# lms-07/LGTEUN

Hardware: AMD Instinct MI355X
Metric: train image-pairs/sec, GF-2 4-band 128x128, K=4, bs=32/GPU (higher is better)
Workload: dtype f32 (GEMMs and the local mixer: split 16-bit MFMA -- f16 pairs in the forward FFN, the W2 products of its backward and P V, bf16 triples elsewhere -- fp32 accumulate; fp32-equivalent); 1 GPU; BASELINE configs[1]: C=4, MS 32x32, PAN 128x128, K=4, 32 pairs/GPU, train step = fwd + L1 + bwd + Adam + StepLR tick; mode=faithful, global_batch=32, parallelism=dp1, dropout=True

## Files before the change

include/lgteun_hip.h:

```cpp
#ifndef LGTEUN_HIP_H
#define LGTEUN_HIP_H

#include <stddef.h>
#include <stdint.h>

#ifdef __cplusplus
extern "C" {
#endif

#define LG_TENSORS_SHARED 12
#define LG_TENSORS_PER_STAGE 119

#define LG_FLAG_FAITHFUL 1
#define LG_FLAG_SAVE 2
#define LG_FLAG_DROPOUT 4

#define LG_FLAG_BWD_LGT 8
#define LG_FLAG_BWD_DATA 16

#define LG_FLAG_CHAINED 32

#define LG_FLAG_DEFER_DEAD 64

enum lg_kernel_id {
    LG_K_NONE = 0, LG_K_FFN1, LG_K_FFN2, LG_K_FFT, LG_K_ATTN, LG_K_UPFUSE, LG_K_DOWN, LG_K_EMBED, LG_K_TAIL, LG_K_DATASTEP,
    LG_K_FFN1_BWD, LG_K_FFN2_BWD, LG_K_FFT_BWD, LG_K_ATTN_BWD, LG_K_WGRAD, LG_K_COUNT
};

typedef struct lg_config {
    int32_t C;
    int32_t K;
    int32_t H, W;
    int32_t precision;
    uint32_t variant;
} lg_config;

#define LG_VAR_FFN_IMPL_MASK 3u
#define LG_VAR_FFN_STRIP 1u
#define LG_VAR_FFN_TILE 2u
#define LG_VAR_FFN_XP 3u
#define LG_VAR_FFN_SAVE_MASK (3u << 2)
#define LG_VAR_FFN_SAVE3 (1u << 2)
#define LG_VAR_FFN_SAVE5 (2u << 2)
#define LG_VAR_FFN_BWD32_PAIR (1u << 4)
#define LG_VAR_FFN_DWBWD_TILE (1u << 5)
#define LG_VAR_ATTN_BWD_R3 (1u << 6)
#define LG_VAR_DSTEP_TILES (1u << 7)
#define LG_VAR_ATTN_FWD_VALU (1u << 8)
#define LG_VAR_FFN_BF16X3 (1u << 9)
#define LG_VAR_FFT_FULL (1u << 10)
#define LG_VAR_FFN_BWD_BF16X3 (1u << 11)
#define LG_VAR_ATTN_BWD_CORE_M (1u << 12)
#define LG_VAR_FFN_XS (1u << 13)
#define LG_VAR_ATTN_BF16X3 (1u << 14)
#define LG_VAR_FFN_H3_RECOMPUTE (1u << 15)
#define LG_VAR_ATTN_BWD_RESTATS (1u << 16)
#define LG_VAR_ALL 0x1ffffu

typedef struct lg_plan lg_plan;

const char* lg_version(void);
#define LG_ABI_VERSION 2
int32_t lg_abi_version(void);
const char* lg_last_error(void);

int lg_plan_create(const lg_config* cfg, const int64_t* offsets, int32_t n_offsets, lg_plan** out);
void lg_plan_destroy(lg_plan* plan);
size_t lg_workspace_bytes(const lg_plan* plan, int32_t B, int32_t train);

int lgteun_forward(const lg_plan* plan, const float* params, const float* ms, const float* pan, float* out,
                   void* workspace, size_t workspace_bytes, int32_t B, int32_t flags, uint64_t seed, void* stream);

int lgteun_dead_forward(const lg_plan* plan, const float* params, void* workspace, size_t workspace_bytes, int32_t B, int32_t flags,
                        uint64_t seed, void* stream);

int lgteun_backward(const lg_plan* plan, const float* params, float* grads, const float* ms, const float* pan,
                    const float* dout, void* workspace, size_t workspace_bytes, int32_t B, int32_t flags,
                    uint64_t seed, void* stream);

int lg_l1_loss(const float* out, const float* gt, float* dout, float* loss_accum, int64_t n_local, int64_t n_global,
               float scale, void* stream);

int lg_adam_step(float* params, const float* grads, float* exp_avg, float* exp_avg_sq, const int64_t* ranges,
                 int32_t n_ranges, int64_t max_range, int32_t step, float lr, float beta1, float beta2, float eps,
                 float grad_scale, void* stream);

int lg_l2_loss(const float* out, const float* gt, float* dout, float* loss_accum, int64_t n_local, int64_t n_global,
               float scale, void* stream);

#define LG_OPT_ADAM 0
#define LG_OPT_ADAMW 1
#define LG_OPT_SGD 2
#define LG_OPT_RMSPROP 3
#define LG_OPT_AMSGRAD 1
#define LG_OPT_NESTEROV 2
#define LG_OPT_CENTERED 4
int lg_optim_step(float* params, const float* grads, float* state0, float* state1, float* state2, const int64_t* ranges,
                  int32_t n_ranges, int64_t max_range, int32_t step, int32_t algo, int32_t flags, double lr, double h0, double h1,
                  double eps, double weight_decay, double grad_scale, void* stream);

int lg_prof_enable(int32_t kernel_id, int32_t max_launches);
int lg_prof_reset(void);
void lg_prof_pause(int32_t paused);
int lg_prof_read(double* total_ms, int64_t* launches);
void lg_prof_disable(void);
const char* lg_kernel_name(int32_t kernel_id);

int lg_dropout_mask(uint64_t seed, int32_t stage, int32_t blk, int64_t first, int64_t n, float* out, void* stream);

int lg_op_resample(const float* x, float* y, int32_t planes, int32_t hi, int32_t wi, int32_t mode, void* stream);
int lg_op_data_step(const lg_plan* plan, const float* params, int32_t stage, const float* z_in, const float* ms,
                    const float* pan, float* z_out, float* tmp, int32_t B, void* stream);
int lg_op_lgt(const lg_plan* plan, const float* params, int32_t stage, const float* z, float* out, void* workspace,
              size_t workspace_bytes, int32_t B, int32_t flags, uint64_t seed, void* stream);
int lg_op_block(const lg_plan* plan, const float* params, int32_t stage, int32_t blk, int32_t which, const float* x,
                float* y, void* workspace, size_t workspace_bytes, int32_t B, void* stream);

int lg_op_block_bwd(const lg_plan* plan, const float* params, float* grads, int32_t stage, int32_t blk, int32_t which,
                    const float* x, const float* dy, float* dx, void* workspace, size_t workspace_bytes, int32_t B,
                    void* stream);

int lg_op_data_step_bwd(const lg_plan* plan, const float* params, float* grads, int32_t stage, const float* z_in, const float* ms,
                        const float* pan, const float* dz_out, float* dz_in, void* workspace, size_t workspace_bytes, int32_t B,
                        void* stream);
int lg_op_lgt_bwd(const lg_plan* plan, const float* params, float* grads, int32_t stage, const float* z, const float* dout, float* dz,
                  void* workspace, size_t workspace_bytes, int32_t B, int32_t flags, uint64_t seed, void* stream);

#define LG_IQA_PEAK 2047.5
#define LG_IQA_SSIM_TAPS 11
#define LG_IQA_SSIM_SIGMA 1.5
#define LG_IQA_Q_BLOCK 8
#define LG_IQA_RATIO 4
#define LG_IQA_QNR_BLOCK 32
#define LG_IQA_MTF_TAPS 41
#define LG_IQA_MTF_GAIN 0.15
#define LG_IQA_MAX_BANDS 16
size_t lg_iqa_workspace_bytes(int32_t B, int32_t C, int32_t H, int32_t W, int32_t no_ref);
int lg_iqa_ref(const float* pred, const float* gt, double* out, int32_t B, int32_t C, int32_t H, int32_t W, float scale,
               void* workspace, size_t workspace_bytes, void* stream);
int lg_iqa_no_ref(const float* pred, const float* pan, const float* ms, double* out, int32_t B, int32_t C, int32_t H, int32_t W,
                  float scale, void* workspace, size_t workspace_bytes, void* stream);

#ifdef __cplusplus
}
#endif
#endif
```

lgteun_amd/_lib.py:

```python
import ctypes
import os
from ctypes import POINTER, c_char_p, c_double, c_float, c_int32, c_int64, c_size_t, c_uint64, c_void_p

_HERE = os.path.dirname(os.path.abspath(__file__))
LIB_PATH = os.environ.get('LGTEUN_HIP_LIB') or os.path.join(_HERE, '_lgteun_hip.so')

LG_FLAG_FAITHFUL = 1
LG_FLAG_SAVE = 2
LG_FLAG_DROPOUT = 4
LG_FLAG_BWD_LGT = 8
LG_FLAG_BWD_DATA = 16
LG_FLAG_CHAINED = 32
LG_FLAG_DEFER_DEAD = 64
KERNEL_IDS = {n: i for i, n in enumerate(['none', 'ffn1', 'ffn', 'fft', 'attn', 'upfuse', 'down', 'embed', 'tail', 'datastep', 'ffn1_bwd',
                                           'ffn2_bwd', 'fft_bwd', 'attn_bwd', 'wgrad'])}


class LgConfig(ctypes.Structure):
    _fields_ = [('C', c_int32), ('K', c_int32), ('H', c_int32), ('W', c_int32), ('precision', c_int32), ('variant', ctypes.c_uint32)]


LG_VAR_FFN_STRIP, LG_VAR_FFN_TILE, LG_VAR_FFN_XP = 1, 2, 3
LG_VAR_FFN_SAVE3, LG_VAR_FFN_SAVE5 = 1 << 2, 2 << 2
LG_VAR_FFN_BWD32_PAIR, LG_VAR_FFN_DWBWD_TILE, LG_VAR_ATTN_BWD_R3 = 1 << 4, 1 << 5, 1 << 6
LG_VAR_DSTEP_TILES = 1 << 7
LG_VAR_ATTN_FWD_VALU = 1 << 8
LG_VAR_FFN_BF16X3 = 1 << 9
LG_VAR_FFT_FULL = 1 << 10
LG_VAR_FFN_BWD_BF16X3 = 1 << 11
LG_VAR_ATTN_BWD_CORE_M = 1 << 12
LG_VAR_FFN_XS = 1 << 13
LG_VAR_ATTN_BF16X3 = 1 << 14
LG_VAR_FFN_H3_RECOMPUTE = 1 << 15
LG_VAR_ATTN_BWD_RESTATS = 1 << 16
LG_OPT_ADAM, LG_OPT_ADAMW, LG_OPT_SGD, LG_OPT_RMSPROP = 0, 1, 2, 3
LG_OPT_AMSGRAD, LG_OPT_NESTEROV, LG_OPT_CENTERED = 1, 2, 4
LG_ABI_VERSION = 2


def variant_from_env(env=None):
    env = os.environ if env is None else env
    v = {'strip': LG_VAR_FFN_STRIP, 'tile': LG_VAR_FFN_TILE, 'xp': LG_VAR_FFN_XP}.get(env.get('LG_FFN_IMPL', ''), 0)
    v |= {'3': LG_VAR_FFN_SAVE3, '5': LG_VAR_FFN_SAVE5}.get(env.get('LG_FFN_SAVE', ''), 0)
    if env.get('LG_FFN_BWD32') == 'pair':
        v |= LG_VAR_FFN_BWD32_PAIR
    if env.get('LG_FFN_DWBWD') == 'tile':
        v |= LG_VAR_FFN_DWBWD_TILE
    if env.get('LG_ATTN_BWD') in ('old', 'r3'):
        v |= LG_VAR_ATTN_BWD_R3
    if env.get('LG_DSTEP') == 'tiles':
        v |= LG_VAR_DSTEP_TILES
    if env.get('LG_ATTN_FWD', '') == 'valu':
        v |= LG_VAR_ATTN_FWD_VALU
    if env.get('LG_FFN_SPLIT', '') == 'bf16x3':
        v |= LG_VAR_FFN_BF16X3
    if env.get('LG_FFT', '') == 'full':
        v |= LG_VAR_FFT_FULL
    if env.get('LG_FFN_BWD_SPLIT', '') == 'bf16x3':
        v |= LG_VAR_FFN_BWD_BF16X3
    if env.get('LG_ATTN_BWD_CORE', '') == 'm':
        v |= LG_VAR_ATTN_BWD_CORE_M
    if env.get('LG_FFN_FWD', '') == 'xs':
        v |= LG_VAR_FFN_XS
    if env.get('LG_ATTN_SPLIT', '') == 'bf16x3':
        v |= LG_VAR_ATTN_BF16X3
    if env.get('LG_FFN_H3', '') == 'recompute':
        v |= LG_VAR_FFN_H3_RECOMPUTE
    if env.get('LG_ATTN_BWD_STATS', '') == 'recompute':
        v |= LG_VAR_ATTN_BWD_RESTATS
    return v


class LgteunHipError(RuntimeError):
    pass


_lib = None

SIGNATURES = {
    'lg_version': (c_char_p, []),
    'lg_abi_version': (c_int32, []),
    'lg_last_error': (c_char_p, []),
    'lg_plan_create': (c_int32, [POINTER(LgConfig), POINTER(c_int64), c_int32, POINTER(c_void_p)]),
    'lg_plan_destroy': (None, [c_void_p]),
    'lg_workspace_bytes': (c_size_t, [c_void_p, c_int32, c_int32]),
    'lgteun_forward': (c_int32, [c_void_p, c_void_p, c_void_p, c_void_p, c_void_p, c_void_p, c_size_t, c_int32, c_int32,
                                 c_uint64, c_void_p]),
    'lgteun_backward': (c_int32, [c_void_p, c_void_p, c_void_p, c_void_p, c_void_p, c_void_p, c_void_p, c_size_t, c_int32,
                                  c_int32, c_uint64, c_void_p]),
    'lgteun_dead_forward': (c_int32, [c_void_p, c_void_p, c_void_p, c_size_t, c_int32, c_int32, c_uint64, c_void_p]),
    'lg_l1_loss': (c_int32, [c_void_p, c_void_p, c_void_p, c_void_p, c_int64, c_int64, c_float, c_void_p]),
    'lg_adam_step': (c_int32, [c_void_p, c_void_p, c_void_p, c_void_p, c_void_p, c_int32, c_int64, c_int32, c_float, c_float,
                               c_float, c_float, c_float, c_void_p]),
    'lg_l2_loss': (c_int32, [c_void_p, c_void_p, c_void_p, c_void_p, c_int64, c_int64, c_float, c_void_p]),
    'lg_optim_step': (c_int32, [c_void_p, c_void_p, c_void_p, c_void_p, c_void_p, c_void_p, c_int32, c_int64, c_int32, c_int32, c_int32,
                                c_double, c_double, c_double, c_double, c_double, c_double, c_void_p]),
    'lg_op_resample': (c_int32, [c_void_p, c_void_p, c_int32, c_int32, c_int32, c_int32, c_void_p]),
    'lg_op_data_step': (c_int32, [c_void_p, c_void_p, c_int32, c_void_p, c_void_p, c_void_p, c_void_p, c_void_p, c_int32,
                                  c_void_p]),
    'lg_op_lgt': (c_int32, [c_void_p, c_void_p, c_int32, c_void_p, c_void_p, c_void_p, c_size_t, c_int32, c_int32, c_uint64,
                            c_void_p]),
    'lg_op_block': (c_int32, [c_void_p, c_void_p, c_int32, c_int32, c_int32, c_void_p, c_void_p, c_void_p, c_size_t, c_int32,
                              c_void_p]),
    'lg_dropout_mask': (c_int32, [c_uint64, c_int32, c_int32, c_int64, c_int64, c_void_p, c_void_p]),
    'lg_prof_enable': (c_int32, [c_int32, c_int32]),
    'lg_prof_reset': (c_int32, []),
    'lg_prof_pause': (None, [c_int32]),
    'lg_prof_read': (c_int32, [POINTER(ctypes.c_double), POINTER(c_int64)]),
    'lg_prof_disable': (None, []),
    'lg_kernel_name': (c_char_p, [c_int32]),
    'lg_op_data_step_bwd': (c_int32, [c_void_p, c_void_p, c_void_p, c_int32, c_void_p, c_void_p, c_void_p, c_void_p, c_void_p, c_void_p,
                                      c_size_t, c_int32, c_void_p]),
    'lg_op_lgt_bwd': (c_int32, [c_void_p, c_void_p, c_void_p, c_int32, c_void_p, c_void_p, c_void_p, c_void_p, c_size_t, c_int32, c_int32,
                                c_uint64, c_void_p]),
    'lg_op_block_bwd': (c_int32, [c_void_p, c_void_p, c_void_p, c_int32, c_int32, c_int32, c_void_p, c_void_p, c_void_p, c_void_p,
                                  c_size_t, c_int32, c_void_p]),
    'lg_iqa_workspace_bytes': (c_size_t, [c_int32, c_int32, c_int32, c_int32, c_int32]),
    'lg_iqa_ref': (c_int32, [c_void_p, c_void_p, c_void_p, c_int32, c_int32, c_int32, c_int32, c_float, c_void_p, c_size_t, c_void_p]),
    'lg_iqa_no_ref': (c_int32, [c_void_p, c_void_p, c_void_p, c_void_p, c_int32, c_int32, c_int32, c_int32, c_float, c_void_p, c_size_t,
                                c_void_p]),
}


def lib():
    global _lib
    if _lib is None:
        if not os.path.exists(LIB_PATH):
            raise LgteunHipError(
                f'HIP extension not built: {LIB_PATH} is missing. Run `make` (or __graft_entry__.build()). '
                'lgteun_amd has no CPU/PyTorch fallback.')
        L = ctypes.CDLL(LIB_PATH)
        for name, (res, args) in SIGNATURES.items():
            fn = getattr(L, name)
            fn.restype = res
            fn.argtypes = args
        got = int(L.lg_abi_version())
        if got != LG_ABI_VERSION:
            raise LgteunHipError(f'{LIB_PATH}: ABI version {got}, this binding was written for {LG_ABI_VERSION} (include/lgteun_hip.h): rebuild with `make`')
        _lib = L
    return _lib


def check(rc, what):
    if rc != 0:
        msg = lib().lg_last_error().decode(errors='replace')
        raise LgteunHipError(f'{what} failed (rc={rc}): {msg}')
```

lgteun_amd/csrc/api.hip:

```cpp
#include <stdarg.h>
#include <stdio.h>
#include <stdlib.h>
#include <string.h>
#include <math.h>
#include <atomic>
#include <mutex>

#pragma GCC visibility push(default)
#include "../../include/lgteun_hip.h"
#pragma GCC visibility pop

#include "kernels.h"
#include "workspace.h"
#include "backward.h"

static thread_local char g_err[512] = "";

void lg_set_error(const char* fmt, ...) {
    va_list ap;
    va_start(ap, fmt);
    vsnprintf(g_err, sizeof(g_err), fmt, ap);
    va_end(ap);
}

static struct {
    std::atomic<int> kid{0};
    std::atomic<int> paused{0};
    int cap = 0, n = 0;
    hipEvent_t* ev = nullptr;
    std::mutex mu;
} g_prof;

void lg_prof_begin(int kid, hipStream_t s) {
    if (kid != g_prof.kid.load(std::memory_order_relaxed) || g_prof.paused.load(std::memory_order_relaxed)) return;
    std::lock_guard<std::mutex> lk(g_prof.mu);
    if (kid != g_prof.kid.load(std::memory_order_relaxed) || g_prof.n >= g_prof.cap) return;
    hipEventRecord(g_prof.ev[2 * g_prof.n], s);
}
void lg_prof_end(int kid, hipStream_t s) {
    if (kid != g_prof.kid.load(std::memory_order_relaxed) || g_prof.paused.load(std::memory_order_relaxed)) return;
    std::lock_guard<std::mutex> lk(g_prof.mu);
    if (kid != g_prof.kid.load(std::memory_order_relaxed) || g_prof.n >= g_prof.cap) return;
    hipEventRecord(g_prof.ev[2 * g_prof.n + 1], s);
    g_prof.n++;
}
static void prof_disable_locked() {
    for (int i = 0; i < 2 * g_prof.cap; ++i) hipEventDestroy(g_prof.ev[i]);
    free(g_prof.ev);
    g_prof.ev = nullptr;
    g_prof.cap = g_prof.n = 0;
    g_prof.kid.store(0);
    g_prof.paused.store(0);
}
extern "C" void lg_prof_disable(void) {
    std::lock_guard<std::mutex> lk(g_prof.mu);
    prof_disable_locked();
}
extern "C" int lg_prof_enable(int32_t kernel_id, int32_t max_launches) {
    if (kernel_id <= 0 || kernel_id >= LG_K_COUNT || max_launches <= 0) { lg_set_error("prof_enable: invalid argument"); return -1; }
    std::lock_guard<std::mutex> lk(g_prof.mu);
    prof_disable_locked();
    g_prof.ev = (hipEvent_t*)malloc(sizeof(hipEvent_t) * 2 * max_launches);
    for (int i = 0; i < 2 * max_launches; ++i) {
        hipError_t e = hipEventCreate(&g_prof.ev[i]);
        if (e != hipSuccess) { lg_set_error("prof_enable: hipEventCreate: %s", hipGetErrorString(e)); return (int)e; }
    }
    g_prof.cap = max_launches;
    g_prof.kid.store(kernel_id);
    return 0;
}
extern "C" void lg_prof_pause(int32_t paused) { g_prof.paused.store(paused ? 1 : 0); }
extern "C" int lg_prof_reset(void) {
    std::lock_guard<std::mutex> lk(g_prof.mu);
    g_prof.n = 0;
    return 0;
}
extern "C" int lg_prof_read(double* total_ms, int64_t* launches) {
    if (!total_ms || !launches) { lg_set_error("prof_read: null argument"); return -1; }
    std::lock_guard<std::mutex> lk(g_prof.mu);
    double tot = 0.0;
    for (int i = 0; i < g_prof.n; ++i) {
        hipError_t e = hipEventSynchronize(g_prof.ev[2 * i + 1]);
        if (e != hipSuccess) { lg_set_error("prof_read: %s", hipGetErrorString(e)); return (int)e; }
        float ms = 0.f;
        hipEventElapsedTime(&ms, g_prof.ev[2 * i], g_prof.ev[2 * i + 1]);
        tot += ms;
    }
    *total_ms = tot;
    *launches = g_prof.n;
    return 0;
}
extern "C" const char* lg_kernel_name(int32_t k) {
    static const char* names[LG_K_COUNT] = {"none", "k_ffn1", "fused FFN forward (k_ffn_xr e=16 / k_ffn_x32 e=32 / k_ffn1_x64+k_ffn2_x64 e=64)", "k_fftmix", "k_attn", "k_upfuse", "k_down", "k_embed", "k_tail",
                                            "k_resample_dw", "k_ffn1_bwd", "k_ffn2_bwd", "k_fftmix_bwd", "k_attn_bwd", "k_wgrad"};
    return (k >= 0 && k < LG_K_COUNT) ? names[k] : "?";
}

extern "C" const char* lg_version(void) { return "lgteun_hip 0.2 (gfx950)"; }
extern "C" int32_t lg_abi_version(void) { return LG_ABI_VERSION; }
extern "C" const char* lg_last_error(void) { return g_err; }

extern "C" int lg_plan_create(const lg_config* cfg, const int64_t* offsets, int32_t n_offsets, lg_plan** out) {
    if (!cfg || !offsets || !out) { lg_set_error("plan_create: null argument"); return -1; }
    if (cfg->C != 4 && cfg->C != 8) { lg_set_error("plan_create: C must be 4 or 8 (got %d)", cfg->C); return -2; }
    if (cfg->precision != 0 && cfg->precision != 1) { lg_set_error("plan_create: precision must be 0 (fp32) or 1 (bf16 hidden storage)"); return -2; }
    if (cfg->K < 1 || cfg->K > LG_MAX_K) { lg_set_error("plan_create: K out of range (%d)", cfg->K); return -2; }
    if (cfg->H % 16 || cfg->W % 16 || cfg->H <= 0 || cfg->W <= 0) { lg_set_error("plan_create: H,W must be positive multiples of 16"); return -2; }
    if (cfg->H > 1024 || cfg->W > 1024) {
        lg_set_error("plan_create: PAN sizes up to 1024x1024 are supported (got %dx%d)", cfg->H, cfg->W);
        return -2;
    }
    const int expect = S_NSHARED + cfg->K + L_NSLOT * cfg->K;
    if (n_offsets != expect) { lg_set_error("plan_create: expected %d offsets, got %d", expect, n_offsets); return -2; }
    for (int i = 0; i < n_offsets; ++i)
        if (offsets[i] < 0 || (offsets[i] & 3)) { lg_set_error("plan_create: offset %d (=%lld) must be a non-negative multiple of 4 floats", i, (long long)offsets[i]); return -2; }
    if (cfg->variant & ~LG_VAR_ALL) { lg_set_error("plan_create: unknown variant bits 0x%x", cfg->variant & ~LG_VAR_ALL); return -2; }
    if ((cfg->variant & LG_VAR_FFN_SAVE_MASK) == LG_VAR_FFN_SAVE_MASK) { lg_set_error("plan_create: invalid FFN save variant"); return -2; }
#ifndef LG_BUILD_AB
    if ((cfg->variant & LG_VAR_FFN_IMPL_MASK) >= LG_VAR_FFN_TILE) { lg_set_error("plan_create: FFN variants 2 / 3 exist in `make AB=1` builds only"); return -2; }
    if (cfg->precision == 1 && (cfg->variant & LG_VAR_FFN_IMPL_MASK)) { lg_set_error("plan_create: precision = 1 with an FFN variant exists in `make AB=1` builds only"); return -2; }
#endif
    lg_plan* p = new lg_plan;
    p->cfg = *cfg;
    p->n_offsets = n_offsets;
    {
        const uint32_t v = cfg->variant;
        p->ffn_tile = (int)(v & LG_VAR_FFN_IMPL_MASK);
        const uint32_t sv = v & LG_VAR_FFN_SAVE_MASK;
        p->save_mode = sv == LG_VAR_FFN_SAVE5 ? 5 : (sv == LG_VAR_FFN_SAVE3 ? 3 : 2);
        p->bwd32_old = (v & LG_VAR_FFN_BWD32_PAIR) ? 1 : 0;
        p->dwbwd_tile = (v & LG_VAR_FFN_DWBWD_TILE) ? 1 : 0;
        p->attn_bwd_old = (v & LG_VAR_ATTN_BWD_R3) ? 1 : 0;
        p->dstep_tiles = (v & LG_VAR_DSTEP_TILES) ? 1 : 0;
        p->attn_fwd_valu = (v & LG_VAR_ATTN_FWD_VALU) ? 1 : 0;
        p->ffn_bf16x3 = (v & LG_VAR_FFN_BF16X3) ? 1 : 0;
        p->fft_full = (v & LG_VAR_FFT_FULL) ? 1 : 0;
        p->attn_bwd_core_m = (v & LG_VAR_ATTN_BWD_CORE_M) ? 1 : 0;
        p->ffn_bwd_bf16x3 = (v & LG_VAR_FFN_BWD_BF16X3) ? 1 : 0;
        p->ffn_xs = (v & LG_VAR_FFN_XS) ? 1 : 0;
        p->attn_bf16x3 = (v & LG_VAR_ATTN_BF16X3) ? 1 : 0;
        p->ffn_h3_re = (v & LG_VAR_FFN_H3_RECOMPUTE) ? 1 : 0;
        p->attn_restats = (v & LG_VAR_ATTN_BWD_RESTATS) ? 1 : 0;
    }
    p->off = (int64_t*)malloc(sizeof(int64_t) * n_offsets);
    memcpy(p->off, offsets, sizeof(int64_t) * n_offsets);
    *out = p;
    return 0;
}

extern "C" void lg_plan_destroy(lg_plan* plan) {
    if (!plan) return;
    free(plan->off);
    delete plan;
}

extern "C" size_t lg_workspace_bytes(const lg_plan* plan, int32_t B, int32_t train) {
    if (!plan || B <= 0 || train < 0 || train > 2) return 0;
    NetBufs nb;
    carve(plan, B, train, nullptr, nb);
    size_t fwd = nb.bytes;
    if (train) fwd += bwd_workspace_bytes(plan, B);
    return fwd;
}

static int data_step_fwd(const lg_plan* pl, const float* P, int stage, const float* z_in, const float* ms, const float* pan,
                         float* z_out, float* t1, float* r, float* s1, float* pr, int B, hipStream_t s) {
    const lg_config& c = pl->cfg;
    const int planes = B * c.C, H = c.H, W = c.W;
    if (pl->dstep_fused(H, W)) {
        DstepFwdArgs f;
        f.z = z_in; f.ms = ms; f.pan = pan; f.zout = z_out; f.t1 = t1; f.r = r; f.s1 = s1; f.pr = pr;
        f.d1w = P + pl->shared(S_D1W); f.d1b = P + pl->shared(S_D1B); f.d3w = P + pl->shared(S_D3W); f.d3b = P + pl->shared(S_D3B);
        f.dt1w = P + pl->shared(S_DT1W); f.dt1b = P + pl->shared(S_DT1B); f.dt3w = P + pl->shared(S_DT3W); f.dt3b = P + pl->shared(S_DT3B);
        f.rw = P + pl->shared(S_RW); f.rb = P + pl->shared(S_RB); f.rtw = P + pl->shared(S_RTW); f.rtb = P + pl->shared(S_RTB);
        f.eta = P + pl->eta(stage);
        f.B = B; f.C = c.C; f.N = H;
        return launch_dstep_fwd(f, s);
    }
    DwArgs a;
    memset(&a, 0, sizeof(a));
    a.C = c.C; a.planes = planes;
    int rc;
    a.in = z_in; a.out = t1; a.w9 = P + pl->shared(S_D1W); a.bias = P + pl->shared(S_D1B);
    a.hi = H; a.wi = W; a.ho = H / 2; a.wo = W / 2;
    if ((rc = launch_resample_dw(0, 0, a, s))) return rc;
    a.in = t1; a.out = r; a.w9 = P + pl->shared(S_D3W); a.bias = P + pl->shared(S_D3B); a.sub = ms;
    a.hi = H / 2; a.wi = W / 2; a.ho = H / 4; a.wo = W / 4;
    if ((rc = launch_resample_dw(0, 1, a, s))) return rc;
    a.in = r; a.out = s1; a.w9 = P + pl->shared(S_DT1W); a.bias = P + pl->shared(S_DT1B); a.sub = nullptr;
    a.hi = H / 4; a.wi = W / 4; a.ho = H / 2; a.wo = W / 2;
    if ((rc = launch_resample_dw(1, 0, a, s))) return rc;
    a.in = s1; a.out = z_out; a.w9 = P + pl->shared(S_DT3W); a.bias = P + pl->shared(S_DT3B);
    a.z = z_in; a.pan = pan; a.rw = P + pl->shared(S_RW); a.rb = P + pl->shared(S_RB);
    a.rtw = P + pl->shared(S_RTW); a.rtb = P + pl->shared(S_RTB); a.eta = P + pl->eta(stage);
    a.hi = H / 2; a.wi = W / 2; a.ho = H; a.wo = W;
    return launch_resample_dw(1, 2, a, s);
}

static int block_mixer_fwd(const lg_plan* pl, const float* P, int stage, int j, const BlockBufs& bb, const float* posT, int B,
                           int flags, uint64_t seed, hipStream_t s, float* fft_scratch = nullptr, const float* attn_scales = nullptr) {
    int rc;
    FftArgs f;
    f.g = bb.g; f.o = bb.o2;
    f.amp = (flags & LG_FLAG_SAVE) ? bb.amp : nullptr;
    f.pha = (flags & LG_FLAG_SAVE) ? bb.pha : nullptr;
    f.sgn = (flags & LG_FLAG_SAVE) ? bb.sgn : nullptr;
    f.scratch = fft_scratch;
    f.ampw = P + pl->blk(stage, j, B_AMPW); f.ampb = P + pl->blk(stage, j, B_AMPB);
    f.phaw = P + pl->blk(stage, j, B_PHAW); f.phab = P + pl->blk(stage, j, B_PHAB);
    f.ch = bb.e / 2; f.planes = B * f.ch; f.n = bb.h; f.h = bb.h; f.w = bb.w; f.full = pl->fft_full;
    if ((rc = launch_fftmix(f, s))) return rc;
    AttnArgs t;
    t.x = bb.xin; t.o2 = bb.o2; t.y = bb.xmid; t.posT = posT; t.pos = P + pl->blk(stage, j, B_POS);
    t.bf16 = pl->cfg.precision == 1 ? 1 : 0;
    t.ln1g = P + pl->blk(stage, j, B_LN1G); t.ln1b = P + pl->blk(stage, j, B_LN1B);
    t.qkvw = P + pl->blk(stage, j, B_QKVW); t.qkvb = P + pl->blk(stage, j, B_QKVB);
    t.projw = P + pl->blk(stage, j, B_PROJW); t.projb = P + pl->blk(stage, j, B_PROJB);
    t.B = B; t.h = bb.h; t.w = bb.w;
    t.dropout = (flags & LG_FLAG_DROPOUT) ? 1 : 0;
    t.seed = mix_seed(seed, stage, j);
    t.scales = (attn_scales && pl->attn_f16x2()) ? attn_scales + ((size_t)stage * 5 + j) * 4 : nullptr;
    if ((flags & LG_FLAG_SAVE) && pl->attn_saves_stats(bb.e)) { t.save_o = bb.att_o; t.save_l = bb.att_l; }
    return pl->attn_fwd_valu ? launch_attn(bb.e, t, s) : launch_attn_m(bb.e, t, s);
}

static int block_ffn_fwd(const lg_plan* pl, const float* P, int stage, int j, const BlockBufs& bb, float* g_next, int next_blk,
                         int B, int flags, hipStream_t s, float* wsplit, const float* ffn_scales) {
    int rc;
    Ffn1Args a1;
    const bool pre = pl->ffn_saves_preact(bb.e);
    const bool noh1 = pl->ffn_bwd_x(bb.e) || pl->ffn1_bwd_x32(bb.e);
    a1.x = bb.xmid; a1.a1s = ((flags & LG_FLAG_SAVE) && !noh1) ? bb.a1 : nullptr; a1.g1s = ((flags & LG_FLAG_SAVE) && !pre && !noh1) ? bb.g1 : nullptr; a1.h2 = bb.h2;
    a1.ln2g = P + pl->blk(stage, j, B_LN2G); a1.ln2b = P + pl->blk(stage, j, B_LN2B);
    a1.w1 = P + pl->blk(stage, j, B_W1); a1.b1 = P + pl->blk(stage, j, B_B1);
    a1.w2 = P + pl->blk(stage, j, B_W2); a1.b2 = P + pl->blk(stage, j, B_B2);
    a1.P = (long)B * bb.h * bb.w;
    a1.hbf = pl->hidden_bf16(bb.e) ? 1 : 0;
    a1.tile16 = pl->ffn_tile ? pl->ffn_tile : ((pl->ffn_xs && bb.e == 16) ? 4 : 0);
    a1.wsplit = wsplit ? wsplit + ((size_t)stage * 5 + j) * (ffn_wsplit_bytes(8 * pl->cfg.C) / sizeof(float)) : nullptr;
    a1.wsplit_ready = (wsplit && bb.e >= 32) ? 1 : 0;
    a1.scales = pl->ffn_f16x2(bb.e) ? ffn_scales + ((size_t)stage * 5 + j) * 8 : nullptr;
    Ffn2Args a2;
    a2.h2 = bb.h2; a2.x = bb.xmid; a2.a3s = ((flags & LG_FLAG_SAVE) && !pl->ffn_h3_recompute(bb.e)) ? bb.a3 : nullptr; a2.g3s = ((flags & LG_FLAG_SAVE) && !pre && !pl->ffn_dw_x32(bb.e, bb.h, bb.w)) ? bb.g3 : nullptr; a2.y = bb.xout;
    a2.g = g_next;
    a2.dww = P + pl->blk(stage, j, B_DWW); a2.dwb = P + pl->blk(stage, j, B_DWB);
    a2.w3 = P + pl->blk(stage, j, B_W3); a2.b3 = P + pl->blk(stage, j, B_B3);
    a2.n1g = g_next ? P + pl->blk(stage, next_blk, B_LN1G) : nullptr;
    a2.n1b = g_next ? P + pl->blk(stage, next_blk, B_LN1B) : nullptr;
    a2.B = B; a2.h = bb.h; a2.w = bb.w; a2.hbf = a1.hbf;
    a1.h2 = ((flags & LG_FLAG_SAVE) || bb.e == 64) ? bb.h2 : nullptr;
    rc = launch_ffn_fused(bb.e, a1, a2, s);
    if (rc != LG_FFN_NOT_FUSED) return rc;
    a1.h2 = bb.h2;
    if ((rc = launch_ffn1(bb.e, a1, s))) return rc;
    return launch_ffn2(bb.e, a2, s);
}

static int pos_transpose_stages(const lg_plan* pl, const float* P, int st0, int st1, float* posT_all, hipStream_t s) {
    if (st1 <= st0) return 0;
    const float* src[5 * LG_MAX_K];
    float* dst[5 * LG_MAX_K];
    int n = 0;
    for (int st = st0; st < st1; ++st)
        for (int j = 0; j < 5; ++j, ++n) { src[n] = P + pl->blk(st, j, B_POS); dst[n] = posT_all + ((size_t)st * 5 + j) * 2 * 64 * 64; }
    return launch_pos_transpose_n(n, src, dst, s);
}
static int prep_stages(const lg_plan* pl, const float* P, int st0, int st1, NetBufs& nb, hipStream_t s) {
    int rc = pl->attn_fwd_valu ? pos_transpose_stages(pl, P, st0, st1, nb.posT, s) : 0;
    if (rc || st1 <= st0) return rc;
    const int E = 4 * pl->cfg.C;
    if (pl->ffn_f16x2(E) || pl->ffn_f16x2(2 * E)) {
        FfnPrepJob jobs[5 * LG_MAX_K];
        int n = 0;
        for (int st = st0; st < st1; ++st)
            for (int j = 0; j < 5; ++j, ++n) {
                FfnPrepJob& q = jobs[n];
                q.ln2g = P + pl->blk(st, j, B_LN2G); q.ln2b = P + pl->blk(st, j, B_LN2B);
                q.w1 = P + pl->blk(st, j, B_W1); q.b1 = P + pl->blk(st, j, B_B1); q.w2 = P + pl->blk(st, j, B_W2); q.b2 = P + pl->blk(st, j, B_B2);
                q.dww = P + pl->blk(st, j, B_DWW); q.dwb = P + pl->blk(st, j, B_DWB); q.w3 = P + pl->blk(st, j, B_W3);
                q.e = j == 2 ? 2 * E : E;
                q.ln1g = P + pl->blk(st, j, B_LN1G); q.ln1b = P + pl->blk(st, j, B_LN1B); q.qkvw = P + pl->blk(st, j, B_QKVW); q.qkvb = P + pl->blk(st, j, B_QKVB);
            }
        if ((rc = launch_ffn_scales(n, jobs, nb.ffn_scales + (size_t)st0 * 5 * 8, s, pl->attn_f16x2() ? nb.attn_scales + (size_t)st0 * 5 * 4 : nullptr))) return rc;
    }
    SplitWJob sj[5 * LG_MAX_K];
    int ns = 0;
    const size_t slot = ffn_wsplit_bytes(2 * E) / sizeof(float);
    for (int st = st0; st < st1; ++st)
        for (int j = 0; j < 5; ++j) {
            const int e = j == 2 ? 2 * E : E;
            if (e < 32 || e % 32) continue;
            SplitWJob& q = sj[ns++];
            q.w1 = P + pl->blk(st, j, B_W1); q.w2 = P + pl->blk(st, j, B_W2); q.w3 = P + pl->blk(st, j, B_W3);
            q.e = e; q.np = pl->hidden_bf16(e) ? 1 : (pl->ffn_f16x2(e) ? 2 : 3);
            q.scales = q.np == 2 ? nb.ffn_scales + ((size_t)st * 5 + j) * 8 : nullptr;
            q.out = nb.wsplit + ((size_t)st * 5 + j) * slot;
        }
    return ns ? launch_split_w_jobs(ns, sj, s) : 0;
}

static int lgt_fwd(const lg_plan* pl, const float* P, int stage, const float* z, float* out, NetBufs& nb, int B, int flags,
                   uint64_t seed, hipStream_t s, bool pos_ready = false) {
    const lg_config& c = pl->cfg;
    const int E = 4 * c.C;
    int rc;
    float* posT = nb.posT + (size_t)stage * 5 * 2 * 64 * 64;
    if (!pos_ready && (rc = prep_stages(pl, P, stage, stage + 1, nb, s))) return rc;
    EmbedArgs ea;
    ea.z = z; ea.x = nb.x0; ea.g = nb.blk[0].g;
    ea.dww = P + pl->lgt(stage, L_PE_DWW); ea.dwb = P + pl->lgt(stage, L_PE_DWB);
    ea.w = P + pl->lgt(stage, L_PE_W); ea.b = P + pl->lgt(stage, L_PE_B);
    ea.lng = P + pl->lgt(stage, L_PE_LNG); ea.lnb = P + pl->lgt(stage, L_PE_LNB);
    ea.n1g = P + pl->blk(stage, 0, B_LN1G); ea.n1b = P + pl->blk(stage, 0, B_LN1B);
    ea.HW = c.H * c.W; ea.total = (long)B * c.H * c.W;
    if ((rc = launch_embed(c.C, ea, s))) return rc;
    if ((rc = block_mixer_fwd(pl, P, stage, 0, nb.blk[0], posT + 0 * 8192, B, flags, seed, s, nb.fft_scratch, nb.attn_scales))) return rc;
    if ((rc = block_ffn_fwd(pl, P, stage, 0, nb.blk[0], nb.blk[1].g, 1, B, flags, s, nb.wsplit, nb.ffn_scales))) return rc;
    if ((rc = block_mixer_fwd(pl, P, stage, 1, nb.blk[1], posT + 1 * 8192, B, flags, seed, s, nb.fft_scratch, nb.attn_scales))) return rc;
    if ((rc = block_ffn_fwd(pl, P, stage, 1, nb.blk[1], nullptr, 0, B, flags, s, nb.wsplit, nb.ffn_scales))) return rc;
    DownArgs da;
    da.x = nb.blk[1].xout; da.y = nb.blk[2].xin; da.g = nb.blk[2].g;
    da.u_save = (flags & LG_FLAG_SAVE) ? nb.u_down : nullptr;
    da.w = P + pl->lgt(stage, L_DOWNW); da.b = P + pl->lgt(stage, L_DOWNB);
    da.n1g = P + pl->blk(stage, 2, B_LN1G); da.n1b = P + pl->blk(stage, 2, B_LN1B);
    da.B = B; da.H = c.H; da.W = c.W;
    if ((rc = launch_down(E, da, s))) return rc;
    if ((rc = block_mixer_fwd(pl, P, stage, 2, nb.blk[2], posT + 2 * 8192, B, flags, seed, s, nb.fft_scratch, nb.attn_scales))) return rc;
    if ((rc = block_ffn_fwd(pl, P, stage, 2, nb.blk[2], nullptr, 0, B, flags, s, nb.wsplit, nb.ffn_scales))) return rc;
    UpFuseArgs ua;
    ua.xb = nb.blk[2].xout; ua.skip = nb.blk[1].xout; ua.y = nb.blk[3].xin; ua.g = nb.blk[3].g;
    ua.t_save = (flags & LG_FLAG_SAVE) ? nb.t_up : nullptr;
    ua.upw = P + pl->lgt(stage, L_UPW); ua.upb = P + pl->lgt(stage, L_UPB);
    ua.fw = P + pl->lgt(stage, L_FUSEW); ua.fb = P + pl->lgt(stage, L_FUSEB);
    ua.n1g = P + pl->blk(stage, 3, B_LN1G); ua.n1b = P + pl->blk(stage, 3, B_LN1B);
    ua.B = B; ua.H = c.H; ua.W = c.W;
    if ((rc = launch_upfuse(E, ua, s))) return rc;
    if ((rc = block_mixer_fwd(pl, P, stage, 3, nb.blk[3], posT + 3 * 8192, B, flags, seed, s, nb.fft_scratch, nb.attn_scales))) return rc;
    if ((rc = block_ffn_fwd(pl, P, stage, 3, nb.blk[3], nb.blk[4].g, 4, B, flags, s, nb.wsplit, nb.ffn_scales))) return rc;
    if ((rc = block_mixer_fwd(pl, P, stage, 4, nb.blk[4], posT + 4 * 8192, B, flags, seed, s, nb.fft_scratch, nb.attn_scales))) return rc;
    if ((rc = block_ffn_fwd(pl, P, stage, 4, nb.blk[4], nullptr, 0, B, flags, s, nb.wsplit, nb.ffn_scales))) return rc;
    TailArgs ta;
    ta.x = nb.blk[4].xout; ta.z = z; ta.out = out;
    ta.w = P + pl->lgt(stage, L_TAILW); ta.b = P + pl->lgt(stage, L_TAILB);
    ta.HW = c.H * c.W; ta.total = (long)B * c.H * c.W;
    return launch_tail(c.C, ta, s);
}

extern "C" int lgteun_forward(const lg_plan* plan, const float* params, const float* ms, const float* pan, float* out,
                              void* workspace, size_t workspace_bytes, int32_t B, int32_t flags, uint64_t seed, void* stream) {
    if (!plan || !params || !ms || !pan || !out || !workspace || B <= 0) { lg_set_error("forward: null/invalid argument"); return -1; }
    const bool chained = (flags & LG_FLAG_CHAINED) != 0;
    const int train = (flags & LG_FLAG_SAVE) ? (chained ? 2 : 1) : 0;
    if (workspace_bytes < lg_workspace_bytes(plan, B, train)) {
        lg_set_error("forward: workspace too small (%zu < %zu)", workspace_bytes, lg_workspace_bytes(plan, B, train));
        return -3;
    }
    hipStream_t s = (hipStream_t)stream;
    const lg_config& c = plan->cfg;
    NetBufs nb;
    carve(plan, B, train, workspace, nb);
    int rc;
    const bool all_stages = chained || ((flags & LG_FLAG_FAITHFUL) && !(flags & LG_FLAG_DEFER_DEAD));
    if ((rc = prep_stages(plan, params, all_stages ? 0 : c.K - 1, c.K, nb, s))) return rc;
    if ((rc = launch_resample(2, ms, nb.Z[0], B * c.C, c.H / 4, c.W / 4, s))) return rc;
    if (chained) {
        for (int i = 0; i < c.K; ++i) {
            if ((rc = data_step_fwd(plan, params, i, nb.X[i], ms, pan, nb.Z[i + 1], nb.t1[i], nb.r[i], nb.s1[i], nb.pr, B, s))) return rc;
            NetBufs sv = (train == 2) ? stage_view(nb, i) : nb;
            if ((rc = lgt_fwd(plan, params, i, nb.Z[i + 1], i == c.K - 1 ? out : nb.X[i + 1], sv, B, flags, seed, s, true))) return rc;
        }
        return 0;
    }
    for (int i = 0; i < c.K; ++i) {
        if ((rc = data_step_fwd(plan, params, i, nb.Z[i], ms, pan, nb.Z[i + 1], nb.t1[i], nb.r[i], nb.s1[i], nb.pr, B, s))) return rc;
        const bool last = (i == c.K - 1);
        if (last) {
            if ((rc = lgt_fwd(plan, params, i, nb.Z[i + 1], out, nb, B, flags, seed, s, true))) return rc;
        } else if ((flags & LG_FLAG_FAITHFUL) && !(flags & LG_FLAG_DEFER_DEAD)) {
            if ((rc = lgt_fwd(plan, params, i, nb.Z[i + 1], nb.deadout, nb, B, flags & ~LG_FLAG_SAVE, seed, s, true))) return rc;
        }
    }
    return 0;
}

extern "C" int lgteun_dead_forward(const lg_plan* plan, const float* params, void* workspace, size_t workspace_bytes, int32_t B,
                                   int32_t flags, uint64_t seed, void* stream) {
    if (!plan || !params || !workspace || B <= 0) { lg_set_error("dead_forward: null/invalid argument"); return -1; }
    if ((flags & LG_FLAG_CHAINED) || !(flags & LG_FLAG_FAITHFUL)) { lg_set_error("dead_forward: only the faithful unfolding has dead stages"); return -2; }
    const int train = (flags & LG_FLAG_SAVE) ? 1 : 0;
    if (workspace_bytes < lg_workspace_bytes(plan, B, train)) { lg_set_error("dead_forward: workspace too small"); return -3; }
    NetBufs nb;
    carve(plan, B, train, workspace, nb);
    {
        const int rc = prep_stages(plan, params, 0, plan->cfg.K - 1, nb, (hipStream_t)stream);
        if (rc) return rc;
    }
    for (int i = 0; i + 1 < plan->cfg.K; ++i) {
        const int rc = lgt_fwd(plan, params, i, nb.Z[i + 1], nb.deadout, nb, B, flags & ~LG_FLAG_SAVE, seed, (hipStream_t)stream, true);
        if (rc) return rc;
    }
    return 0;
}

extern "C" int lgteun_backward(const lg_plan* plan, const float* params, float* grads, const float* ms, const float* pan,
                               const float* dout, void* workspace, size_t workspace_bytes, int32_t B, int32_t flags, uint64_t seed,
                               void* stream) {
    if (!plan || !params || !grads || !ms || !pan || !dout || !workspace || B <= 0) { lg_set_error("backward: null/invalid argument"); return -1; }
    const int train = (flags & LG_FLAG_CHAINED) ? 2 : 1;
    if ((flags & LG_FLAG_CHAINED) && (flags & (LG_FLAG_BWD_LGT | LG_FLAG_BWD_DATA))) {
        lg_set_error("backward: LG_FLAG_BWD_LGT / LG_FLAG_BWD_DATA do not apply to LG_FLAG_CHAINED");
        return -2;
    }
    if (workspace_bytes < lg_workspace_bytes(plan, B, train)) { lg_set_error("backward: workspace too small"); return -3; }
    NetBufs nb;
    carve(plan, B, train, workspace, nb);
    return net_backward(plan, params, grads, ms, pan, dout, nb, (char*)workspace + nb.bytes, B, flags, seed, (hipStream_t)stream);
}

extern "C" int lg_op_resample(const float* x, float* y, int32_t planes, int32_t hi, int32_t wi, int32_t mode, void* stream) {
    if (!x || !y || planes <= 0 || hi <= 0 || wi <= 0 || mode < 0 || mode > 2) { lg_set_error("op_resample: invalid argument"); return -1; }
    if (mode == 0 && ((hi & 1) || (wi & 1))) { lg_set_error("op_resample: x0.5 needs even sizes"); return -2; }
    return launch_resample(mode, x, y, planes, hi, wi, (hipStream_t)stream);
}

extern "C" int lg_op_data_step(const lg_plan* plan, const float* params, int32_t stage, const float* z_in, const float* ms,
                               const float* pan, float* z_out, float* tmp, int32_t B, void* stream) {
    if (!plan || !params || !z_in || !ms || !pan || !z_out || !tmp || stage < 0 || stage >= plan->cfg.K) { lg_set_error("op_data_step: invalid argument"); return -1; }
    const lg_config& c = plan->cfg;
    size_t q = (size_t)B * c.C * c.H * c.W / 4;
    return data_step_fwd(plan, params, stage, z_in, ms, pan, z_out, tmp, tmp + q, tmp + 2 * q, tmp + 3 * q, B, (hipStream_t)stream);
}

extern "C" int lg_op_lgt(const lg_plan* plan, const float* params, int32_t stage, const float* z, float* out, void* workspace,
                         size_t workspace_bytes, int32_t B, int32_t flags, uint64_t seed, void* stream) {
    if (!plan || !params || !z || !out || !workspace || stage < 0 || stage >= plan->cfg.K) { lg_set_error("op_lgt: invalid argument"); return -1; }
    const int train = (flags & LG_FLAG_SAVE) ? 1 : 0;
    if (workspace_bytes < lg_workspace_bytes(plan, B, train)) { lg_set_error("op_lgt: workspace too small"); return -3; }
    NetBufs nb;
    carve(plan, B, train, workspace, nb);
    return lgt_fwd(plan, params, stage, z, out, nb, B, flags, seed, (hipStream_t)stream);
}

extern "C" int lg_op_block(const lg_plan* plan, const float* params, int32_t stage, int32_t blk, int32_t which, const float* x,
                           float* y, void* workspace, size_t workspace_bytes, int32_t B, void* stream) {
    if (!plan || !params || !x || !y || !workspace || stage < 0 || stage >= plan->cfg.K || blk < 0 || blk > 4 || which < 0 || which > 2) {
        lg_set_error("op_block: invalid argument");
        return -1;
    }
    if (workspace_bytes < lg_workspace_bytes(plan, B, 0)) { lg_set_error("op_block: workspace too small"); return -3; }
    hipStream_t s = (hipStream_t)stream;
    NetBufs nb;
    carve(plan, B, 0, workspace, nb);
    BlockBufs bb = nb.blk[blk];
    int rc;
    const size_t npix = (size_t)B * bb.h * bb.w;
    if (which == 0 || which == 1) {
        if ((rc = launch_ln_split(bb.e, x, params + plan->blk(stage, blk, B_LN1G), params + plan->blk(stage, blk, B_LN1B), bb.g, B,
                                  bb.h * bb.w, s)))
            return rc;
    }
    if (which == 0) {
        FftArgs f;
        f.g = bb.g; f.o = y; f.amp = nullptr; f.pha = nullptr; f.sgn = nullptr; f.scratch = nb.fft_scratch;
        f.ampw = params + plan->blk(stage, blk, B_AMPW); f.ampb = params + plan->blk(stage, blk, B_AMPB);
        f.phaw = params + plan->blk(stage, blk, B_PHAW); f.phab = params + plan->blk(stage, blk, B_PHAB);
        f.ch = bb.e / 2; f.planes = B * f.ch; f.n = bb.h; f.h = bb.h; f.w = bb.w; f.full = plan->fft_full;
        return launch_fftmix(f, s);
    }
    if (which == 1) {
        float* posT = nb.posT;
        if ((rc = prep_stages(plan, params, stage, stage + 1, nb, s))) return rc;
        if ((rc = launch_pos_transpose(params + plan->blk(stage, blk, B_POS), posT, s))) return rc;
        bb.xin = const_cast<float*>(x);
        bb.xmid = y;
        return block_mixer_fwd(plan, params, stage, blk, bb, posT, B, 0, 0, s, nb.fft_scratch, nb.attn_scales);
    }
    bb.xmid = const_cast<float*>(x);
    bb.xout = y;
    (void)npix;
    if ((rc = prep_stages(plan, params, stage, stage + 1, nb, s))) return rc;
    return block_ffn_fwd(plan, params, stage, blk, bb, nullptr, 0, B, 0, s, nb.wsplit, nb.ffn_scales);
}

extern "C" int lg_op_block_bwd(const lg_plan* plan, const float* params, float* grads, int32_t stage, int32_t blk, int32_t which,
                               const float* x, const float* dy, float* dx, void* workspace, size_t workspace_bytes, int32_t B,
                               void* stream) {
    if (!plan || !params || !grads || !x || !dy || !dx || !workspace || stage < 0 || stage >= plan->cfg.K || blk < 0 || blk > 4 ||
        which < 0 || which > 2) {
        lg_set_error("op_block_bwd: invalid argument");
        return -1;
    }
    if (workspace_bytes < lg_workspace_bytes(plan, B, 1)) { lg_set_error("op_block_bwd: workspace too small"); return -3; }
    hipStream_t s = (hipStream_t)stream;
    NetBufs nb;
    carve(plan, B, 1, workspace, nb);
    BlockBufs& bb = nb.blk[blk];
    int rc;
    if (which == 0 || which == 1) {
        if ((rc = launch_ln_split(bb.e, x, params + plan->blk(stage, blk, B_LN1G), params + plan->blk(stage, blk, B_LN1B), bb.g, B,
                                  bb.h * bb.w, s)))
            return rc;
        if ((rc = prep_stages(plan, params, stage, stage + 1, nb, s))) return rc;
        if ((rc = launch_pos_transpose(params + plan->blk(stage, blk, B_POS), nb.posT, s))) return rc;
        bb.xin = const_cast<float*>(x);
        if ((rc = block_mixer_fwd(plan, params, stage, blk, bb, nb.posT, B, LG_FLAG_SAVE, 0, s, nb.fft_scratch, nb.attn_scales))) return rc;
    } else {
        bb.xmid = const_cast<float*>(x);
        if ((rc = prep_stages(plan, params, stage, stage + 1, nb, s))) return rc;
        if ((rc = block_ffn_fwd(plan, params, stage, blk, bb, nullptr, 0, B, LG_FLAG_SAVE, s, nb.wsplit, nb.ffn_scales))) return rc;
    }
    return op_block_bwd(plan, params, grads, stage, blk, which, dy, dx, nb, (char*)workspace + nb.bytes, B, s);
}

extern "C" int lg_op_data_step_bwd(const lg_plan* plan, const float* params, float* grads, int32_t stage, const float* z_in,
                                   const float* ms, const float* pan, const float* dz_out, float* dz_in, void* workspace,
                                   size_t workspace_bytes, int32_t B, void* stream) {
    if (!plan || !params || !grads || !z_in || !ms || !pan || !dz_out || !dz_in || !workspace || B <= 0 || stage < 0 || stage >= plan->cfg.K) {
        lg_set_error("op_data_step_bwd: invalid argument");
        return -1;
    }
    if (workspace_bytes < lg_workspace_bytes(plan, B, 1)) { lg_set_error("op_data_step_bwd: workspace too small"); return -3; }
    hipStream_t s = (hipStream_t)stream;
    NetBufs nb;
    carve(plan, B, 1, workspace, nb);
    int rc;
    if ((rc = data_step_fwd(plan, params, stage, z_in, ms, pan, nb.Z[stage + 1], nb.t1[stage], nb.r[stage], nb.s1[stage], nb.pr, B, s))) return rc;
    return op_data_step_bwd(plan, params, grads, stage, nb, (char*)workspace + nb.bytes, z_in, pan, dz_out, dz_in, B, s);
}

extern "C" int lg_op_lgt_bwd(const lg_plan* plan, const float* params, float* grads, int32_t stage, const float* z, const float* dout,
                             float* dz, void* workspace, size_t workspace_bytes, int32_t B, int32_t flags, uint64_t seed, void* stream) {
    if (!plan || !params || !grads || !z || !dout || !dz || !workspace || B <= 0 || stage < 0 || stage >= plan->cfg.K) {
        lg_set_error("op_lgt_bwd: invalid argument");
        return -1;
    }
    if (flags & ~LG_FLAG_DROPOUT) { lg_set_error("op_lgt_bwd: only LG_FLAG_DROPOUT applies"); return -2; }
    if (workspace_bytes < lg_workspace_bytes(plan, B, 1)) { lg_set_error("op_lgt_bwd: workspace too small"); return -3; }
    hipStream_t s = (hipStream_t)stream;
    NetBufs nb;
    carve(plan, B, 1, workspace, nb);
    int rc;
    if ((rc = lgt_fwd(plan, params, stage, z, nb.deadout, nb, B, flags | LG_FLAG_SAVE, seed, s))) return rc;
    return op_lgt_bwd(plan, params, grads, stage, nb, (char*)workspace + nb.bytes, z, dout, dz, B, flags, seed, s);
}

__global__ __launch_bounds__(256) void k_dropout_mask(uint64_t seed, long first, long n, float* __restrict__ out) {
    for (long i = blockIdx.x * 256L + threadIdx.x; i < n; i += gridDim.x * 256L) out[i] = dropout_scale(seed, (uint64_t)(first + i));
}
extern "C" int lg_dropout_mask(uint64_t seed, int32_t stage, int32_t blk, int64_t first, int64_t n, float* out, void* stream) {
    if (!out || n < 0 || first < 0 || stage < 0 || stage >= LG_MAX_K || blk < 0 || blk > 4) { lg_set_error("dropout_mask: invalid argument"); return -1; }
    if (n == 0) return 0;
    const int grid = (int)((n + 255) / 256 < 1024 ? (n + 255) / 256 : 1024);
    k_dropout_mask<<<grid, 256, 0, (hipStream_t)stream>>>(mix_seed(seed, stage, blk), first, n, out);
    LG_CHECK_LAUNCH();
    return 0;
}

__global__ __launch_bounds__(256) void k_l1(const float* __restrict__ out, const float* __restrict__ gt, float* __restrict__ dout,
                                            float* loss_accum, long n, float inv_n, float gscale) {
    float part = 0.f;
    const long n4 = n >> 2, stride = (long)gridDim.x * 256L;
    const float4* __restrict__ o4 = reinterpret_cast<const float4*>(out);
    const float4* __restrict__ g4 = reinterpret_cast<const float4*>(gt);
    float4* __restrict__ d4 = reinterpret_cast<float4*>(dout);
    auto one = [&](float d) { part += fabsf(d); return d > 0.f ? gscale : (d < 0.f ? -gscale : 0.f); };
    long i = blockIdx.x * 256L + threadIdx.x;
    for (; i + 3 * stride < n4; i += 4 * stride) {
        float4 a[4], b[4];
#pragma unroll
        for (int u = 0; u < 4; ++u) { a[u] = o4[i + u * stride]; b[u] = g4[i + u * stride]; }
#pragma unroll
        for (int u = 0; u < 4; ++u)
            d4[i + u * stride] = make_float4(one(a[u].x - b[u].x), one(a[u].y - b[u].y), one(a[u].z - b[u].z), one(a[u].w - b[u].w));
    }
    for (; i < n4; i += stride) {
        const float4 a = o4[i], b = g4[i];
        d4[i] = make_float4(one(a.x - b.x), one(a.y - b.y), one(a.z - b.z), one(a.w - b.w));
    }
    for (long j = 4 * n4 + blockIdx.x * 256L + threadIdx.x; j < n; j += stride) dout[j] = one(out[j] - gt[j]);
#pragma unroll
    for (int off = 32; off > 0; off >>= 1) part += __shfl_xor(part, off);
    __shared__ float sm[4];
    if ((threadIdx.x & 63) == 0) sm[threadIdx.x >> 6] = part;
    __syncthreads();
    if (threadIdx.x == 0) atomicAdd(loss_accum, (sm[0] + sm[1] + sm[2] + sm[3]) * inv_n);
}

extern "C" int lg_l1_loss(const float* out, const float* gt, float* dout, float* loss_accum, int64_t n_local, int64_t n_global,
                          float scale, void* stream) {
    if (!out || !gt || !dout || !loss_accum || n_local <= 0 || n_global <= 0) { lg_set_error("l1_loss: invalid argument"); return -1; }
    if (((uintptr_t)out | (uintptr_t)gt | (uintptr_t)dout) & 15) { lg_set_error("l1_loss: tensors must be 16-byte aligned"); return -1; }
    int grid = (int)((n_local / 4 + 255) / 256);
    if (grid > 256) grid = 256;
    if (grid < 1) grid = 1;
    k_l1<<<grid, 256, 0, (hipStream_t)stream>>>(out, gt, dout, loss_accum, n_local, 1.0f / (float)n_global, scale / (float)n_global);
    LG_CHECK_LAUNCH();
    return 0;
}

#define LG_L2_SLOTS 64
struct l2_slot { double acc; unsigned int arrived; unsigned int pad; };
__device__ l2_slot g_l2_slots[LG_L2_SLOTS];

__global__ __launch_bounds__(256) void k_l2(const float* __restrict__ out, const float* __restrict__ gt, float* __restrict__ dout,
                                            float* loss_accum, long n, double inv_n, float norm, float scale, int slot_id) {
    l2_slot* slot = &g_l2_slots[slot_id];
    double part = 0.0;
    const long n4 = n >> 2, stride = (long)gridDim.x * 256L;
    const float4* __restrict__ o4 = reinterpret_cast<const float4*>(out);
    const float4* __restrict__ g4 = reinterpret_cast<const float4*>(gt);
    float4* __restrict__ d4 = reinterpret_cast<float4*>(dout);
    auto one = [&](float d) { part += (double)d * (double)d; return (norm * d) * scale; };
    long i = blockIdx.x * 256L + threadIdx.x;
    for (; i + 3 * stride < n4; i += 4 * stride) {
        float4 a[4], b[4];
#pragma unroll
        for (int u = 0; u < 4; ++u) { a[u] = o4[i + u * stride]; b[u] = g4[i + u * stride]; }
#pragma unroll
        for (int u = 0; u < 4; ++u)
            d4[i + u * stride] = make_float4(one(a[u].x - b[u].x), one(a[u].y - b[u].y), one(a[u].z - b[u].z), one(a[u].w - b[u].w));
    }
    for (; i < n4; i += stride) {
        const float4 a = o4[i], b = g4[i];
        d4[i] = make_float4(one(a.x - b.x), one(a.y - b.y), one(a.z - b.z), one(a.w - b.w));
    }
    for (long j = 4 * n4 + blockIdx.x * 256L + threadIdx.x; j < n; j += stride) dout[j] = one(out[j] - gt[j]);
#pragma unroll
    for (int off = 32; off > 0; off >>= 1) part += __shfl_xor(part, off);
    __shared__ double sm[4];
    if ((threadIdx.x & 63) == 0) sm[threadIdx.x >> 6] = part;
    __syncthreads();
    if (threadIdx.x == 0) {
        atomicAdd(&slot->acc, sm[0] + sm[1] + sm[2] + sm[3]);
        __threadfence();
        if (atomicAdd(&slot->arrived, 1u) == gridDim.x - 1) {
            __threadfence();
            const double total = __longlong_as_double((long long)atomicExch((unsigned long long*)&slot->acc, 0ull));
            atomicExch(&slot->arrived, 0u);
            atomicAdd(loss_accum, (float)(total * inv_n));
        }
    }
}

extern "C" int lg_l2_loss(const float* out, const float* gt, float* dout, float* loss_accum, int64_t n_local, int64_t n_global,
                          float scale, void* stream) {
    if (!out || !gt || !dout || !loss_accum || n_local <= 0 || n_global <= 0) { lg_set_error("l2_loss: invalid argument"); return -1; }
    if (((uintptr_t)out | (uintptr_t)gt | (uintptr_t)dout) & 15) { lg_set_error("l2_loss: tensors must be 16-byte aligned"); return -1; }
    int grid = (int)((n_local / 4 + 255) / 256);
    if (grid > 256) grid = 256;
    if (grid < 1) grid = 1;
    static std::atomic<unsigned> next_slot{0};
    k_l2<<<grid, 256, 0, (hipStream_t)stream>>>(out, gt, dout, loss_accum, n_local, 1.0 / (double)n_global, (float)(2.0 / (double)n_global), scale,
                                                (int)(next_slot.fetch_add(1) % LG_L2_SLOTS));
    LG_CHECK_LAUNCH();
    return 0;
}

extern "C" size_t lg_iqa_workspace_bytes(int32_t B, int32_t C, int32_t H, int32_t W, int32_t no_ref) {
    return iqa_workspace_bytes(B, C, H, W, no_ref);
}
extern "C" int lg_iqa_ref(const float* pred, const float* gt, double* out, int32_t B, int32_t C, int32_t H, int32_t W, float scale,
                          void* workspace, size_t workspace_bytes, void* stream) {
    return launch_iqa_ref(pred, gt, out, B, C, H, W, scale, workspace, workspace_bytes, (hipStream_t)stream);
}
extern "C" int lg_iqa_no_ref(const float* pred, const float* pan, const float* ms, double* out, int32_t B, int32_t C, int32_t H, int32_t W,
                             float scale, void* workspace, size_t workspace_bytes, void* stream) {
    return launch_iqa_no_ref(pred, pan, ms, out, B, C, H, W, scale, workspace, workspace_bytes, (hipStream_t)stream);
}

__global__ __launch_bounds__(256) void k_adam(float* __restrict__ p, const float* __restrict__ g, float* __restrict__ m,
                                              float* __restrict__ v, const int64_t* __restrict__ ranges, float step_size, float b1,
                                              float b2, float inv_bc2_sqrt, float eps, float gscale) {
    const int64_t lo = ranges[2 * blockIdx.y], hi = ranges[2 * blockIdx.y + 1];
    for (int64_t i = lo + blockIdx.x * 256L + threadIdx.x; i < hi; i += (int64_t)gridDim.x * 256L) {
        float gi = g[i] * gscale;
        float mi = b1 * m[i] + (1.0f - b1) * gi;
        float vi = b2 * v[i] + (1.0f - b2) * gi * gi;
        m[i] = mi;
        v[i] = vi;
        float denom = sqrtf(vi) * inv_bc2_sqrt + eps;
        p[i] = p[i] - step_size * (mi / denom);
    }
}

extern "C" int lg_adam_step(float* params, const float* grads, float* exp_avg, float* exp_avg_sq, const int64_t* ranges,
                            int32_t n_ranges, int64_t max_range, int32_t step, float lr, float beta1, float beta2, float eps,
                            float grad_scale, void* stream) {
    if (!params || !grads || !exp_avg || !exp_avg_sq || !ranges || n_ranges <= 0 || step < 1) { lg_set_error("adam_step: invalid argument"); return -1; }
    double bc1 = 1.0 - pow((double)beta1, (double)step);
    double bc2 = 1.0 - pow((double)beta2, (double)step);
    int gx = (int)((max_range + 255) / 256);
    if (gx < 1) gx = 1;
    if (gx > 512) gx = 512;
    dim3 grid(gx, n_ranges);
    k_adam<<<grid, 256, 0, (hipStream_t)stream>>>(params, grads, exp_avg, exp_avg_sq, ranges, (float)(lr / bc1), beta1, beta2,
                                                   (float)(1.0 / sqrt(bc2)), eps, grad_scale);
    LG_CHECK_LAUNCH();
    return 0;
}

enum { OPT_WD = 1, OPT_ALT = 2, OPT_MOM = 4, OPT_FIRST = 8 };
struct optim_args {
    float lr;
    float h0, h1;
    float c0, c1;
    float eps, wd, gscale;
    float bc2_sqrt;
    float decay;
};

#ifndef LG_OPT_FMA
#define LG_OPT_FMA(a, b, c) __builtin_fmaf(a, b, c)
#endif
template <int ALGO, int OPT>
__global__ __launch_bounds__(256) void k_optim(float* __restrict__ p, const float* __restrict__ g, float* __restrict__ s0,
                                               float* __restrict__ s1, float* __restrict__ s2, const int64_t* __restrict__ ranges,
                                               optim_args a) {
#pragma clang fp contract(off)
    const int64_t lo = ranges[2 * blockIdx.y], hi = ranges[2 * blockIdx.y + 1];
    for (int64_t i = lo + blockIdx.x * 256L + threadIdx.x; i < hi; i += (int64_t)gridDim.x * 256L) {
        float pi = p[i];
        float gi = g[i] * a.gscale;
        if constexpr (ALGO == LG_OPT_ADAMW) pi = pi * a.decay;
        else if constexpr ((OPT & OPT_WD) != 0) gi = LG_OPT_FMA(a.wd, pi, gi);
        if constexpr (ALGO == LG_OPT_ADAM || ALGO == LG_OPT_ADAMW) {
            float mi = s0[i];
            mi = LG_OPT_FMA(a.c0, gi - mi, mi);
            const float vb = s1[i] * a.h1;
            float vi = LG_OPT_FMA(a.c1, gi * gi, vb);
            s0[i] = mi;
            s1[i] = vi;
            if constexpr ((OPT & OPT_ALT) != 0) { vi = fmaxf(s2[i], vi); s2[i] = vi; }
            float denom = sqrtf(vi) / a.bc2_sqrt;
            denom = denom + a.eps;
            pi = LG_OPT_FMA(-a.lr, mi / denom, pi);
        } else if constexpr (ALGO == LG_OPT_SGD) {
            if constexpr ((OPT & OPT_MOM) != 0) {
                float bi;
                if constexpr ((OPT & OPT_FIRST) != 0) bi = gi;
                else bi = LG_OPT_FMA(a.c1, gi, s0[i] * a.h0);
                s0[i] = bi;
                if constexpr ((OPT & OPT_ALT) != 0) gi = LG_OPT_FMA(a.h0, bi, gi);
                else gi = bi;
            }
            pi = LG_OPT_FMA(-a.lr, gi, pi);
        } else {
            const float vb = s0[i] * a.h0;
            const float vi = LG_OPT_FMA(a.c0, gi * gi, vb);
            s0[i] = vi;
            float avg;
            if constexpr ((OPT & OPT_ALT) != 0) {
                float ci = s2[i];
                ci = LG_OPT_FMA(a.c0, gi - ci, ci);
                s2[i] = ci;
                avg = sqrtf(LG_OPT_FMA(-1.0f, ci * ci, vi));
            } else {
                avg = sqrtf(vi);
            }
            avg = avg + a.eps;
            if constexpr ((OPT & OPT_MOM) != 0) {
                const float bi = LG_OPT_FMA(1.0f, gi / avg, s1[i] * a.h1);
                s1[i] = bi;
                pi = LG_OPT_FMA(-a.lr, bi, pi);
            } else {
                pi = LG_OPT_FMA(-a.lr, gi / avg, pi);
            }
        }
        p[i] = pi;
    }
}

template <int ALGO, int OPT>
static void launch_optim(dim3 grid, hipStream_t st, float* p, const float* g, float* s0, float* s1, float* s2, const int64_t* ranges,
                         const optim_args& a) {
    k_optim<ALGO, OPT><<<grid, 256, 0, st>>>(p, g, s0, s1, s2, ranges, a);
}

extern "C" int lg_optim_step(float* params, const float* grads, float* state0, float* state1, float* state2, const int64_t* ranges,
                             int32_t n_ranges, int64_t max_range, int32_t step, int32_t algo, int32_t flags, double lr, double h0, double h1,
                             double eps, double weight_decay, double grad_scale, void* stream) {
    if (!params || !grads || !ranges || n_ranges <= 0 || step < 1 || algo < LG_OPT_ADAM || algo > LG_OPT_RMSPROP ||
        (flags & ~(LG_OPT_AMSGRAD | LG_OPT_NESTEROV | LG_OPT_CENTERED))) { lg_set_error("optim_step: invalid argument"); return -1; }
    const bool adam = algo == LG_OPT_ADAM || algo == LG_OPT_ADAMW;
    const int own = adam ? LG_OPT_AMSGRAD : (algo == LG_OPT_SGD ? LG_OPT_NESTEROV : LG_OPT_CENTERED);
    if (flags & ~own) { lg_set_error("optim_step: the flag belongs to another algorithm"); return -1; }
    int opt = (weight_decay != 0.0 && algo != LG_OPT_ADAMW ? OPT_WD : 0) | (flags ? OPT_ALT : 0);
    if (algo == LG_OPT_SGD && h0 != 0.0) opt |= OPT_MOM | (step == 1 ? OPT_FIRST : 0);
    if (algo == LG_OPT_RMSPROP && h1 > 0.0) opt |= OPT_MOM;
    if (algo == LG_OPT_SGD && (opt & OPT_ALT) && !(opt & OPT_MOM)) { lg_set_error("optim_step: nesterov needs a momentum"); return -1; }
    const bool need0 = algo != LG_OPT_SGD || (opt & OPT_MOM), need1 = adam || (algo == LG_OPT_RMSPROP && (opt & OPT_MOM));
    const bool need2 = algo != LG_OPT_SGD && (opt & OPT_ALT);
    if ((need0 && !state0) || (need1 && !state1) || (need2 && !state2)) { lg_set_error("optim_step: a state buffer of this option set is missing"); return -1; }
    optim_args a = {(float)lr, (float)h0, (float)h1, (float)(1.0 - h0), (float)(1.0 - h1), (float)eps, (float)weight_decay, (float)grad_scale,
                    1.f, 1.f};
    if (adam) {
        a.lr = (float)(lr / (1.0 - pow(h0, (double)step)));
        a.bc2_sqrt = (float)sqrt(1.0 - pow(h1, (double)step));
        a.decay = (float)(1.0 - lr * weight_decay);
    }
    int gx = (int)((max_range + 255) / 256);
    if (gx < 1) gx = 1;
    if (gx > 512) gx = 512;
    const dim3 grid(gx, n_ranges);
    const hipStream_t st = (hipStream_t)stream;
#define LG_OPT_CASE(A, O) case (A) * 16 + (O): launch_optim<A, O>(grid, st, params, grads, state0, state1, state2, ranges, a); break;
    switch (algo * 16 + opt) {
        LG_OPT_CASE(LG_OPT_ADAM, 0) LG_OPT_CASE(LG_OPT_ADAM, OPT_WD) LG_OPT_CASE(LG_OPT_ADAM, OPT_ALT) LG_OPT_CASE(LG_OPT_ADAM, OPT_WD | OPT_ALT)
        LG_OPT_CASE(LG_OPT_ADAMW, 0) LG_OPT_CASE(LG_OPT_ADAMW, OPT_ALT)
        LG_OPT_CASE(LG_OPT_SGD, 0) LG_OPT_CASE(LG_OPT_SGD, OPT_WD)
        LG_OPT_CASE(LG_OPT_SGD, OPT_MOM) LG_OPT_CASE(LG_OPT_SGD, OPT_MOM | OPT_WD)
        LG_OPT_CASE(LG_OPT_SGD, OPT_MOM | OPT_FIRST) LG_OPT_CASE(LG_OPT_SGD, OPT_MOM | OPT_FIRST | OPT_WD)
        LG_OPT_CASE(LG_OPT_SGD, OPT_MOM | OPT_ALT) LG_OPT_CASE(LG_OPT_SGD, OPT_MOM | OPT_ALT | OPT_WD)
        LG_OPT_CASE(LG_OPT_SGD, OPT_MOM | OPT_ALT | OPT_FIRST) LG_OPT_CASE(LG_OPT_SGD, OPT_MOM | OPT_ALT | OPT_FIRST | OPT_WD)
        LG_OPT_CASE(LG_OPT_RMSPROP, 0) LG_OPT_CASE(LG_OPT_RMSPROP, OPT_WD) LG_OPT_CASE(LG_OPT_RMSPROP, OPT_ALT) LG_OPT_CASE(LG_OPT_RMSPROP, OPT_ALT | OPT_WD)
        LG_OPT_CASE(LG_OPT_RMSPROP, OPT_MOM) LG_OPT_CASE(LG_OPT_RMSPROP, OPT_MOM | OPT_WD)
        LG_OPT_CASE(LG_OPT_RMSPROP, OPT_MOM | OPT_ALT) LG_OPT_CASE(LG_OPT_RMSPROP, OPT_MOM | OPT_ALT | OPT_WD)
        default: lg_set_error("optim_step: no kernel for this option set"); return -1;
    }
#undef LG_OPT_CASE
    LG_CHECK_LAUNCH();
    return 0;
}
```

lgteun_amd/csrc/bwd_kernels.h:

```cpp
#pragma once
#include "common.h"

struct WgradArgs {
    const void* Y;
    const void* X;
    float* dW;
    float* db;
    long P;
    int ldy, ldx, ldw;
    int N, K;
    int n_valid, k_valid;
    int ybf, xbf;
    int xgelu;
};
size_t wgrad_slab_floats(int N, int K, long P);
#define PIXEL_PART_WGS 2048
size_t chan_partial_floats(int C, int B, int H, int W);
struct ChanReduce {
    float* dst[14];
    float* dst2[14];
    int stride[14];
    int NK, C, nslices;
    unsigned allc_mask;
};
int launch_reduce_chan(const float* part, const ChanReduce& m, hipStream_t s);
int launch_reduce_slab_pair(const float* slab_a, const float* slab_b, long nslices, int n, float* dst_a, float* dst_b, hipStream_t s);

struct ReduceJob {
    const float* slab;
    float* dst;
    float* dst2;
    long nslices, slice_stride;
    int rows, cols, row_stride, ld, rows_valid, cols_valid;
};
#define LG_MAX_REDUCE_JOBS 56
struct ReduceJobTable {
    ReduceJob j[LG_MAX_REDUCE_JOBS];
    int n;
};
struct ReduceQueue {
    float* arena;
    size_t cap, off;
    hipStream_t stream;
    ReduceJobTable tab;
    void init(float* base, size_t cap_floats, hipStream_t s) { arena = base; cap = cap_floats; off = 0; stream = s; tab.n = 0; }
    float* take(size_t nfloats);
    int push(const ReduceJob& j);
    int flush();
};
int launch_reduce_slab_wb(const float* wslab, const float* bslab, long nslices, int rows, int cols, float* dW, int ld, float* db, hipStream_t s);
int launch_reduce_job(const ReduceJob& j, hipStream_t s);
bool reduce_chan_enqueue(const float* part, const ChanReduce& m, int* rc);
void reduce_queue_begin(ReduceQueue* q);
int reduce_queue_end();
int launch_wgrad(const WgradArgs& a, float* slab, hipStream_t s);
int launch_reduce_slab(const float* slab, long nslices, int rows, int cols, float* dst, int ld, int rows_valid, int cols_valid,
                       hipStream_t s);

struct DwBwdArgs {
    const float* gout;
    const float* in;
    float* gin;
    const float* w9;
    float* dw9;
    float* dbias;
    float* part;
    int C, planes, hi, wi, n_h, n_w;
};
int launch_dw_bwd(int mode, const DwBwdArgs& a, hipStream_t s);
struct DstepTopArgs {
    const float* g;
    const float* s1;
    const float* z;
    const float* pan;
    float* gu;
    float* dz;
    const float *w9, *b9, *rw, *rb, *rtw, *rtb, *eta;
    float *dw9, *dbias, *drw, *drb, *drtw, *drtb, *deta;
    float* part;
    int C, B, H, W;
};
int launch_dstep_top_bwd(const DstepTopArgs& a, hipStream_t s);
struct DstepPreBwdArgs {
    const float *z, *g, *pan;
    float* dz;
    const float *rw, *rb, *rtw, *rtb, *eta;
    float* part;
    int hw4;
};
struct DstepBwdArgs {
    const float* g;
    const float* z;
    const float* pan;
    const float *t1, *r, *s1;
    float* dz;
    const float *d1w, *d3w, *dt1w, *dt3w, *dt3b, *rw, *rb, *rtw, *rtb, *eta;
    float *part_top, *part_dt1, *part_d3, *part_d1, *part_pre;
    int B, C, N;
};
struct DstepBwdGrads { float *d1w, *d1b, *d3w, *d3b, *dt1w, *dt1b, *dt3w, *dt3b, *rw, *rb, *rtw, *rtb, *eta; };
size_t dstep_bwd_part_floats(int C, int B, int N);
int launch_dstep_bwd(const DstepBwdArgs& a, const DstepBwdGrads& g, hipStream_t s);
int launch_resample_adj(int mode, const float* gout, float* gin, int planes, int hi, int wi, int accumulate, hipStream_t s);

struct TailBwdArgs {
    const float* dout;
    const float* x;
    float* dx;
    float* dz;
    const float* w;
    float *d_w, *d_b;
    float* part;
    int HW;
    long total;
};
size_t tail_bwd_part_floats(int C);
int launch_tail_bwd(int C, const TailBwdArgs& a, hipStream_t s);

struct EmbedBwdArgs {
    const float* dx;
    const float* z;
    float* dz;
    const float *dww, *dwb, *w, *b, *lng;
    float *d_dww, *d_dwb, *d_lng, *d_lnb;
    float *d_w, *d_b;
    float* part;
    int HW;
    long total;
};
size_t embed_bwd_part_floats(int C);
int launch_embed_bwd(int C, const EmbedBwdArgs& a, hipStream_t s);

struct DownBwdArgs {
    const float* dy;
    float* du;
    const float* dskip;
    float* dx;
    const float* w;
    int B, H, W;
};
int launch_down_bwd_a(int E, const DownBwdArgs& a, hipStream_t s);
int launch_down_bwd_b(int E, const DownBwdArgs& a, hipStream_t s);

struct UpFuseBwdArgs {
    const float* dy;
    float* dt;
    float* dskip;
    float* v;
    float* dxb;
    float* tmp;
    const float *fw, *upw;
    int B, H, W;
};
int launch_upfuse_bwd_a(int E, const UpFuseBwdArgs& a, hipStream_t s);
int launch_upfuse_bwd_b(int E, const UpFuseBwdArgs& a, hipStream_t s);

struct FfnDwBwdArgs {
    const float* dy;
    const void* g3;
    const void* h2;
    void* dh2;
    int hbf;
    int pre;
    const float *w3t;
    const float* dww;
    float *slab_w, *slab_b;
    float *d_dww, *d_dwb;
    int B, h, w;
};
size_t ffn_dw_bwd_slab_floats(int e, int B, int h, int w);
int launch_ffn_dw_bwd(int e, const FfnDwBwdArgs& a, hipStream_t s);
struct Ffn1BwdArgs {
    const void* dh2;
    const void* g1;
    const float* x;
    const float* dy;
    void* dh1;
    float* y2;
    float* dx;
    const float *w2t, *w1t, *ln2g, *ln2b;
    float *d_ln2g, *d_ln2b;
    float* part;
    float *w1slab, *d_w1, *d_b1;
    float *w2slab, *d_w2, *d_b2;
    long P;
    int hbf;
    int pre;
    const float* w1;
    void* wsplit;
};
#define FFN1_BWD_WGS 512
inline bool ffn1_bwd_fuses_w1(int e) { return e <= 32; }
#ifndef LG_FW2
#define LG_FW2 0
#endif
inline bool ffn1_bwd_fuses_w2(int e, int pre) { return LG_FW2 && pre && e == 16; }
int launch_ffn1_bwd(int e, const Ffn1BwdArgs& a, hipStream_t s);
int launch_ffn1_bwd_x32(const Ffn1BwdArgs& a, const float* w1, void* wsplit, hipStream_t s);
struct Ffn1BwdXArgs {
    const void* dh2;
    int hbf;
    const float* x;
    const float* dy;
    float* dx;
    const float *w1, *b1;
    const float *w2t, *w1t;
    const float *ln2g, *ln2b;
    float* slab;
    float *d_w1, *d_b1, *d_w2, *d_b2, *d_ln2g, *d_ln2b;
    long P;
    const float* scales = nullptr;
};
inline int ffn1_bwd_x_wgs(int e) { return e == 16 ? 512 : 256; }
size_t ffn1_bwd_x_slab_floats(int e);
bool ffn1_bwd_x32_built();
int launch_ffn1_bwd_xs(int e, const Ffn1BwdXArgs& a, hipStream_t s);
struct FfnDwBwdXArgs {
    const float* dy;
    const void* h3;
    const void* h2;
    void* dh2;
    int hbf;
    const float* w3t;
    const float* dww;
    const float* dwb = nullptr;
    float* slab;
    float *d_dww, *d_dwb, *d_w3, *d_b3;
    int B, h, w;
    float* dh2_max = nullptr;
};
#define FFN_DW_BWD_X_WGS 512
#define FFN_DW_BWD_X_DB 576
#define FFN_DW_BWD_X_W3 640
#define FFN_DW_BWD_X_B3 1664
#define FFN_DW_BWD_X_ROW 1680
#define FFN_DW_BWD_X32_ROW 2720
inline size_t ffn_dw_bwd_x_slab_floats(int e) { return (size_t)FFN_DW_BWD_X_WGS * (e == 16 ? FFN_DW_BWD_X_ROW : FFN_DW_BWD_X32_ROW); }
int launch_ffn_dw_bwd_xs(int e, const FfnDwBwdXArgs& a, hipStream_t s);
#define FFN_DW_BWD_H_WGS 512
#define FFN_DW_BWD_H_ROW 848
inline size_t ffn_dw_bwd_h_slab_floats() { return (size_t)2 * FFN_DW_BWD_H_WGS * FFN_DW_BWD_H_ROW; }
int launch_ffn_dw_bwd_h(const FfnDwBwdXArgs& a, hipStream_t s);
int launch_transpose(const float* src, float* dst, int rows, int cols, hipStream_t s);
int launch_transpose3(const float* const* src, float* const* dst, const int* rows, const int* cols, int njobs, hipStream_t s);

struct ProjO2BwdArgs {
    const float* dy;
    float* do2;
    float* dym;
    const float* projw;
    int HW;
    long total;
    int dropout;
    uint64_t seed;
};
int launch_proj_o2_bwd(int e, const ProjO2BwdArgs& a, hipStream_t s);

struct FftBwdArgs {
    const float* do2;
    const float* sgn;
    const float* amp;
    const float* pha;
    float* dg;
    float* scratch;
    const float *ampw, *ampb, *phaw, *phab;
    float *d_ampw, *d_ampb, *d_phaw, *d_phab;
    float* part;
    int planes, ch, n;
    int h, w;
    int full = 0;
};
size_t fft_bwd_part_floats(int planes, int h, int w);
int launch_fftmix_bwd(const FftBwdArgs& a, hipStream_t s);

struct AttnBwdArgs {
    const float* x;
    const float* dy;
    const float* dym;
    const float* o2;
    const float* dg;
    float* dx;
    float* cat;
    float* y1;
    float* dqkv;
    const float* pos;
    const float* posT;
    float* dpos_slab;
    const float *ln1g, *ln1b, *qkvw, *qkvb, *projw;
    float *d_ln1g, *d_ln1b;
    float *d_qkvw, *d_qkvb;
    float* part;
    int B, h, w;
    const float* so = nullptr;
    const float* sl = nullptr;
    float* stats = nullptr;
    int core_m = 0;
};
int launch_attn_bwd_core_m(int e, const AttnBwdArgs& a, int grid, int nwin, int ngroups, hipStream_t s);
#ifndef LG_ATTN_FUSE_QKV
#define LG_ATTN_FUSE_QKV 1
#endif
constexpr bool attn_bwd_fuses_qkv(int e) { return LG_ATTN_FUSE_QKV && e == 16; }
inline size_t attn_bwd_part_floats(int e) { return (size_t)PIXEL_PART_WGS * 2 * e + (attn_bwd_fuses_qkv(e) ? (size_t)1024 * ((3 * e / 2) * (e / 2) + 3 * e / 2) : 0); }
int attn_bwd_grid(int e, int B, int h, int w);
int launch_attn_bwd(int e, const AttnBwdArgs& a, hipStream_t s);

struct ProjO2BwdKArgs {
    const float* dy;
    float* do2;
    uint32_t* keep;
    const float* projw;
    float* slab;
    float* d_projb;
    int HW;
    long total;
    uint64_t seed;
};
#ifndef PROJ_O2_K_WGS
#define PROJ_O2_K_WGS 512
#endif
int launch_proj_o2_bwd_k(int e, const ProjO2BwdKArgs& a, hipStream_t s);
struct AttnBwdFArgs {
    const float* x;
    const float* dy;
    const uint32_t* keep;
    const float* o2;
    const float* dg;
    float* dx;
    const float* pos;
    const float *ln1g, *ln1b, *qkvw, *qkvb, *projw;
    const float* so = nullptr;
    const float* sl = nullptr;
    float* slab;
    float *d_pos, *d_qkvw, *d_qkvb, *d_projw, *d_ln1g, *d_ln1b;
    int B, h, w;
    unsigned rcp_nwx, rcp_nwy;
};
#define ATTN_BWD_F_WGS 256
#define ATTN_BWD_F_WQ 8192
#define ATTN_BWD_F_ROW (8192 + 192 + 24 + 256 + 32)
inline bool attn_bwd_fused(int e) { return e == 16; }
int attn_bwd_f_grid(int B, int h, int w);
int launch_attn_bwd_f(int e, const AttnBwdFArgs& a, hipStream_t s);
```

lgteun_amd/csrc/common.h:

```cpp
#pragma once
#include <hip/hip_runtime.h>
#include <stdint.h>
#include <stddef.h>
#include <atomic>
#include "../../include/lgteun_hip.h"

enum SharedSlot { S_D1W, S_D1B, S_D3W, S_D3B, S_DT1W, S_DT1B, S_DT3W, S_DT3B, S_RW, S_RB, S_RTW, S_RTB, S_NSHARED };

enum BlockSlot {
    B_POS, B_QKVW, B_QKVB, B_AMPW, B_AMPB, B_PHAW, B_PHAB, B_PROJW, B_PROJB, B_LN1G, B_LN1B,
    B_W1, B_B1, B_W2, B_B2, B_DWW, B_DWB, B_W3, B_B3, B_LN2G, B_LN2B, B_NSLOT
};
enum LgtSlot {
    L_PE_DWW = 0, L_PE_DWB, L_PE_W, L_PE_B, L_PE_LNG, L_PE_LNB,
    L_ENC0 = 6, L_ENC1 = 27, L_DOWNW = 48, L_DOWNB, L_BOTT = 50, L_UPW = 71, L_UPB, L_FUSEW, L_FUSEB,
    L_DEC0 = 75, L_DEC1 = 96, L_TAILW = 117, L_TAILB, L_NSLOT = 119
};
static inline int block_base(int blk) {
    const int b[5] = {L_ENC0, L_ENC1, L_BOTT, L_DEC0, L_DEC1};
    return b[blk];
}

struct lg_plan {
    lg_config cfg;
    int n_offsets;
    int ffn_tile;
    int save_mode;
    int dwbwd_tile;
    bool hidden_bf16(int e) const { return cfg.precision == 1 && e != 64; }
    int attn_bwd_old;
    int ffn_bwd_bf16x3;
    int attn_bwd_core_m;
    int fft_full;
    int ffn_bf16x3;
    bool ffn_f16x2(int e) const { return cfg.precision == 0 && ffn_tile == 0 && !ffn_bf16x3 && (e == 16 || e == 32 || e == 64); }
    int attn_restats;
    int ffn_h3_re;
    bool ffn_h3_recompute(int e) const { return e == 16 && ffn_bwd_x(e) && cfg.precision == 0 && !dwbwd_tile && ffn_h3_re && !ffn_xs && ffn_f16x2(e); }
    int ffn_xs;
    int attn_bf16x3;
    bool attn_saves_stats(int e) const { return cfg.precision == 0 && !attn_fwd_valu && !attn_restats && !(e == 32 && attn_bwd_core_m); }
    bool attn_f16x2() const { return cfg.precision == 0 && !attn_bf16x3 && !attn_fwd_valu && ffn_tile == 0 && !ffn_bf16x3; }
    int attn_fwd_valu;
    int dstep_tiles;
    bool dstep_fused(int h, int w) const;
    int bwd32_old;
    bool ffn1_bwd_x32(int e) const { return e == 32 && ffn_tile == 0 && !bwd32_old; }
    bool ffn_dw_x32(int e, int h, int w) const { return e == 32 && ffn_tile == 0 && !dwbwd_tile && (h & 7) == 0 && (w & 15) == 0; }
    bool ffn_bwd_x(int e) const { return e == 16 && ffn_tile == 0 && save_mode == 2; }
    bool ffn_saves_preact(int e) const { return e == 16 && ffn_tile == 0 && (save_mode == 2 || (save_mode == 3 && cfg.precision == 0)); }
    int64_t* off;
    int64_t shared(int s) const { return off[s]; }
    int64_t eta(int i) const { return off[S_NSHARED + i]; }
    int64_t lgt(int stage, int slot) const { return off[S_NSHARED + cfg.K + stage * L_NSLOT + slot]; }
    int64_t blk(int stage, int b, int slot) const { return lgt(stage, block_base(b) + slot); }
};

void lg_set_error(const char* fmt, ...);

struct DeviceOnce {
    std::atomic<uint64_t> mask{0};
    static int dev() { int d = 0; (void)hipGetDevice(&d); return d & 63; }
    bool need() const { return !((mask.load(std::memory_order_acquire) >> dev()) & 1); }
    void done() { mask.fetch_or(1ull << dev(), std::memory_order_release); }
};

static inline uint64_t mix_seed(uint64_t seed, int stage, int blk) {
    uint64_t z = seed + 0x9E3779B97F4A7C15ull * (uint64_t)(stage * 8 + blk + 1);
    z = (z ^ (z >> 30)) * 0xBF58476D1CE4E5B9ull;
    z = (z ^ (z >> 27)) * 0x94D049BB133111EBull;
    return z ^ (z >> 31);
}


#define LG_CHECK_LAUNCH()                                                              \
    do {                                                                               \
        hipError_t e__ = hipGetLastError();                                            \
        if (e__ != hipSuccess) {                                                       \
            lg_set_error("%s:%d launch failed: %s", __FILE__, __LINE__, hipGetErrorString(e__)); \
            return (int)e__;                                                           \
        }                                                                              \
    } while (0)

#define LG_EPS 1e-5f

void lg_prof_begin(int kid, hipStream_t s);
void lg_prof_end(int kid, hipStream_t s);
struct ProfScope {
    int kid;
    hipStream_t s;
    ProfScope(int k, hipStream_t st) : kid(k), s(st) { lg_prof_begin(kid, s); }
    ~ProfScope() { lg_prof_end(kid, s); }
};

#ifdef __HIPCC__
__device__ __forceinline__ float erfc_abs_f(float az) {
    const float t = __builtin_amdgcn_rcpf(1.0f + 0.3275911f * az);
    const float poly = ((((1.061405429f * t - 1.453152027f) * t + 1.421413741f) * t - 0.284496736f) * t + 0.254829592f) * t;
    return poly * __expf(-az * az);
}
__device__ __forceinline__ float gelu_f(float x) {
    const float z = x * 0.70710678118654752440f;
    const float e = 0.5f * erfc_abs_f(fabsf(z));
    const float phi = z >= 0.f ? 1.0f - e : e;
    return x * phi;
}
__device__ __forceinline__ void gelu_both_f(float x, float& a, float& g) {
    const float az = fabsf(x) * 0.70710678118654752440f;
    const float t = __builtin_amdgcn_rcpf(1.0f + 0.3275911f * az);
    const float poly = ((((1.061405429f * t - 1.453152027f) * t + 1.421413741f) * t - 0.284496736f) * t + 0.254829592f) * t;
    const float ex = __expf(-az * az);
    const float e = 0.5f * poly * ex;
    const float cdf = x >= 0.f ? 1.0f - e : e;
    a = x * cdf;
    g = cdf + x * (0.39894228040143267794f * ex);
}
typedef float lg_v2f __attribute__((ext_vector_type(2)));
__device__ __forceinline__ lg_v2f gelu2_core(lg_v2f x, lg_v2f& absx, lg_v2f& ex) {
    absx = (lg_v2f){fabsf(x.x), fabsf(x.y)};
    const lg_v2f az = absx * 0.70710678118654752440f;
    const lg_v2f d = az * 0.3275911f + 1.0f;
    const lg_v2f t = (lg_v2f){__builtin_amdgcn_rcpf(d.x), __builtin_amdgcn_rcpf(d.y)};
    const lg_v2f poly = ((((1.061405429f * t - 1.453152027f) * t + 1.421413741f) * t - 0.284496736f) * t + 0.254829592f) * t;
    const lg_v2f m = az * az * -1.44269504088896340736f;
    ex = (lg_v2f){__builtin_amdgcn_exp2f(m.x), __builtin_amdgcn_exp2f(m.y)};
    return poly * ex * -0.5f + 0.5f;
}
__device__ __forceinline__ lg_v2f gelu2_f(lg_v2f x) {
    lg_v2f absx, ex;
    const lg_v2f sv = gelu2_core(x, absx, ex);
    return absx * sv + x * 0.5f;
}
__device__ __forceinline__ void gelu2_both_f(lg_v2f x, lg_v2f& a, lg_v2f& g) {
    lg_v2f absx, ex;
    const lg_v2f sv = gelu2_core(x, absx, ex);
    a = absx * sv + x * 0.5f;
    const lg_v2f cs = (lg_v2f){copysignf(sv.x, x.x), copysignf(sv.y, x.y)};
    g = x * (ex * 0.39894228040143267794f) + (cs + 0.5f);
}
__device__ __forceinline__ lg_v2f gelu2_scaled(lg_v2f x, float c1, float hr) {
    const lg_v2f absx = (lg_v2f){fabsf(x.x), fabsf(x.y)};
    const lg_v2f az = absx * c1;
    const lg_v2f d = az * 0.3275911f + 1.0f;
    const lg_v2f t = (lg_v2f){__builtin_amdgcn_rcpf(d.x), __builtin_amdgcn_rcpf(d.y)};
    const lg_v2f poly = ((((1.061405429f * t - 1.453152027f) * t + 1.421413741f) * t - 0.284496736f) * t + 0.254829592f) * t;
    const lg_v2f m = az * az * -1.44269504088896340736f;
    const lg_v2f ex = (lg_v2f){__builtin_amdgcn_exp2f(m.x), __builtin_amdgcn_exp2f(m.y)};
    const lg_v2f sv = poly * ex * (0.0f - hr) + hr;
    return absx * sv + x * hr;
}
struct GeluK { float k1, kd, hr, a1, a2, a3, a4, a5; };
__device__ __forceinline__ GeluK gelu_k(float c1, float hr) {
    GeluK k;
    k.k1 = c1 * 1.20112240878645f;
    k.kd = 0.3275911f / 1.20112240878645f;
    k.hr = hr;
    k.a1 = -hr * 0.254829592f; k.a2 = -hr * -0.284496736f; k.a3 = -hr * 1.421413741f; k.a4 = -hr * -1.453152027f; k.a5 = -hr * 1.061405429f;
    return k;
}
__device__ __forceinline__ lg_v2f gelu2_k(lg_v2f x, const GeluK& k) {
    const lg_v2f w = (lg_v2f){fabsf(x.x) * k.k1, fabsf(x.y) * k.k1};
    const lg_v2f d = w * k.kd + 1.0f;
    const lg_v2f t = (lg_v2f){__builtin_amdgcn_rcpf(d.x), __builtin_amdgcn_rcpf(d.y)};
    const lg_v2f ph = ((((k.a5 * t + k.a4) * t + k.a3) * t + k.a2) * t + k.a1) * t;
    const lg_v2f w2 = w * w;
    const lg_v2f ex = (lg_v2f){__builtin_amdgcn_exp2f(-w2.x), __builtin_amdgcn_exp2f(-w2.y)};
    const lg_v2f sv = ph * ex + k.hr;
    return (lg_v2f){__builtin_fmaf(fabsf(x.x), sv.x, x.x * k.hr), __builtin_fmaf(fabsf(x.y), sv.y, x.y * k.hr)};
}
__device__ __forceinline__ lg_v2f gelu2_fast_sig(lg_v2f x, lg_v2f& x2) {
    x2 = x * x;
    const lg_v2f v = x * (x2 * -0.1029432395800235f + -2.302208198144325f);
    const lg_v2f d = (lg_v2f){__builtin_amdgcn_exp2f(v.x), __builtin_amdgcn_exp2f(v.y)} + 1.0f;
    return (lg_v2f){__builtin_amdgcn_rcpf(d.x), __builtin_amdgcn_rcpf(d.y)};
}
template <bool FAST>
__device__ __forceinline__ lg_v2f gelu2_t(lg_v2f x) {
    if constexpr (FAST) {
        lg_v2f x2;
        return x * gelu2_fast_sig(x, x2);
    } else {
        return gelu2_f(x);
    }
}
template <bool FAST>
__device__ __forceinline__ void gelu2_both_t(lg_v2f x, lg_v2f& a, lg_v2f& g) {
    if constexpr (FAST) {
        lg_v2f x2;
        const lg_v2f sg = gelu2_fast_sig(x, x2);
        a = x * sg;
        g = a * (1.0f - sg) * (x2 * 0.21406444881780073f + 1.5957691216057308f) + sg;
    } else {
        gelu2_both_f(x, a, g);
    }
}
__device__ __forceinline__ float gelu_grad_f(float x) {
    const float z = x * 0.70710678118654752440f;
    const float e = 0.5f * erfc_abs_f(fabsf(z));
    const float cdf = z >= 0.f ? 1.0f - e : e;
    const float pdf = 0.39894228040143267794f * __expf(-0.5f * x * x);
    return cdf + x * pdf;
}
__device__ __forceinline__ int clampi(int v, int lo, int hi) { return v < lo ? lo : (v > hi ? hi : v); }

__device__ __forceinline__ void cubic_w(float t, float w[4]) {
    const float A = -0.75f;
    float x;
    x = t + 1.0f; w[0] = ((A * x - 5.0f * A) * x + 8.0f * A) * x - 4.0f * A;
    x = t;        w[1] = ((A + 2.0f) * x - (A + 3.0f)) * x * x + 1.0f;
    x = 1.0f - t; w[2] = ((A + 2.0f) * x - (A + 3.0f)) * x * x + 1.0f;
    x = 2.0f - t; w[3] = ((A * x - 5.0f * A) * x + 8.0f * A) * x - 4.0f * A;
}
template <int MODE>
__device__ __forceinline__ void resample_plan(int o, int& i0, float w[4]) {
    if (MODE == 0) { i0 = 2 * o; cubic_w(0.5f, w); }
    else if (MODE == 1) {
        int m = o >> 1;
        if (o & 1) { i0 = m; cubic_w(0.25f, w); } else { i0 = m - 1; cubic_w(0.75f, w); }
    } else {
        int m = o >> 2, r = o & 3;
        if (r == 0) { i0 = m - 1; cubic_w(0.625f, w); }
        else if (r == 1) { i0 = m - 1; cubic_w(0.875f, w); }
        else if (r == 2) { i0 = m; cubic_w(0.125f, w); }
        else { i0 = m; cubic_w(0.375f, w); }
    }
}
template <int MODE>
__device__ __forceinline__ float resample_at(const float* __restrict__ p, int hi, int wi, int oy, int ox) {
    int iy0, ix0;
    float wy[4], wx[4];
    resample_plan<MODE>(oy, iy0, wy);
    resample_plan<MODE>(ox, ix0, wx);
    float acc = 0.f;
#pragma unroll
    for (int a = 0; a < 4; ++a) {
        int yy = clampi(iy0 - 1 + a, 0, hi - 1);
        float r = 0.f;
#pragma unroll
        for (int b = 0; b < 4; ++b) r += wx[b] * p[yy * wi + clampi(ix0 - 1 + b, 0, wi - 1)];
        acc += wy[a] * r;
    }
    return acc;
}

template <int E>
__device__ __forceinline__ void ln_stats(const float (&x)[E], float& mu, float& rstd) {
    float s = 0.f;
#pragma unroll
    for (int i = 0; i < E; ++i) s += x[i];
    mu = s * (1.0f / E);
    float v = 0.f;
#pragma unroll
    for (int i = 0; i < E; ++i) { float d = x[i] - mu; v += d * d; }
    rstd = __builtin_amdgcn_rsqf(v * (1.0f / E) + LG_EPS);
}

template <int N>
__device__ __forceinline__ float lane_group_sum(float v) {
    static_assert(N == 4 || N == 8 || N == 16, "group of 4, 8 or 16 lanes");
    v += __builtin_bit_cast(float, __builtin_amdgcn_mov_dpp(__builtin_bit_cast(int, v), 0xB1, 0xF, 0xF, true));
    v += __builtin_bit_cast(float, __builtin_amdgcn_mov_dpp(__builtin_bit_cast(int, v), 0x4E, 0xF, 0xF, true));
    if (N >= 8) v += __shfl_xor(v, 4);
    if (N >= 16) v += __shfl_xor(v, 8);
    return v;
}
#define LG_DROP_T16 6554u
__device__ __forceinline__ uint32_t dropout_hash(uint64_t seed, uint64_t pair) {
    uint32_t x = (uint32_t)pair + (uint32_t)seed;
    x ^= x >> 16; x *= 0x7feb352du;
    x ^= (uint32_t)(seed >> 32) ^ (uint32_t)(pair >> 32);
    x ^= x >> 15; x *= 0x846ca68bu;
    x ^= x >> 16;
    return x;
}
__device__ __forceinline__ float dropout_scale(uint64_t seed, uint64_t idx) {
    const uint32_t x = dropout_hash(seed, idx >> 1);
    return ((idx & 1) ? (x >> 16) : (x & 0xffffu)) < LG_DROP_T16 ? 0.0f : (1.0f / 0.9f);
}
__device__ __forceinline__ void dropout_scale2(uint64_t seed, uint64_t idx_even, float& s0, float& s1) {
    const uint32_t x = dropout_hash(seed, idx_even >> 1);
    s0 = (x & 0xffffu) < LG_DROP_T16 ? 0.0f : (1.0f / 0.9f);
    s1 = (x >> 16) < LG_DROP_T16 ? 0.0f : (1.0f / 0.9f);
}
__device__ __forceinline__ void lds_stage(float* dst, const float* __restrict__ src, int n) {
    for (int i = threadIdx.x; i < n; i += blockDim.x) dst[i] = src[i];
}
template <int NT, int N>
__device__ __forceinline__ void lds_stage_ld(float (&v)[(N + NT - 1) / NT], const float* __restrict__ src) {
#pragma unroll
    for (int k = 0; k < (N + NT - 1) / NT; ++k) { const int i = k * NT + (int)threadIdx.x; v[k] = src[i < N ? i : N - 1]; }
}
template <int NT, int N>
__device__ __forceinline__ void lds_stage_st(float* dst, const float (&v)[(N + NT - 1) / NT]) {
#pragma unroll
    for (int k = 0; k < (N + NT - 1) / NT; ++k) { const int i = k * NT + (int)threadIdx.x; if (i < N) dst[i] = v[k]; }
}
#endif
```

lgteun_amd/csrc/k_bwd.hip:

```cpp
#include <string.h>

#include "kernels.h"
#include "bwd_kernels.h"
#include "backward.h"

struct BwdBufs {
    float *dzA, *dzB, *gu3, *gs1, *gu1, *gr, *gd3, *gt1, *gd1;
    float *dx[3];
    float *dh2, *dh1, *y2, *do2, *dg, *dym, *cat, *y1, *dqkv, *dpos_slab;
    float *w3t[5], *w2t[5], *w1t[5], *wsp, *dt, *dskip, *v, *du, *fft_scratch;
    float* slab_arena;
    float* attn_stats;
    float* ffn_scales;
    size_t slab_cap;
    ReduceQueue rq;
    size_t bytes;
};

static void carve_bwd(const lg_plan* plan, int B, void* base, BwdBufs& bb) {
    const lg_config& c = plan->cfg;
    Carver cv{reinterpret_cast<char*>(base), 0};
    const size_t P0 = (size_t)c.H * c.W * B, P1 = P0 / 4, E = 4 * (size_t)c.C, C = c.C;
    bb.dzA = cv.take(C * P0); bb.dzB = cv.take(C * P0); bb.gu3 = cv.take(C * P0);
    bb.gs1 = cv.take(C * P1); bb.gu1 = cv.take(C * P1); bb.gt1 = cv.take(C * P1); bb.gd1 = cv.take(C * P1);
    bb.gr = cv.take(C * P1 / 4); bb.gd3 = cv.take(C * P1 / 4);
    for (int i = 0; i < 3; ++i) bb.dx[i] = cv.take(P0 * E);
    bb.dh2 = cv.take(P0 * 4 * E); bb.dh1 = cv.take(P0 * 4 * E);
    bb.y2 = cv.take(P0 * E); bb.do2 = cv.take(P0 * E / 2); bb.dg = cv.take(P0 * E / 2);
    bb.dym = cv.take(P0 * E); bb.cat = cv.take(P0 * E); bb.y1 = cv.take(P0 * 16 > P0 * E / 2 ? P0 * 16 : P0 * E / 2);
    bb.dqkv = cv.take(P0 * 2 * E);
    bb.attn_stats = cv.take(P0 * 8);
    bb.dpos_slab = cv.take((size_t)ATTN_BWD_F_WGS * ATTN_BWD_F_ROW > (size_t)512 * 2 * 64 * 64 ? (size_t)ATTN_BWD_F_WGS * ATTN_BWD_F_ROW : (size_t)512 * 2 * 64 * 64);
    for (int j = 0; j < 5; ++j) { bb.w3t[j] = cv.take(8 * E * 2 * E); bb.w2t[j] = cv.take(8 * E * 8 * E); bb.w1t[j] = cv.take(8 * E * 2 * E); }
    bb.wsp = cv.take(ffn_wsplit_bytes(32) / sizeof(float));
    size_t sl = wgrad_slab_floats((int)(8 * E), (int)(8 * E), (long)P0);
    size_t sl2 = wgrad_slab_floats(64, 64, (long)P0);
    size_t sl3 = ffn_dw_bwd_slab_floats((int)E, B, c.H, c.W);
    if (sl2 > sl) sl = sl2;
    size_t sl4 = chan_partial_floats(c.C, B, c.H, c.W);
    const size_t sl5 = (size_t)PIXEL_PART_WGS * (2 * 8 * c.C + 2 * c.C);
    if (sl5 > sl4) sl4 = sl5;
    if (sl4 > sl) sl = sl4;
    if (sl3 > sl) sl = sl3;
    for (size_t e = E; e <= 2 * E; e *= 2)
        if ((e == 16 && plan->ffn_bwd_x(16)) || (e == 32 && plan->ffn1_bwd_x32(32))) {
            if (ffn1_bwd_x_slab_floats((int)e) > sl) sl = ffn1_bwd_x_slab_floats((int)e);
        }
    if (ffn_dw_bwd_x_slab_floats(16) > sl) sl = ffn_dw_bwd_x_slab_floats(16);
    if (ffn_dw_bwd_x_slab_floats(32) > sl) sl = ffn_dw_bwd_x_slab_floats(32);
    if (ffn_dw_bwd_h_slab_floats() > sl) sl = ffn_dw_bwd_h_slab_floats();
    bb.slab_cap = 4 * sl;
    bb.slab_arena = cv.take(bb.slab_cap);
    bb.ffn_scales = nullptr;
    bb.dt = cv.take(P0 * E); bb.dskip = cv.take(P0 * E); bb.v = cv.take(P1 * E); bb.du = cv.take(P1 * E);
    bb.bytes = cv.off;
}

size_t bwd_workspace_bytes(const lg_plan* plan, int B) {
    BwdBufs bb;
    carve_bwd(plan, B, nullptr, bb);
    return bb.bytes;
}

#define RC(x) do { int rc__ = (x); if (rc__) return rc__; } while (0)

struct ReduceQueueScope {
    explicit ReduceQueueScope(BwdBufs& bb, hipStream_t s) {
        bb.rq.init(bb.slab_arena, bb.slab_cap, s);
        reduce_queue_begin(&bb.rq);
    }
    ~ReduceQueueScope() { (void)reduce_queue_end(); }
};

static int wgrad(const void* Y, int ldy, const void* X, int ldx, float* dW, int ldw, float* db, long P, int N, int K, int nv, int kv,
                 int ybf, int xbf, BwdBufs& bb, hipStream_t s, int xgelu = 0) {
    float* slab = bb.rq.take(wgrad_slab_floats(N, K, P));
    if (!slab) return -3;
    WgradArgs a;
    a.Y = Y; a.X = X; a.dW = dW; a.db = db; a.P = P; a.ldy = ldy; a.ldx = ldx; a.ldw = ldw; a.N = N; a.K = K;
    a.n_valid = nv; a.k_valid = kv; a.ybf = ybf; a.xbf = xbf; a.xgelu = xgelu;
    return launch_wgrad(a, slab, s);
}

static int ffn_transposes(const lg_plan* pl, const float* P, int st, int j0, int j1, const NetBufs& nb, BwdBufs& bb, hipStream_t s) {
    const float* tsrc[15];
    float* tdst[15];
    int trows[15], tcols[15], n = 0;
    for (int j = j0; j < j1; ++j) {
        const int e = nb.blk[j].e, n1 = 4 * e;
        tsrc[n] = P + pl->blk(st, j, B_W3); tdst[n] = bb.w3t[j]; trows[n] = e; tcols[n] = n1; ++n;
        tsrc[n] = P + pl->blk(st, j, B_W2); tdst[n] = bb.w2t[j]; trows[n] = n1; tcols[n] = n1; ++n;
        tsrc[n] = P + pl->blk(st, j, B_W1); tdst[n] = bb.w1t[j]; trows[n] = n1; tcols[n] = e; ++n;
    }
    return launch_transpose3(tsrc, tdst, trows, tcols, n, s);
}

static int ffn_half_bwd(const lg_plan* pl, const float* P, float* G, int st, int j, const BlockBufs& fb, BwdBufs& bb, const float* dy,
                        float* tmp, int B, hipStream_t s) {
    const int e = fb.e, n1 = 4 * e;
    const int hbf = pl->hidden_bf16(e) ? 1 : 0;
    const int pre = pl->ffn_saves_preact(e) ? 1 : 0;
    const long Pn = (long)B * fb.h * fb.w;
    if (pl->ffn_bwd_x(e) && (!pl->dwbwd_tile || hbf)) {
        FfnDwBwdXArgs fk;
        const bool h3re = pl->ffn_h3_recompute(e) && (fb.h & 7) == 0 && (fb.w & 15) == 0;
        fk.dy = dy; fk.h3 = h3re ? nullptr : fb.a3; fk.h2 = fb.h2; fk.dh2 = bb.dh2; fk.w3t = bb.w3t[j]; fk.dww = P + pl->blk(st, j, B_DWW); fk.dwb = P + pl->blk(st, j, B_DWB);
        fk.slab = bb.rq.take(h3re ? ffn_dw_bwd_h_slab_floats() : ffn_dw_bwd_x_slab_floats(e));
        if (!fk.slab) return -3;
        fk.d_dww = G + pl->blk(st, j, B_DWW); fk.d_dwb = G + pl->blk(st, j, B_DWB); fk.d_w3 = G + pl->blk(st, j, B_W3); fk.d_b3 = G + pl->blk(st, j, B_B3);
        fk.B = B; fk.h = fb.h; fk.w = fb.w; fk.hbf = hbf;
        float* fsc = (bb.ffn_scales && pl->ffn_f16x2(e) && !pl->ffn_bwd_bf16x3 && !hbf) ? bb.ffn_scales + ((size_t)st * 5 + j) * 8 : nullptr;
        fk.dh2_max = fsc ? fsc + 6 : nullptr;
        RC(h3re ? launch_ffn_dw_bwd_h(fk, s) : launch_ffn_dw_bwd_xs(e, fk, s));
        Ffn1BwdXArgs fx;
        fx.scales = fsc;
        fx.dh2 = bb.dh2; fx.x = fb.xmid; fx.dy = dy; fx.dx = tmp;
        fx.w1 = P + pl->blk(st, j, B_W1); fx.b1 = P + pl->blk(st, j, B_B1); fx.w2t = bb.w2t[j]; fx.w1t = bb.w1t[j];
        fx.ln2g = P + pl->blk(st, j, B_LN2G); fx.ln2b = P + pl->blk(st, j, B_LN2B);
        fx.slab = bb.rq.take(ffn1_bwd_x_slab_floats(e));
        if (!fx.slab) return -3;
        fx.d_w1 = G + pl->blk(st, j, B_W1); fx.d_b1 = G + pl->blk(st, j, B_B1); fx.d_w2 = G + pl->blk(st, j, B_W2); fx.d_b2 = G + pl->blk(st, j, B_B2);
        fx.d_ln2g = G + pl->blk(st, j, B_LN2G); fx.d_ln2b = G + pl->blk(st, j, B_LN2B);
        fx.P = Pn; fx.hbf = hbf;
        return launch_ffn1_bwd_xs(e, fx, s);
    }
    const bool dwx32 = pl->ffn_dw_x32(e, fb.h, fb.w);
    float* fsc2 = nullptr;
    if (dwx32) {
        FfnDwBwdXArgs fk;
        fk.dy = dy; fk.h3 = fb.a3; fk.h2 = fb.h2; fk.dh2 = bb.dh2; fk.w3t = bb.w3t[j]; fk.dww = P + pl->blk(st, j, B_DWW);
        fk.slab = bb.rq.take(ffn_dw_bwd_x_slab_floats(e));
        if (!fk.slab) return -3;
        fk.d_dww = G + pl->blk(st, j, B_DWW); fk.d_dwb = G + pl->blk(st, j, B_DWB); fk.d_w3 = G + pl->blk(st, j, B_W3); fk.d_b3 = G + pl->blk(st, j, B_B3);
        fk.B = B; fk.h = fb.h; fk.w = fb.w; fk.hbf = hbf;
        fsc2 = (bb.ffn_scales && pl->ffn_f16x2(e) && !pl->ffn_bwd_bf16x3 && !hbf && pl->ffn1_bwd_x32(e)) ? bb.ffn_scales + ((size_t)st * 5 + j) * 8 : nullptr;
        fk.dh2_max = fsc2 ? fsc2 + 6 : nullptr;
        RC(launch_ffn_dw_bwd_xs(e, fk, s));
    }
    if (!dwx32) {
        FfnDwBwdArgs fd;
        fd.dy = dy; fd.g3 = pre ? fb.a3 : fb.g3; fd.h2 = fb.h2; fd.dh2 = bb.dh2; fd.w3t = bb.w3t[j]; fd.dww = P + pl->blk(st, j, B_DWW);
        fd.slab_w = bb.rq.take(ffn_dw_bwd_slab_floats(e, B, fb.h, fb.w));
        if (!fd.slab_w) return -3;
        fd.slab_b = fd.slab_w + ffn_dw_bwd_slab_floats(e, B, fb.h, fb.w) / 10 * 9;
        fd.d_dww = G + pl->blk(st, j, B_DWW); fd.d_dwb = G + pl->blk(st, j, B_DWB);
        fd.B = B; fd.h = fb.h; fd.w = fb.w; fd.hbf = hbf; fd.pre = pre;
        RC(launch_ffn_dw_bwd(e, fd, s));
    }
    if (pl->ffn_bwd_x(e) || pl->ffn1_bwd_x32(e)) {
        Ffn1BwdXArgs fx;
        fx.scales = fsc2;
        fx.dh2 = bb.dh2; fx.x = fb.xmid; fx.dy = dy; fx.dx = tmp;
        fx.w1 = P + pl->blk(st, j, B_W1); fx.b1 = P + pl->blk(st, j, B_B1); fx.w2t = bb.w2t[j]; fx.w1t = bb.w1t[j];
        fx.ln2g = P + pl->blk(st, j, B_LN2G); fx.ln2b = P + pl->blk(st, j, B_LN2B);
        fx.slab = bb.rq.take(ffn1_bwd_x_slab_floats(e));
        if (!fx.slab) return -3;
        fx.d_w1 = G + pl->blk(st, j, B_W1); fx.d_b1 = G + pl->blk(st, j, B_B1); fx.d_w2 = G + pl->blk(st, j, B_W2); fx.d_b2 = G + pl->blk(st, j, B_B2);
        fx.d_ln2g = G + pl->blk(st, j, B_LN2G); fx.d_ln2b = G + pl->blk(st, j, B_LN2B);
        fx.P = Pn; fx.hbf = hbf;
        RC(launch_ffn1_bwd_xs(e, fx, s));
        if (dwx32) return 0;
        return wgrad(dy, e, fb.a3, n1, G + pl->blk(st, j, B_W3), n1, G + pl->blk(st, j, B_B3), Pn, e, n1, e, n1, 0, hbf, bb, s, pre);
    }
    Ffn1BwdArgs f1;
    f1.dh2 = bb.dh2; f1.g1 = pre ? fb.a1 : fb.g1; f1.x = fb.xmid; f1.dy = dy; f1.dh1 = bb.dh1; f1.y2 = bb.y2; f1.dx = tmp;
    f1.w2t = bb.w2t[j]; f1.w1t = bb.w1t[j];
    f1.ln2g = P + pl->blk(st, j, B_LN2G); f1.ln2b = P + pl->blk(st, j, B_LN2B);
    f1.d_ln2g = G + pl->blk(st, j, B_LN2G); f1.d_ln2b = G + pl->blk(st, j, B_LN2B); f1.part = bb.rq.take((size_t)PIXEL_PART_WGS * 2 * e);
    if (!f1.part) return -3;
    f1.P = Pn; f1.hbf = hbf; f1.pre = pre;
    f1.w1 = nullptr; f1.wsplit = nullptr;
    if (e == 32 && pl->ffn_tile == 0) { f1.w1 = P + pl->blk(st, j, B_W1); f1.wsplit = bb.wsp; }
    f1.w1slab = nullptr; f1.d_w1 = nullptr; f1.d_b1 = nullptr;
    if (ffn1_bwd_fuses_w1(e)) {
        f1.w1slab = bb.rq.take((size_t)FFN1_BWD_WGS * ((size_t)n1 * e + n1));
        if (!f1.w1slab) return -3;
        f1.d_w1 = G + pl->blk(st, j, B_W1); f1.d_b1 = G + pl->blk(st, j, B_B1);
    }
    f1.w2slab = nullptr; f1.d_w2 = nullptr; f1.d_b2 = nullptr;
    if (ffn1_bwd_fuses_w2(e, pre)) {
        f1.w2slab = bb.rq.take((size_t)FFN1_BWD_WGS * ((size_t)n1 * n1 + n1));
        if (!f1.w2slab) return -3;
        f1.d_w2 = G + pl->blk(st, j, B_W2); f1.d_b2 = G + pl->blk(st, j, B_B2);
    }
    RC(launch_ffn1_bwd(e, f1, s));
    if (!ffn1_bwd_fuses_w2(e, pre))
        RC(wgrad(bb.dh2, n1, fb.a1, n1, G + pl->blk(st, j, B_W2), n1, G + pl->blk(st, j, B_B2), Pn, n1, n1, n1, n1, hbf, hbf, bb, s, pre));
    if (!ffn1_bwd_fuses_w1(e))
        RC(wgrad(bb.dh1, n1, bb.y2, e, G + pl->blk(st, j, B_W1), e, G + pl->blk(st, j, B_B1), Pn, n1, e, n1, e, hbf, 0, bb, s));
    if (!dwx32) RC(wgrad(dy, e, fb.a3, n1, G + pl->blk(st, j, B_W3), n1, G + pl->blk(st, j, B_B3), Pn, e, n1, e, n1, 0, hbf, bb, s, pre));
    return 0;
}

static int fft_bwd_call(const lg_plan* pl, const float* P, float* G, int st, int j, const BlockBufs& fb, const float* do2, float* dg,
                        int B, hipStream_t s, float* fft_scratch, float* part) {
    const int hc = fb.e / 2;
    FftBwdArgs fa;
    fa.do2 = do2; fa.sgn = fb.sgn; fa.amp = fb.amp; fa.pha = fb.pha; fa.dg = dg; fa.scratch = fft_scratch;
    fa.ampw = P + pl->blk(st, j, B_AMPW); fa.ampb = P + pl->blk(st, j, B_AMPB);
    fa.phaw = P + pl->blk(st, j, B_PHAW); fa.phab = P + pl->blk(st, j, B_PHAB);
    fa.d_ampw = G + pl->blk(st, j, B_AMPW); fa.d_ampb = G + pl->blk(st, j, B_AMPB);
    fa.d_phaw = G + pl->blk(st, j, B_PHAW); fa.d_phab = G + pl->blk(st, j, B_PHAB);
    fa.ch = hc; fa.planes = B * hc; fa.n = fb.h; fa.h = fb.h; fa.w = fb.w; fa.part = part; fa.full = pl->fft_full;
    return launch_fftmix_bwd(fa, s);
}

static int mixer_half_bwd(const lg_plan* pl, const float* P, float* G, int st, int j, const BlockBufs& fb, BwdBufs& bb, const float* posT,
                          const float* tmp, float* dx_out, int B, int flags, uint64_t seed, hipStream_t s) {
    const int e = fb.e, hc = e / 2;
    const long Pn = (long)B * fb.h * fb.w;
    const int drop = (flags & LG_FLAG_DROPOUT) ? 1 : 0;
    if (attn_bwd_fused(e) && !pl->attn_bwd_old) {
        uint32_t* keep = drop ? reinterpret_cast<uint32_t*>(bb.dym) : nullptr;
        ProjO2BwdKArgs pk;
        pk.dy = tmp; pk.do2 = bb.do2; pk.keep = keep; pk.projw = P + pl->blk(st, j, B_PROJW);
        pk.slab = bb.rq.take((size_t)PROJ_O2_K_WGS * e);
        if (!pk.slab) return -3;
        pk.d_projb = G + pl->blk(st, j, B_PROJB); pk.HW = fb.h * fb.w; pk.total = Pn; pk.seed = mix_seed(seed, st, j);
        RC(launch_proj_o2_bwd_k(e, pk, s));
        float* fpart = bb.rq.take(fft_bwd_part_floats(B * hc, fb.h, fb.w));
        if (!fpart) return -3;
        RC(fft_bwd_call(pl, P, G, st, j, fb, bb.do2, bb.dg, B, s, bb.fft_scratch, fpart));
        AttnBwdFArgs af;
        af.x = fb.xin; af.dy = tmp; af.keep = keep; af.o2 = fb.o2; af.dg = bb.dg; af.dx = dx_out;
        af.pos = P + pl->blk(st, j, B_POS);
        af.ln1g = P + pl->blk(st, j, B_LN1G); af.ln1b = P + pl->blk(st, j, B_LN1B);
        af.qkvw = P + pl->blk(st, j, B_QKVW); af.qkvb = P + pl->blk(st, j, B_QKVB); af.projw = P + pl->blk(st, j, B_PROJW);
        af.slab = bb.dpos_slab;
        af.d_pos = G + pl->blk(st, j, B_POS); af.d_qkvw = G + pl->blk(st, j, B_QKVW); af.d_qkvb = G + pl->blk(st, j, B_QKVB);
        af.d_projw = G + pl->blk(st, j, B_PROJW); af.d_ln1g = G + pl->blk(st, j, B_LN1G); af.d_ln1b = G + pl->blk(st, j, B_LN1B);
        af.B = B; af.h = fb.h; af.w = fb.w;
        if (pl->attn_saves_stats(e)) { af.so = fb.att_o; af.sl = fb.att_l; }
        return launch_attn_bwd_f(e, af, s);
    }
    ProjO2BwdArgs po;
    po.dy = tmp; po.do2 = bb.do2; po.dym = drop ? bb.dym : nullptr; po.projw = P + pl->blk(st, j, B_PROJW);
    po.HW = fb.h * fb.w; po.total = Pn; po.dropout = drop; po.seed = mix_seed(seed, st, j);
    RC(launch_proj_o2_bwd(e, po, s));
    const float* dym = drop ? bb.dym : tmp;
    float* fpart = bb.rq.take(fft_bwd_part_floats(B * hc, fb.h, fb.w));
    if (!fpart) return -3;
    RC(fft_bwd_call(pl, P, G, st, j, fb, bb.do2, bb.dg, B, s, bb.fft_scratch, fpart));
    AttnBwdArgs at;
    at.x = fb.xin; at.dy = tmp; at.dym = dym; at.o2 = fb.o2; at.dg = bb.dg; at.dx = dx_out;
    at.cat = bb.cat; at.y1 = bb.y1; at.dqkv = bb.dqkv;
    at.pos = P + pl->blk(st, j, B_POS); at.posT = posT; at.dpos_slab = bb.dpos_slab;
    at.ln1g = P + pl->blk(st, j, B_LN1G); at.ln1b = P + pl->blk(st, j, B_LN1B);
    at.qkvw = P + pl->blk(st, j, B_QKVW); at.qkvb = P + pl->blk(st, j, B_QKVB); at.projw = P + pl->blk(st, j, B_PROJW);
    at.d_ln1g = G + pl->blk(st, j, B_LN1G); at.d_ln1b = G + pl->blk(st, j, B_LN1B); at.part = bb.rq.take(attn_bwd_part_floats(e));
    at.d_qkvw = G + pl->blk(st, j, B_QKVW); at.d_qkvb = G + pl->blk(st, j, B_QKVB);
    if (attn_bwd_fuses_qkv(e)) at.y1 = nullptr;
    if (!at.part) return -3;
    at.B = B; at.h = fb.h; at.w = fb.w; at.core_m = pl->attn_bwd_core_m; at.stats = bb.attn_stats;
    if (pl->attn_saves_stats(e) && !(e == 32 && pl->attn_bwd_core_m)) { at.so = fb.att_o; at.sl = fb.att_l; }
    RC(launch_attn_bwd(e, at, s));
    const int grid = attn_bwd_grid(e, B, fb.h, fb.w);
    RC(launch_reduce_slab(bb.dpos_slab, grid, 1, 2 * 64 * 64, G + pl->blk(st, j, B_POS), 2 * 64 * 64, 1, 2 * 64 * 64, s));
    RC(wgrad(dym, e, bb.cat, e, G + pl->blk(st, j, B_PROJW), e, G + pl->blk(st, j, B_PROJB), Pn, e, e, e, e, 0, 0, bb, s));
    if (!attn_bwd_fuses_qkv(e)) {
        const int y1ld = (hc + 15) / 16 * 16, dqld = (3 * hc + 15) / 16 * 16;
        RC(wgrad(bb.dqkv, dqld, bb.y1, y1ld, G + pl->blk(st, j, B_QKVW), hc, G + pl->blk(st, j, B_QKVB), Pn, dqld, y1ld, 3 * hc, hc, 0, 0,
                 bb, s));
    }
    return 0;
}

static int block_bwd(const lg_plan* pl, const float* P, float* G, int st, int j, const BlockBufs& fb, BwdBufs& bb, const float* posT,
                     const float* dy, float* tmp, float* dx_out, int B, int flags, uint64_t seed, hipStream_t s) {
    RC(ffn_half_bwd(pl, P, G, st, j, fb, bb, dy, tmp, B, s));
    RC(mixer_half_bwd(pl, P, G, st, j, fb, bb, posT, tmp, dx_out, B, flags, seed, s));
    return bb.rq.flush();
}

int op_block_bwd(const lg_plan* pl, const float* P, float* G, int st, int j, int which, const float* dy, float* dx, NetBufs& nb,
                 void* bwd_ws, int B, hipStream_t s) {
    BwdBufs bb;
    carve_bwd(pl, B, bwd_ws, bb);
    bb.fft_scratch = nb.fft_scratch;
    bb.ffn_scales = nb.ffn_scales;
    const BlockBufs& fb = nb.blk[j];
    if (which == 0) return fft_bwd_call(pl, P, G, st, j, fb, dy, dx, B, s, nb.fft_scratch, bb.slab_arena);
    ReduceQueueScope rqs(bb, s);
    int rc = which == 1 ? 0 : ffn_transposes(pl, P, st, j, j + 1, nb, bb, s);
    if (!rc) rc = which == 1 ? mixer_half_bwd(pl, P, G, st, j, fb, bb, nb.posT, dy, dx, B, 0, 0, s)
                             : ffn_half_bwd(pl, P, G, st, j, fb, bb, dy, dx, B, s);
    const int rc2 = reduce_queue_end();
    return rc ? rc : rc2;
}

static int data_step_bwd(const lg_plan* pl, const float* P, float* G, int st, const NetBufs& nb, BwdBufs& bb, const float* zin,
                         const float* pan, const float* g, float* dz, int B, hipStream_t s) {
    const lg_config& c = pl->cfg;
    const int planes = B * c.C, H = c.H, W = c.W;
    if (pl->dstep_fused(H, W)) {
        DstepBwdArgs a;
        a.g = g; a.z = zin; a.pan = pan; a.t1 = nb.t1[st]; a.r = nb.r[st]; a.s1 = nb.s1[st]; a.dz = dz;
        a.d1w = P + pl->shared(S_D1W); a.d3w = P + pl->shared(S_D3W); a.dt1w = P + pl->shared(S_DT1W); a.dt3w = P + pl->shared(S_DT3W);
        a.dt3b = P + pl->shared(S_DT3B);
        a.rw = P + pl->shared(S_RW); a.rb = P + pl->shared(S_RB); a.rtw = P + pl->shared(S_RTW); a.rtb = P + pl->shared(S_RTB);
        a.eta = P + pl->eta(st);
        a.B = B; a.C = c.C; a.N = H;
        float* part = bb.rq.take(dstep_bwd_part_floats(c.C, B, H));
        if (!part) return -3;
        const size_t bc = (size_t)B * c.C;
        a.part_top = part; a.part_dt1 = part + 14 * bc; a.part_d3 = part + 24 * bc; a.part_d1 = part + 34 * bc; a.part_pre = part + 44 * bc;
        DstepBwdGrads gg;
        gg.d1w = G + pl->shared(S_D1W); gg.d1b = G + pl->shared(S_D1B); gg.d3w = G + pl->shared(S_D3W); gg.d3b = G + pl->shared(S_D3B);
        gg.dt1w = G + pl->shared(S_DT1W); gg.dt1b = G + pl->shared(S_DT1B); gg.dt3w = G + pl->shared(S_DT3W); gg.dt3b = G + pl->shared(S_DT3B);
        gg.rw = G + pl->shared(S_RW); gg.rb = G + pl->shared(S_RB); gg.rtw = G + pl->shared(S_RTW); gg.rtb = G + pl->shared(S_RTB);
        gg.eta = G + pl->eta(st);
        RC(launch_dstep_bwd(a, gg, s));
        return bb.rq.flush();
    }
    DstepTopArgs t;
    t.g = g; t.s1 = nb.s1[st]; t.z = zin; t.pan = pan; t.gu = bb.gu3; t.dz = dz;
    t.w9 = P + pl->shared(S_DT3W); t.b9 = P + pl->shared(S_DT3B);
    t.rw = P + pl->shared(S_RW); t.rb = P + pl->shared(S_RB); t.rtw = P + pl->shared(S_RTW); t.rtb = P + pl->shared(S_RTB);
    t.eta = P + pl->eta(st);
    t.dw9 = G + pl->shared(S_DT3W); t.dbias = G + pl->shared(S_DT3B);
    t.drw = G + pl->shared(S_RW); t.drb = G + pl->shared(S_RB); t.drtw = G + pl->shared(S_RTW); t.drtb = G + pl->shared(S_RTB);
    t.deta = G + pl->eta(st);
    t.C = c.C; t.B = B; t.H = H; t.W = W; t.part = bb.rq.take(chan_partial_floats(c.C, B, H, W));
    if (!t.part) return -3;
    RC(launch_dstep_top_bwd(t, s));
    RC(launch_resample_adj(1, bb.gu3, bb.gs1, planes, H / 2, W / 2, 0, s));
    DwBwdArgs d;
    d.C = c.C; d.planes = planes;
    d.gout = bb.gs1; d.in = nb.r[st]; d.gin = bb.gu1; d.w9 = P + pl->shared(S_DT1W);
    d.dw9 = G + pl->shared(S_DT1W); d.dbias = G + pl->shared(S_DT1B);
    d.hi = H / 4; d.wi = W / 4; d.n_h = H / 2; d.n_w = W / 2;
    d.part = bb.rq.take(chan_partial_floats(c.C, B, H, W));
    if (!d.part) return -3;
    RC(launch_dw_bwd(1, d, s));
    RC(launch_resample_adj(1, bb.gu1, bb.gr, planes, H / 4, W / 4, 0, s));
    d.gout = bb.gr; d.in = nb.t1[st]; d.gin = bb.gd3; d.w9 = P + pl->shared(S_D3W);
    d.dw9 = G + pl->shared(S_D3W); d.dbias = G + pl->shared(S_D3B);
    d.hi = H / 2; d.wi = W / 2; d.n_h = H / 4; d.n_w = W / 4;
    d.part = bb.rq.take(chan_partial_floats(c.C, B, H, W));
    if (!d.part) return -3;
    RC(launch_dw_bwd(0, d, s));
    RC(launch_resample_adj(0, bb.gd3, bb.gt1, planes, H / 2, W / 2, 0, s));
    d.gout = bb.gt1; d.in = zin; d.gin = bb.gd1; d.w9 = P + pl->shared(S_D1W);
    d.dw9 = G + pl->shared(S_D1W); d.dbias = G + pl->shared(S_D1B);
    d.hi = H; d.wi = W; d.n_h = H / 2; d.n_w = W / 2;
    d.part = bb.rq.take(chan_partial_floats(c.C, B, H, W));
    if (!d.part) return -3;
    RC(launch_dw_bwd(0, d, s));
    RC(launch_resample_adj(0, bb.gd1, dz, planes, H, W, 1, s));
    return bb.rq.flush();
}

static int lgt_bwd(const lg_plan* pl, const float* P, float* G, int st, const NetBufs& nb, BwdBufs& bb, const float* dout,
                   const float* zin, int B, int flags, uint64_t seed, hipStream_t s) {
    const lg_config& c = pl->cfg;
    const int E = 4 * c.C;
    const long P0 = (long)B * c.H * c.W, P1 = P0 / 4;
    const float* posT = nb.posT + (size_t)st * 5 * 2 * 64 * 64;
    float *A = bb.dx[0], *Bf = bb.dx[1], *Cf = bb.dx[2];
    RC(ffn_transposes(pl, P, st, 0, 5, nb, bb, s));
    TailBwdArgs tb;
    tb.dout = dout; tb.x = nb.blk[4].xout; tb.dx = A; tb.dz = bb.dzA; tb.w = P + pl->lgt(st, L_TAILW);
    tb.d_w = G + pl->lgt(st, L_TAILW); tb.d_b = G + pl->lgt(st, L_TAILB);
    tb.HW = c.H * c.W; tb.total = P0; tb.part = bb.rq.take(tail_bwd_part_floats(c.C));
    if (!tb.part) return -3;
    RC(launch_tail_bwd(c.C, tb, s));
    RC(block_bwd(pl, P, G, st, 4, nb.blk[4], bb, posT + 4 * 8192, A, Bf, Cf, B, flags, seed, s));
    RC(block_bwd(pl, P, G, st, 3, nb.blk[3], bb, posT + 3 * 8192, Cf, Bf, A, B, flags, seed, s));
    UpFuseBwdArgs ub;
    ub.dy = A; ub.dt = bb.dt; ub.dskip = bb.dskip; ub.v = bb.v; ub.dxb = Bf; ub.tmp = Cf;
    ub.fw = P + pl->lgt(st, L_FUSEW); ub.upw = P + pl->lgt(st, L_UPW);
    ub.B = B; ub.H = c.H; ub.W = c.W;
    RC(launch_upfuse_bwd_a(E, ub, s));
    RC(wgrad(A, E, nb.t_up, E, G + pl->lgt(st, L_FUSEW), 2 * E, G + pl->lgt(st, L_FUSEB), P0, E, E, E, E, 0, 0, bb, s));
    RC(wgrad(A, E, nb.blk[1].xout, E, G + pl->lgt(st, L_FUSEW) + E, 2 * E, nullptr, P0, E, E, E, E, 0, 0, bb, s));
    RC(launch_upfuse_bwd_b(E, ub, s));
    RC(wgrad(bb.v, E, nb.blk[2].xout, 2 * E, G + pl->lgt(st, L_UPW), 2 * E, G + pl->lgt(st, L_UPB), P1, E, 2 * E, E, 2 * E, 0, 0, bb, s));
    RC(block_bwd(pl, P, G, st, 2, nb.blk[2], bb, posT + 2 * 8192, Bf, Cf, A, B, flags, seed, s));
    DownBwdArgs db;
    db.dy = A; db.du = bb.du; db.dskip = bb.dskip; db.dx = Bf; db.w = P + pl->lgt(st, L_DOWNW);
    db.B = B; db.H = c.H; db.W = c.W;
    RC(launch_down_bwd_a(E, db, s));
    RC(wgrad(A, 2 * E, nb.u_down, E, G + pl->lgt(st, L_DOWNW), E, G + pl->lgt(st, L_DOWNB), P1, 2 * E, E, 2 * E, E, 0, 0, bb, s));
    RC(launch_down_bwd_b(E, db, s));
    RC(block_bwd(pl, P, G, st, 1, nb.blk[1], bb, posT + 1 * 8192, Bf, Cf, A, B, flags, seed, s));
    RC(block_bwd(pl, P, G, st, 0, nb.blk[0], bb, posT + 0 * 8192, A, Bf, Cf, B, flags, seed, s));
    EmbedBwdArgs eb;
    eb.dx = Cf; eb.z = zin; eb.dz = bb.dzA;
    eb.dww = P + pl->lgt(st, L_PE_DWW); eb.dwb = P + pl->lgt(st, L_PE_DWB); eb.w = P + pl->lgt(st, L_PE_W); eb.b = P + pl->lgt(st, L_PE_B);
    eb.lng = P + pl->lgt(st, L_PE_LNG);
    eb.d_dww = G + pl->lgt(st, L_PE_DWW); eb.d_dwb = G + pl->lgt(st, L_PE_DWB);
    eb.d_lng = G + pl->lgt(st, L_PE_LNG); eb.d_lnb = G + pl->lgt(st, L_PE_LNB);
    eb.d_w = G + pl->lgt(st, L_PE_W); eb.d_b = G + pl->lgt(st, L_PE_B);
    eb.HW = c.H * c.W; eb.total = P0; eb.part = bb.rq.take(embed_bwd_part_floats(c.C));
    if (!eb.part) return -3;
    RC(launch_embed_bwd(c.C, eb, s));
    return 0;
}

int op_data_step_bwd(const lg_plan* pl, const float* P, float* G, int st, NetBufs& nb, void* bwd_ws, const float* z_in, const float* pan,
                     const float* g, float* dz, int B, hipStream_t s) {
    BwdBufs bb;
    carve_bwd(pl, B, bwd_ws, bb);
    ReduceQueueScope rqs(bb, s);
    const int rc = data_step_bwd(pl, P, G, st, nb, bb, z_in, pan, g, dz, B, s);
    const int rc2 = reduce_queue_end();
    return rc ? rc : rc2;
}

int op_lgt_bwd(const lg_plan* pl, const float* P, float* G, int st, NetBufs& nb, void* bwd_ws, const float* z, const float* dout, float* dz,
               int B, int flags, uint64_t seed, hipStream_t s) {
    BwdBufs bb;
    carve_bwd(pl, B, bwd_ws, bb);
    bb.fft_scratch = nb.fft_scratch;
    bb.ffn_scales = nb.ffn_scales;
    bb.dzA = dz;
    ReduceQueueScope rqs(bb, s);
    const int rc = lgt_bwd(pl, P, G, st, nb, bb, dout, z, B, flags, seed, s);
    const int rc2 = reduce_queue_end();
    return rc ? rc : rc2;
}

int net_backward(const lg_plan* pl, const float* P, float* G, const float* ms, const float* pan, const float* dout, NetBufs& nb,
                 void* bwd_ws, int B, int flags, uint64_t seed, hipStream_t s) {
    (void)ms;
    const lg_config& c = pl->cfg;
    BwdBufs bb;
    carve_bwd(pl, B, bwd_ws, bb);
    bb.fft_scratch = nb.fft_scratch;
    bb.ffn_scales = nb.ffn_scales;
    ReduceQueueScope rqs(bb, s);
    if (flags & LG_FLAG_CHAINED) {
        const float* g = dout;
        for (int i = c.K - 1; i >= 0; --i) {
            const NetBufs sv = stage_view(nb, i);
            RC(lgt_bwd(pl, P, G, i, sv, bb, g, nb.Z[i + 1], B, flags, seed, s));
            RC(data_step_bwd(pl, P, G, i, nb, bb, nb.X[i], pan, bb.dzA, bb.dzB, B, s));
            g = bb.dzB;
        }
        return reduce_queue_end();
    }
    const bool do_lgt = !(flags & (LG_FLAG_BWD_LGT | LG_FLAG_BWD_DATA)) || (flags & LG_FLAG_BWD_LGT);
    const bool do_data = !(flags & (LG_FLAG_BWD_LGT | LG_FLAG_BWD_DATA)) || (flags & LG_FLAG_BWD_DATA);
    if (do_lgt) RC(lgt_bwd(pl, P, G, c.K - 1, nb, bb, dout, nb.Z[c.K], B, flags, seed, s));
    if (!do_data) return reduce_queue_end();
    float* g = bb.dzA;
    float* dz = bb.dzB;
    for (int i = c.K - 1; i >= 0; --i) {
        RC(data_step_bwd(pl, P, G, i, nb, bb, nb.Z[i], pan, g, dz, B, s));
        float* t = g; g = dz; dz = t;
    }
    return reduce_queue_end();
}
```

lgteun_amd/csrc/k_wgrad.hip:

```cpp
#include "kernels.h"
#include "bwd_kernels.h"
#include "hstore.h"

typedef float f32x4 __attribute__((ext_vector_type(4)));


#ifndef LG_WGRAD_VEC_U
#define LG_WGRAD_VEC_U 4
#endif
#ifndef LG_WGRAD_WGS
#define LG_WGRAD_WGS 512
#endif
#ifndef LG_WGRAD_INTERLEAVE
#define LG_WGRAD_INTERLEAVE 1
#endif
__host__ __device__ constexpr int wgrad_batch(int nt, int kt, bool vec) { return vec ? LG_WGRAD_VEC_U : (nt + kt <= 2 ? 16 : (nt + kt <= 4 ? 8 : 4)); }

template <int NT, int KT, bool VEC, bool YBF, bool XBF, bool XGELU = false>
__global__ __launch_bounds__(256) void k_wgrad_t(WgradArgs a, int k_blocks, long px_per_wave, float* slab, float* bslab) {
    constexpr int U = wgrad_batch(NT, KT, VEC);
    constexpr int NB = 16 * NT, KB = 16 * KT;
    const int wave = threadIdx.x >> 6, lane = threadIdx.x & 63, r = lane & 15, g = lane >> 4;
    const int nb = blockIdx.y / k_blocks, kb = blockIdx.y - nb * k_blocks;
    const int n0 = nb * NB, k0 = kb * KB;
    const long slice = (long)blockIdx.x * 4 + wave;
#if LG_WGRAD_INTERLEAVE
    const long p_stride = (long)gridDim.x * 4 * (4 * U);
    const long p_begin = slice * (4 * U);
    const long p_end = a.P;
#else
    const long p_stride = 4 * U;
    const long p_begin = slice * px_per_wave;
    long p_end = p_begin + px_per_wave;
    if (p_end > a.P) p_end = a.P;
#endif
    f32x4 acc[NT][KT];
    float bsum[NT];
#pragma unroll
    for (int i = 0; i < NT; ++i) {
        bsum[i] = 0.f;
#pragma unroll
        for (int j = 0; j < KT; ++j) acc[i][j] = (f32x4){0.f, 0.f, 0.f, 0.f};
    }
    int ycol[NT], xcol[KT];
    bool yok[NT], xok[KT];
#pragma unroll
    for (int t = 0; t < NT; ++t) { const int c = n0 + t * 16 + r; yok[t] = c < a.n_valid; ycol[t] = yok[t] ? c : 0; }
#pragma unroll
    for (int t = 0; t < KT; ++t) { const int c = k0 + t * 16 + r; xok[t] = c < a.k_valid; xcol[t] = xok[t] ? c : 0; }
    float ym[NT], xm[KT];
#pragma unroll
    for (int t = 0; t < NT; ++t) ym[t] = yok[t] ? 1.f : 0.f;
#pragma unroll
    for (int t = 0; t < KT; ++t) xm[t] = xok[t] ? 1.f : 0.f;
    auto fetch = [&](long p, float (&y)[U][NT], float (&x)[U][KT]) {
#pragma unroll
        for (int u = 0; u < U; ++u) {
            const long row = p + 4 * u + g;
            const long rc = row < p_end ? row : p_begin;
            if (VEC) {
                const float4 yv = HS<YBF>::ld4(a.Y, rc * a.ldy + n0 + 4 * r);
                const float4 xv = HS<XBF>::ld4(a.X, rc * a.ldx + k0 + 4 * r);
                const float yy[4] = {yv.x, yv.y, yv.z, yv.w}, xx[4] = {xv.x, xv.y, xv.z, xv.w};
#pragma unroll
                for (int t = 0; t < NT; ++t) y[u][t] = yy[t & 3];
#pragma unroll
                for (int t = 0; t < KT; ++t) x[u][t] = xx[t & 3];
            } else {
#pragma unroll
                for (int t = 0; t < NT; ++t) y[u][t] = HS<YBF>::ld1(a.Y, rc * a.ldy + ycol[t]);
#pragma unroll
                for (int t = 0; t < KT; ++t) x[u][t] = HS<XBF>::ld1(a.X, rc * a.ldx + xcol[t]);
            }
        }
    };
    if (p_begin < p_end) {
        float yc[U][NT], xc[U][KT];
        fetch(p_begin, yc, xc);
#pragma unroll 1
        for (long p = p_begin; p < p_end; p += p_stride) {
            float yn[U][NT], xn[U][KT];
            fetch(p + p_stride, yn, xn);
            __builtin_amdgcn_sched_barrier(0);
#pragma unroll
            for (int u = 0; u < U; ++u) {
                const float rm = (p + 4 * u + g) < p_end ? 1.f : 0.f;
                float yv[NT], xv[KT];
#pragma unroll
                for (int i = 0; i < NT; ++i) { yv[i] = yc[u][i] * (VEC ? rm : rm * ym[i]); bsum[i] += yv[i]; }
                if constexpr (XGELU && KT % 2 == 0) {
#pragma unroll
                    for (int j = 0; j < KT; j += 2) {
                        const lg_v2f gp = gelu2_f((lg_v2f){xc[u][j], xc[u][j + 1]});
                        xv[j] = VEC ? gp.x : gp.x * xm[j];
                        xv[j + 1] = VEC ? gp.y : gp.y * xm[j + 1];
                    }
                } else {
#pragma unroll
                    for (int j = 0; j < KT; ++j) {
                        const float xg = XGELU ? gelu_f(xc[u][j]) : xc[u][j];
                        xv[j] = VEC ? xg : xg * xm[j];
                    }
                }
#pragma unroll
                for (int i = 0; i < NT; ++i)
#pragma unroll
                    for (int j = 0; j < KT; ++j) acc[i][j] = __builtin_amdgcn_mfma_f32_16x16x4f32(yv[i], xv[j], acc[i][j], 0, 0, 0);
            }
            __builtin_amdgcn_sched_barrier(0);
#pragma unroll
            for (int u = 0; u < U; ++u) {
#pragma unroll
                for (int i = 0; i < NT; ++i) yc[u][i] = yn[u][i];
#pragma unroll
                for (int j = 0; j < KT; ++j) xc[u][j] = xn[u][j];
            }
        }
    }
    __shared__ float red[NB * KB + NB];
    for (int w = 0; w < 4; ++w) {
        if (wave == w) {
#pragma unroll
            for (int i = 0; i < NT; ++i)
#pragma unroll
                for (int j = 0; j < KT; ++j)
#pragma unroll
                    for (int v = 0; v < 4; ++v) {
                        const int idx = VEC ? (4 * (4 * g + v) + i) * KB + 4 * r + j : (i * 16 + 4 * g + v) * KB + j * 16 + r;
                        red[idx] = (w == 0 ? 0.f : red[idx]) + acc[i][j][v];
                    }
#pragma unroll
            for (int i = 0; i < NT; ++i) {
                float sv = bsum[i];
                sv += __shfl_xor(sv, 16);
                sv += __shfl_xor(sv, 32);
                const int idx = NB * KB + (VEC ? 4 * r + i : i * 16 + r);
                if (g == 0) red[idx] = (w == 0 ? 0.f : red[idx]) + sv;
            }
        }
        __syncthreads();
    }
    float* my = slab + (long)blockIdx.x * ((long)a.N * a.K);
    for (int i = threadIdx.x; i < NB * KB; i += 256) {
        const int rr = i / KB, cc = i - rr * KB;
        my[(long)(n0 + rr) * a.K + k0 + cc] = red[i];
    }
    if (a.db && kb == 0 && threadIdx.x < NB) bslab[(long)blockIdx.x * a.N + n0 + threadIdx.x] = red[NB * KB + threadIdx.x];
}

__global__ __launch_bounds__(256) void k_reduce_slab(const float* __restrict__ slab, long nslices, int rows, int cols, float* dst,
                                                     int ld, int rows_valid, int cols_valid, const float* __restrict__ slab2, int n2,
                                                     float* dst2, int n2_valid) {
    __shared__ float part[16][17];
    if (blockIdx.y == 1) { slab = slab2; rows = 1; cols = n2; dst = dst2; ld = n2; rows_valid = 1; cols_valid = n2_valid; }
    const long n = (long)rows * cols;
    const int o = threadIdx.x & 15, ph = threadIdx.x >> 4;
    const long i = blockIdx.x * 16L + o;
    float sv[8];
#pragma unroll
    for (int u = 0; u < 8; ++u) sv[u] = 0.f;
    if (i < n) {
        long k = ph;
        for (; k + 16 * 7 < nslices; k += 16 * 8) {
#pragma unroll
            for (int u = 0; u < 8; ++u) sv[u] += slab[(k + 16 * u) * n + i];
        }
        for (; k < nslices; k += 16) sv[0] += slab[k * n + i];
    }
    part[ph][o] = ((sv[0] + sv[1]) + (sv[2] + sv[3])) + ((sv[4] + sv[5]) + (sv[6] + sv[7]));
    __syncthreads();
    if (ph == 0 && i < n) {
        const int row = (int)(i / cols), col = (int)(i - (long)row * cols);
        if (row < rows_valid && col < cols_valid) {
            float t = 0.f;
#pragma unroll
            for (int q = 0; q < 16; ++q) t += part[q][o];
            dst[(long)row * ld + col] += t;
        }
    }
}

__global__ __launch_bounds__(256) void k_reduce_jobs(ReduceJobTable t) {
    __shared__ float4 part[16][17];
    const ReduceJob& jb = t.j[blockIdx.y];
    const long n = (long)jb.rows * jb.cols;
    const int o = threadIdx.x & 15, ph = threadIdx.x >> 4;
    const bool v4 = ((jb.cols | jb.row_stride | jb.ld) & 3) == 0 && (jb.slice_stride & 3) == 0 && jb.rows_valid == jb.rows && jb.cols_valid == jb.cols &&
                    ((reinterpret_cast<uintptr_t>(jb.slab) | reinterpret_cast<uintptr_t>(jb.dst) | reinterpret_cast<uintptr_t>(jb.dst2)) & 15) == 0;
    if (v4) {
        const long n4 = n >> 2;
        if (blockIdx.x * 16L >= n4) return;
        const long i4 = blockIdx.x * 16L + o;
        const long i = i4 << 2;
        const int row = (int)(i / jb.cols), col = (int)(i - (long)row * jb.cols);
        float4 sv[8];
#pragma unroll
        for (int u = 0; u < 8; ++u) sv[u] = make_float4(0.f, 0.f, 0.f, 0.f);
        if (i4 < n4) {
            const float* __restrict__ src = jb.slab + (long)row * jb.row_stride + col;
            const long ss = jb.slice_stride, ns = jb.nslices;
            long k = ph;
            for (; k + 16 * 7 < ns; k += 16 * 8) {
                float4 ld[8];
#pragma unroll
                for (int u = 0; u < 8; ++u) ld[u] = *reinterpret_cast<const float4*>(src + (k + 16 * u) * ss);
#pragma unroll
                for (int u = 0; u < 8; ++u) { sv[u].x += ld[u].x; sv[u].y += ld[u].y; sv[u].z += ld[u].z; sv[u].w += ld[u].w; }
            }
            for (; k < ns; k += 16) {
                const float4 l = *reinterpret_cast<const float4*>(src + k * ss);
                sv[0].x += l.x; sv[0].y += l.y; sv[0].z += l.z; sv[0].w += l.w;
            }
        }
        auto add4 = [](const float4& a, const float4& b) { return make_float4(a.x + b.x, a.y + b.y, a.z + b.z, a.w + b.w); };
        part[ph][o] = add4(add4(add4(sv[0], sv[1]), add4(sv[2], sv[3])), add4(add4(sv[4], sv[5]), add4(sv[6], sv[7])));
        __syncthreads();
        if (ph == 0 && i4 < n4) {
            float4 ts = make_float4(0.f, 0.f, 0.f, 0.f);
#pragma unroll
            for (int q = 0; q < 16; ++q) ts = add4(ts, part[q][o]);
            float4* d = reinterpret_cast<float4*>(jb.dst + (long)row * jb.ld + col);
            *d = add4(*d, ts);
            if (jb.dst2) {
                float4* d2 = reinterpret_cast<float4*>(jb.dst2 + (long)row * jb.ld + col);
                *d2 = add4(*d2, ts);
            }
        }
        return;
    }
    if (blockIdx.x * 16L >= n) return;
    const long i = blockIdx.x * 16L + o;
    const int row = (int)(i / jb.cols), col = (int)(i - (long)row * jb.cols);
    float sv[8];
#pragma unroll
    for (int u = 0; u < 8; ++u) sv[u] = 0.f;
    if (i < n) {
        const float* __restrict__ src = jb.slab + (long)row * jb.row_stride + col;
        const long ss = jb.slice_stride, ns = jb.nslices;
        long k = ph;
        for (; k + 16 * 7 < ns; k += 16 * 8) {
#pragma unroll
            for (int u = 0; u < 8; ++u) sv[u] += src[(k + 16 * u) * ss];
        }
        for (; k < ns; k += 16) sv[0] += src[k * ss];
    }
    float* parts = reinterpret_cast<float*>(part);
    parts[ph * 17 + o] = ((sv[0] + sv[1]) + (sv[2] + sv[3])) + ((sv[4] + sv[5]) + (sv[6] + sv[7]));
    __syncthreads();
    if (ph == 0 && i < n && row < jb.rows_valid && col < jb.cols_valid) {
        float tsum = 0.f;
#pragma unroll
        for (int q = 0; q < 16; ++q) tsum += parts[q * 17 + o];
        jb.dst[(long)row * jb.ld + col] += tsum;
        if (jb.dst2) jb.dst2[(long)row * jb.ld + col] += tsum;
    }
}

static thread_local ReduceQueue* tl_rq = nullptr;
void reduce_queue_begin(ReduceQueue* q) { tl_rq = q; }
int reduce_queue_end() {
    ReduceQueue* q = tl_rq;
    tl_rq = nullptr;
    return q ? q->flush() : 0;
}
int ReduceQueue::flush() {
    off = 0;
    if (tab.n == 0) return 0;
    long nmax = 0;
    for (int k = 0; k < tab.n; ++k) {
        const long n = (long)tab.j[k].rows * tab.j[k].cols;
        if (n > nmax) nmax = n;
    }
    dim3 grid((unsigned)((nmax + 15) / 16), (unsigned)tab.n);
#ifdef LG_RQ_DEBUG
    fprintf(stderr, "[rq] flush: %d jobs, grid.x %u:", tab.n, grid.x);
    for (int k = 0; k < tab.n; ++k) fprintf(stderr, " (%ld sl x %d x %d)", tab.j[k].nslices, tab.j[k].rows, tab.j[k].cols);
    fprintf(stderr, "\n");
#endif
    k_reduce_jobs<<<grid, 256, 0, stream>>>(tab);
    tab.n = 0;
    LG_CHECK_LAUNCH();
    return 0;
}
int ReduceQueue::push(const ReduceJob& j) {
    if (tab.n == LG_MAX_REDUCE_JOBS) {
        const size_t keep = off;
        int rc = flush();
        off = keep;
        if (rc) return rc;
    }
    tab.j[tab.n++] = j;
    return 0;
}
float* ReduceQueue::take(size_t nfloats) {
    nfloats = (nfloats + 63) & ~(size_t)63;
    if (nfloats > cap) { lg_set_error("reduce queue: slab of %zu floats exceeds the arena (%zu)", nfloats, cap); return nullptr; }
    if (off + nfloats > cap && flush()) return nullptr;
    float* p = arena + off;
    off += nfloats;
    return p;
}

static int launch_reduce_slab2(const float* slab, long nslices, int rows, int cols, float* dst, int ld, int rows_valid, int cols_valid,
                               const float* slab2, int n2, float* dst2, int n2_valid, hipStream_t s) {
    if (tl_rq) {
        ReduceJob j;
        j.slab = slab; j.dst = dst; j.dst2 = nullptr; j.nslices = nslices; j.slice_stride = (long)rows * cols;
        j.rows = rows; j.cols = cols; j.row_stride = cols; j.ld = ld; j.rows_valid = rows_valid; j.cols_valid = cols_valid;
        int rc = tl_rq->push(j);
        if (rc || !slab2) return rc;
        j.slab = slab2; j.dst = dst2; j.slice_stride = n2; j.rows = 1; j.cols = n2; j.row_stride = n2; j.ld = n2; j.rows_valid = 1;
        j.cols_valid = n2_valid;
        return tl_rq->push(j);
    }
    long n = (long)rows * cols;
    dim3 grid((unsigned)((n + 15) / 16), slab2 ? 2 : 1);
    k_reduce_slab<<<grid, 256, 0, s>>>(slab, nslices, rows, cols, dst, ld, rows_valid, cols_valid, slab2, n2, dst2, n2_valid);
    LG_CHECK_LAUNCH();
    return 0;
}
int launch_reduce_job(const ReduceJob& j, hipStream_t s) {
    if (tl_rq) return tl_rq->push(j);
    ReduceJobTable t;
    t.j[0] = j;
    t.n = 1;
    const long n = (long)j.rows * j.cols;
    k_reduce_jobs<<<dim3((unsigned)((n + 15) / 16), 1), 256, 0, s>>>(t);
    LG_CHECK_LAUNCH();
    return 0;
}
bool reduce_chan_enqueue(const float* part, const ChanReduce& m, int* rc) {
    if (!tl_rq) return false;
    *rc = 0;
    for (int k = 0; k < m.NK && !*rc; ++k) {
        ReduceJob j;
        j.slab = part + k; j.dst = m.dst[k]; j.dst2 = m.dst2[k]; j.cols = 1; j.cols_valid = 1;
        if ((m.allc_mask >> k) & 1u) {
            j.nslices = (long)m.nslices * m.C; j.slice_stride = m.NK; j.rows = 1; j.row_stride = 0; j.ld = 1; j.rows_valid = 1;
        } else {
            j.nslices = m.nslices; j.slice_stride = (long)m.C * m.NK; j.rows = m.C; j.row_stride = m.NK; j.ld = m.stride[k]; j.rows_valid = m.C;
        }
        *rc = tl_rq->push(j);
    }
    return true;
}
int launch_reduce_slab_wb(const float* wslab, const float* bslab, long nslices, int rows, int cols, float* dW, int ld, float* db, hipStream_t s) {
    return launch_reduce_slab2(wslab, nslices, rows, cols, dW, ld, rows, cols, bslab, rows, db, rows, s);
}
int launch_reduce_slab_pair(const float* slab_a, const float* slab_b, long nslices, int n, float* dst_a, float* dst_b, hipStream_t s) {
    return launch_reduce_slab2(slab_a, nslices, 1, n, dst_a, n, 1, n, slab_b, n, dst_b, n, s);
}
int launch_reduce_slab(const float* slab, long nslices, int rows, int cols, float* dst, int ld, int rows_valid, int cols_valid,
                       hipStream_t s) {
    return launch_reduce_slab2(slab, nslices, rows, cols, dst, ld, rows_valid, cols_valid, nullptr, 0, nullptr, 0, s);
}

static int tiles_per_block(int n16) {
    for (int t = 4; t > 1; --t) if (n16 % t == 0) return t;
    return 1;
}
static long wgrad_splits(int N, int K) {
    const int blocks = (N / 16 / tiles_per_block(N / 16)) * (K / 16 / tiles_per_block(K / 16));
    long splits = LG_WGRAD_WGS / blocks;
    return splits < 1 ? 1 : splits;
}
size_t wgrad_slab_floats(int N, int K, long P) {
    (void)P;
    return (size_t)wgrad_splits(N, K) * ((size_t)N * K + N);
}

template <int NT, int KT, bool VEC>
static void wgrad_dispatch_bf(const WgradArgs& a, dim3 grid, int k_blocks, long px, float* slab, float* bslab, hipStream_t s) {
    if constexpr (KT == 4) {
        if (a.xgelu) { k_wgrad_t<NT, KT, VEC, false, false, true><<<grid, 256, 0, s>>>(a, k_blocks, px, slab, bslab); return; }
    }
    if (a.ybf && a.xbf) k_wgrad_t<NT, KT, VEC, true, true><<<grid, 256, 0, s>>>(a, k_blocks, px, slab, bslab);
    else if (a.ybf) k_wgrad_t<NT, KT, VEC, true, false><<<grid, 256, 0, s>>>(a, k_blocks, px, slab, bslab);
    else if (a.xbf) k_wgrad_t<NT, KT, VEC, false, true><<<grid, 256, 0, s>>>(a, k_blocks, px, slab, bslab);
    else k_wgrad_t<NT, KT, VEC, false, false><<<grid, 256, 0, s>>>(a, k_blocks, px, slab, bslab);
}
template <int NT>
static void wgrad_dispatch_kt(int KT, const WgradArgs& a, dim3 grid, int k_blocks, long px, float* slab, float* bslab, hipStream_t s) {
    switch (KT) {
        case 1: wgrad_dispatch_bf<NT, 1, false>(a, grid, k_blocks, px, slab, bslab, s); break;
        case 2: wgrad_dispatch_bf<NT, 2, false>(a, grid, k_blocks, px, slab, bslab, s); break;
        case 3: wgrad_dispatch_bf<NT, 3, false>(a, grid, k_blocks, px, slab, bslab, s); break;
        default: wgrad_dispatch_bf<NT, 4, false>(a, grid, k_blocks, px, slab, bslab, s); break;
    }
}

int launch_wgrad(const WgradArgs& a, float* slab, hipStream_t s) {
    ProfScope prof__(LG_K_WGRAD, s);
    if ((a.N & 15) || (a.K & 15) || a.N <= 0 || a.K <= 0 || a.P <= 0) { lg_set_error("wgrad: N,K must be positive multiples of 16"); return -2; }
    if (a.n_valid > a.N || a.k_valid > a.K || a.n_valid > a.ldy || a.k_valid > a.ldx) { lg_set_error("wgrad: valid extents exceed the operands"); return -2; }
    const int NT = tiles_per_block(a.N / 16), KT = tiles_per_block(a.K / 16);
    if (a.xgelu && (KT != 4 || a.ybf || a.xbf)) { lg_set_error("wgrad: gelu(X) operands need fp32 storage and K a multiple of 64"); return -2; }
    const int n_blocks = a.N / (16 * NT), k_blocks = a.K / (16 * KT);
    const int blocks = n_blocks * k_blocks;
    long splits = wgrad_splits(a.N, a.K);
    long nslices = splits * 4;
    long px = (a.P + nslices - 1) / nslices;
    const bool vec = NT == 4 && KT == 4 && a.n_valid == a.N && a.k_valid == a.K && (a.ldy & 3) == 0 && (a.ldx & 3) == 0;
    const long batch = 4L * wgrad_batch(NT, KT, vec);
    px = (px + batch - 1) / batch * batch;
    nslices = (a.P + px - 1) / px;
    splits = (nslices + 3) / 4;
    float* bslab = slab + splits * (long)a.N * a.K;
    dim3 grid((unsigned)splits, (unsigned)blocks);
    if (vec) wgrad_dispatch_bf<4, 4, true>(a, grid, k_blocks, px, slab, bslab, s);
    else switch (NT) {
        case 1: wgrad_dispatch_kt<1>(KT, a, grid, k_blocks, px, slab, bslab, s); break;
        case 2: wgrad_dispatch_kt<2>(KT, a, grid, k_blocks, px, slab, bslab, s); break;
        case 3: wgrad_dispatch_kt<3>(KT, a, grid, k_blocks, px, slab, bslab, s); break;
        default: wgrad_dispatch_kt<4>(KT, a, grid, k_blocks, px, slab, bslab, s); break;
    }
    LG_CHECK_LAUNCH();
    return launch_reduce_slab2(slab, splits, a.N, a.K, a.dW, a.ldw, a.n_valid, a.k_valid, a.db ? bslab : nullptr, a.N, a.db, a.n_valid, s);
}
```

Before: 6149 image-pairs/sec.

## Batch gradient slab reductions across blocks into one cached job-table launch

Weight-gradient slab reductions used to be flushed at the end of every block. They now accumulate in a larger queue (up to 512 jobs) across a whole LGT stage and its data step, with a bigger slab arena that also holds the attention dpos slabs. On flush, jobs that add into the same gradient are chained together, and each gets a workgroup count sized to its own work instead of the maximum. The job table is cached on the device by hash, so repeated steps launch without re-uploading it. This aims to cut reduce-kernel launches and wasted workgroups, at the cost of a larger workspace, host-side hashing and chaining work, and a device synchronize on a cache miss. The old per-block behaviour remains available behind an environment flag.

```diff
diff --git a/include/lgteun_hip.h b/include/lgteun_hip.h
--- a/include/lgteun_hip.h
+++ b/include/lgteun_hip.h
@@ -55,7 +55,8 @@
 #define LG_VAR_ATTN_BF16X3 (1u << 14)
 #define LG_VAR_FFN_H3_RECOMPUTE (1u << 15)
 #define LG_VAR_ATTN_BWD_RESTATS (1u << 16)
-#define LG_VAR_ALL 0x1ffffu
+#define LG_VAR_REDUCE_PER_BLOCK (1u << 17)
+#define LG_VAR_ALL 0x3ffffu
 
 typedef struct lg_plan lg_plan;
 
diff --git a/lgteun_amd/_lib.py b/lgteun_amd/_lib.py
--- a/lgteun_amd/_lib.py
+++ b/lgteun_amd/_lib.py
@@ -33,6 +33,7 @@
 LG_VAR_ATTN_BF16X3 = 1 << 14
 LG_VAR_FFN_H3_RECOMPUTE = 1 << 15
 LG_VAR_ATTN_BWD_RESTATS = 1 << 16
+LG_VAR_REDUCE_PER_BLOCK = 1 << 17
 LG_OPT_ADAM, LG_OPT_ADAMW, LG_OPT_SGD, LG_OPT_RMSPROP = 0, 1, 2, 3
 LG_OPT_AMSGRAD, LG_OPT_NESTEROV, LG_OPT_CENTERED = 1, 2, 4
 LG_ABI_VERSION = 2
@@ -68,6 +69,8 @@
         v |= LG_VAR_FFN_H3_RECOMPUTE
     if env.get('LG_ATTN_BWD_STATS', '') == 'recompute':
         v |= LG_VAR_ATTN_BWD_RESTATS
+    if env.get('LG_REDUCE', '') == 'per_block':
+        v |= LG_VAR_REDUCE_PER_BLOCK
     return v
 
 
diff --git a/lgteun_amd/csrc/api.hip b/lgteun_amd/csrc/api.hip
--- a/lgteun_amd/csrc/api.hip
+++ b/lgteun_amd/csrc/api.hip
@@ -141,6 +141,7 @@
         p->attn_bf16x3 = (v & LG_VAR_ATTN_BF16X3) ? 1 : 0;
         p->ffn_h3_re = (v & LG_VAR_FFN_H3_RECOMPUTE) ? 1 : 0;
         p->attn_restats = (v & LG_VAR_ATTN_BWD_RESTATS) ? 1 : 0;
+        p->reduce_per_block = (v & LG_VAR_REDUCE_PER_BLOCK) ? 1 : 0;
     }
     p->off = (int64_t*)malloc(sizeof(int64_t) * n_offsets);
     memcpy(p->off, offsets, sizeof(int64_t) * n_offsets);
diff --git a/lgteun_amd/csrc/bwd_kernels.h b/lgteun_amd/csrc/bwd_kernels.h
--- a/lgteun_amd/csrc/bwd_kernels.h
+++ b/lgteun_amd/csrc/bwd_kernels.h
@@ -32,22 +32,37 @@
     float* dst2;
     long nslices, slice_stride;
     int rows, cols, row_stride, ld, rows_valid, cols_valid;
+    int next = -1;
+    int v4 = -1;
 };
 #define LG_MAX_REDUCE_JOBS 56
+#define LG_RQ_MAX_JOBS 512
 struct ReduceJobTable {
     ReduceJob j[LG_MAX_REDUCE_JOBS];
     int n;
+};
+struct ReduceImage {
+    int nheads, njobs, total_wgs, pad;
+    int wg_start[LG_RQ_MAX_JOBS];
+    ReduceJob j[LG_RQ_MAX_JOBS];
 };
 struct ReduceQueue {
     float* arena;
     size_t cap, off;
     hipStream_t stream;
-    ReduceJobTable tab;
-    void init(float* base, size_t cap_floats, hipStream_t s) { arena = base; cap = cap_floats; off = 0; stream = s; tab.n = 0; }
+    bool per_block;
+    int n;
+    ReduceJob jobs[LG_RQ_MAX_JOBS];
+    void init(float* base, size_t cap_floats, hipStream_t s, bool per_block_form) {
+        arena = base; cap = cap_floats; off = 0; stream = s; per_block = per_block_form; n = 0;
+    }
     float* take(size_t nfloats);
     int push(const ReduceJob& j);
     int flush();
-};
+    int block_end() { return per_block ? flush() : 0; }
+};
+#define LG_RQ_NSTATS 6
+void reduce_queue_stats(long long out[LG_RQ_NSTATS], int reset);
 int launch_reduce_slab_wb(const float* wslab, const float* bslab, long nslices, int rows, int cols, float* dW, int ld, float* db, hipStream_t s);
 int launch_reduce_job(const ReduceJob& j, hipStream_t s);
 bool reduce_chan_enqueue(const float* part, const ChanReduce& m, int* rc);
diff --git a/lgteun_amd/csrc/common.h b/lgteun_amd/csrc/common.h
--- a/lgteun_amd/csrc/common.h
+++ b/lgteun_amd/csrc/common.h
@@ -42,6 +42,7 @@
     bool attn_saves_stats(int e) const { return cfg.precision == 0 && !attn_fwd_valu && !attn_restats && !(e == 32 && attn_bwd_core_m); }
     bool attn_f16x2() const { return cfg.precision == 0 && !attn_bf16x3 && !attn_fwd_valu && ffn_tile == 0 && !ffn_bf16x3; }
     int attn_fwd_valu;
+    int reduce_per_block;
     int dstep_tiles;
     bool dstep_fused(int h, int w) const;
     int bwd32_old;
diff --git a/lgteun_amd/csrc/k_bwd.hip b/lgteun_amd/csrc/k_bwd.hip
--- a/lgteun_amd/csrc/k_bwd.hip
+++ b/lgteun_amd/csrc/k_bwd.hip
@@ -7,7 +7,7 @@
 struct BwdBufs {
     float *dzA, *dzB, *gu3, *gs1, *gu1, *gr, *gd3, *gt1, *gd1;
     float *dx[3];
-    float *dh2, *dh1, *y2, *do2, *dg, *dym, *cat, *y1, *dqkv, *dpos_slab;
+    float *dh2, *dh1, *y2, *do2, *dg, *dym, *cat, *y1, *dqkv;
     float *w3t[5], *w2t[5], *w1t[5], *wsp, *dt, *dskip, *v, *du, *fft_scratch;
     float* slab_arena;
     float* attn_stats;
@@ -17,6 +17,10 @@
     size_t bytes;
 };
 
+static size_t dpos_slab_floats() {
+    const size_t f = (size_t)ATTN_BWD_F_WGS * ATTN_BWD_F_ROW, r3 = (size_t)512 * 2 * 64 * 64;
+    return f > r3 ? f : r3;
+}
 static void carve_bwd(const lg_plan* plan, int B, void* base, BwdBufs& bb) {
     const lg_config& c = plan->cfg;
     Carver cv{reinterpret_cast<char*>(base), 0};
@@ -30,7 +34,6 @@
     bb.dym = cv.take(P0 * E); bb.cat = cv.take(P0 * E); bb.y1 = cv.take(P0 * 16 > P0 * E / 2 ? P0 * 16 : P0 * E / 2);
     bb.dqkv = cv.take(P0 * 2 * E);
     bb.attn_stats = cv.take(P0 * 8);
-    bb.dpos_slab = cv.take((size_t)ATTN_BWD_F_WGS * ATTN_BWD_F_ROW > (size_t)512 * 2 * 64 * 64 ? (size_t)ATTN_BWD_F_WGS * ATTN_BWD_F_ROW : (size_t)512 * 2 * 64 * 64);
     for (int j = 0; j < 5; ++j) { bb.w3t[j] = cv.take(8 * E * 2 * E); bb.w2t[j] = cv.take(8 * E * 8 * E); bb.w1t[j] = cv.take(8 * E * 2 * E); }
     bb.wsp = cv.take(ffn_wsplit_bytes(32) / sizeof(float));
     size_t sl = wgrad_slab_floats((int)(8 * E), (int)(8 * E), (long)P0);
@@ -49,7 +52,7 @@
     if (ffn_dw_bwd_x_slab_floats(16) > sl) sl = ffn_dw_bwd_x_slab_floats(16);
     if (ffn_dw_bwd_x_slab_floats(32) > sl) sl = ffn_dw_bwd_x_slab_floats(32);
     if (ffn_dw_bwd_h_slab_floats() > sl) sl = ffn_dw_bwd_h_slab_floats();
-    bb.slab_cap = 4 * sl;
+    bb.slab_cap = 5 * (4 * sl + dpos_slab_floats());
     bb.slab_arena = cv.take(bb.slab_cap);
     bb.ffn_scales = nullptr;
     bb.dt = cv.take(P0 * E); bb.dskip = cv.take(P0 * E); bb.v = cv.take(P1 * E); bb.du = cv.take(P1 * E);
@@ -65,8 +68,8 @@
 #define RC(x) do { int rc__ = (x); if (rc__) return rc__; } while (0)
 
 struct ReduceQueueScope {
-    explicit ReduceQueueScope(BwdBufs& bb, hipStream_t s) {
-        bb.rq.init(bb.slab_arena, bb.slab_cap, s);
+    explicit ReduceQueueScope(BwdBufs& bb, hipStream_t s, bool per_block) {
+        bb.rq.init(bb.slab_arena, bb.slab_cap, s, per_block);
         reduce_queue_begin(&bb.rq);
     }
     ~ReduceQueueScope() { (void)reduce_queue_end(); }
@@ -226,7 +229,8 @@
         af.pos = P + pl->blk(st, j, B_POS);
         af.ln1g = P + pl->blk(st, j, B_LN1G); af.ln1b = P + pl->blk(st, j, B_LN1B);
         af.qkvw = P + pl->blk(st, j, B_QKVW); af.qkvb = P + pl->blk(st, j, B_QKVB); af.projw = P + pl->blk(st, j, B_PROJW);
-        af.slab = bb.dpos_slab;
+        af.slab = bb.rq.take((size_t)ATTN_BWD_F_WGS * ATTN_BWD_F_ROW);
+        if (!af.slab) return -3;
         af.d_pos = G + pl->blk(st, j, B_POS); af.d_qkvw = G + pl->blk(st, j, B_QKVW); af.d_qkvb = G + pl->blk(st, j, B_QKVB);
         af.d_projw = G + pl->blk(st, j, B_PROJW); af.d_ln1g = G + pl->blk(st, j, B_LN1G); af.d_ln1b = G + pl->blk(st, j, B_LN1B);
         af.B = B; af.h = fb.h; af.w = fb.w;
@@ -244,7 +248,8 @@
     AttnBwdArgs at;
     at.x = fb.xin; at.dy = tmp; at.dym = dym; at.o2 = fb.o2; at.dg = bb.dg; at.dx = dx_out;
     at.cat = bb.cat; at.y1 = bb.y1; at.dqkv = bb.dqkv;
-    at.pos = P + pl->blk(st, j, B_POS); at.posT = posT; at.dpos_slab = bb.dpos_slab;
+    at.pos = P + pl->blk(st, j, B_POS); at.posT = posT; at.dpos_slab = bb.rq.take((size_t)512 * 2 * 64 * 64);
+    if (!at.dpos_slab) return -3;
     at.ln1g = P + pl->blk(st, j, B_LN1G); at.ln1b = P + pl->blk(st, j, B_LN1B);
     at.qkvw = P + pl->blk(st, j, B_QKVW); at.qkvb = P + pl->blk(st, j, B_QKVB); at.projw = P + pl->blk(st, j, B_PROJW);
     at.d_ln1g = G + pl->blk(st, j, B_LN1G); at.d_ln1b = G + pl->blk(st, j, B_LN1B); at.part = bb.rq.take(attn_bwd_part_floats(e));
@@ -255,7 +260,7 @@
     if (pl->attn_saves_stats(e) && !(e == 32 && pl->attn_bwd_core_m)) { at.so = fb.att_o; at.sl = fb.att_l; }
     RC(launch_attn_bwd(e, at, s));
     const int grid = attn_bwd_grid(e, B, fb.h, fb.w);
-    RC(launch_reduce_slab(bb.dpos_slab, grid, 1, 2 * 64 * 64, G + pl->blk(st, j, B_POS), 2 * 64 * 64, 1, 2 * 64 * 64, s));
+    RC(launch_reduce_slab(at.dpos_slab, grid, 1, 2 * 64 * 64, G + pl->blk(st, j, B_POS), 2 * 64 * 64, 1, 2 * 64 * 64, s));
     RC(wgrad(dym, e, bb.cat, e, G + pl->blk(st, j, B_PROJW), e, G + pl->blk(st, j, B_PROJB), Pn, e, e, e, e, 0, 0, bb, s));
     if (!attn_bwd_fuses_qkv(e)) {
         const int y1ld = (hc + 15) / 16 * 16, dqld = (3 * hc + 15) / 16 * 16;
@@ -269,7 +274,7 @@
                      const float* dy, float* tmp, float* dx_out, int B, int flags, uint64_t seed, hipStream_t s) {
     RC(ffn_half_bwd(pl, P, G, st, j, fb, bb, dy, tmp, B, s));
     RC(mixer_half_bwd(pl, P, G, st, j, fb, bb, posT, tmp, dx_out, B, flags, seed, s));
-    return bb.rq.flush();
+    return bb.rq.block_end();
 }
 
 int op_block_bwd(const lg_plan* pl, const float* P, float* G, int st, int j, int which, const float* dy, float* dx, NetBufs& nb,
@@ -280,7 +285,7 @@
     bb.ffn_scales = nb.ffn_scales;
     const BlockBufs& fb = nb.blk[j];
     if (which == 0) return fft_bwd_call(pl, P, G, st, j, fb, dy, dx, B, s, nb.fft_scratch, bb.slab_arena);
-    ReduceQueueScope rqs(bb, s);
+    ReduceQueueScope rqs(bb, s, pl->reduce_per_block != 0);
     int rc = which == 1 ? 0 : ffn_transposes(pl, P, st, j, j + 1, nb, bb, s);
     if (!rc) rc = which == 1 ? mixer_half_bwd(pl, P, G, st, j, fb, bb, nb.posT, dy, dx, B, 0, 0, s)
                              : ffn_half_bwd(pl, P, G, st, j, fb, bb, dy, dx, B, s);
@@ -310,7 +315,7 @@
         gg.rw = G + pl->shared(S_RW); gg.rb = G + pl->shared(S_RB); gg.rtw = G + pl->shared(S_RTW); gg.rtb = G + pl->shared(S_RTB);
         gg.eta = G + pl->eta(st);
         RC(launch_dstep_bwd(a, gg, s));
-        return bb.rq.flush();
+        return bb.rq.block_end();
     }
     DstepTopArgs t;
     t.g = g; t.s1 = nb.s1[st]; t.z = zin; t.pan = pan; t.gu = bb.gu3; t.dz = dz;
@@ -347,7 +352,7 @@
     if (!d.part) return -3;
     RC(launch_dw_bwd(0, d, s));
     RC(launch_resample_adj(0, bb.gd1, dz, planes, H, W, 1, s));
-    return bb.rq.flush();
+    return bb.rq.block_end();
 }
 
 static int lgt_bwd(const lg_plan* pl, const float* P, float* G, int st, const NetBufs& nb, BwdBufs& bb, const float* dout,
@@ -401,7 +406,7 @@
                      const float* g, float* dz, int B, hipStream_t s) {
     BwdBufs bb;
     carve_bwd(pl, B, bwd_ws, bb);
-    ReduceQueueScope rqs(bb, s);
+    ReduceQueueScope rqs(bb, s, pl->reduce_per_block != 0);
     const int rc = data_step_bwd(pl, P, G, st, nb, bb, z_in, pan, g, dz, B, s);
     const int rc2 = reduce_queue_end();
     return rc ? rc : rc2;
@@ -414,7 +419,7 @@
     bb.fft_scratch = nb.fft_scratch;
     bb.ffn_scales = nb.ffn_scales;
     bb.dzA = dz;
-    ReduceQueueScope rqs(bb, s);
+    ReduceQueueScope rqs(bb, s, pl->reduce_per_block != 0);
     const int rc = lgt_bwd(pl, P, G, st, nb, bb, dout, z, B, flags, seed, s);
     const int rc2 = reduce_queue_end();
     return rc ? rc : rc2;
@@ -428,13 +433,15 @@
     carve_bwd(pl, B, bwd_ws, bb);
     bb.fft_scratch = nb.fft_scratch;
     bb.ffn_scales = nb.ffn_scales;
-    ReduceQueueScope rqs(bb, s);
+    ReduceQueueScope rqs(bb, s, pl->reduce_per_block != 0);
     if (flags & LG_FLAG_CHAINED) {
         const float* g = dout;
         for (int i = c.K - 1; i >= 0; --i) {
             const NetBufs sv = stage_view(nb, i);
             RC(lgt_bwd(pl, P, G, i, sv, bb, g, nb.Z[i + 1], B, flags, seed, s));
+            if (!bb.rq.per_block) RC(bb.rq.flush());
             RC(data_step_bwd(pl, P, G, i, nb, bb, nb.X[i], pan, bb.dzA, bb.dzB, B, s));
+            RC(bb.rq.flush());
             g = bb.dzB;
         }
         return reduce_queue_end();
@@ -443,6 +450,7 @@
     const bool do_data = !(flags & (LG_FLAG_BWD_LGT | LG_FLAG_BWD_DATA)) || (flags & LG_FLAG_BWD_DATA);
     if (do_lgt) RC(lgt_bwd(pl, P, G, c.K - 1, nb, bb, dout, nb.Z[c.K], B, flags, seed, s));
     if (!do_data) return reduce_queue_end();
+    if (do_lgt && !bb.rq.per_block) RC(bb.rq.flush());
     float* g = bb.dzA;
     float* dz = bb.dzB;
     for (int i = c.K - 1; i >= 0; --i) {
diff --git a/lgteun_amd/csrc/k_wgrad.hip b/lgteun_amd/csrc/k_wgrad.hip
--- a/lgteun_amd/csrc/k_wgrad.hip
+++ b/lgteun_amd/csrc/k_wgrad.hip
@@ -1,6 +1,11 @@
 #include "kernels.h"
 #include "bwd_kernels.h"
 #include "hstore.h"
+#include <string.h>
+#include <algorithm>
+#include <chrono>
+#include <mutex>
+#include <vector>
 
 typedef float f32x4 __attribute__((ext_vector_type(4)));
 
@@ -180,35 +185,49 @@
     }
 }
 
-__global__ __launch_bounds__(256) void k_reduce_jobs(ReduceJobTable t) {
-    __shared__ float4 part[16][17];
-    const ReduceJob& jb = t.j[blockIdx.y];
+__host__ __device__ inline bool reduce_job_v4(const ReduceJob& jb) {
+    return ((jb.cols | jb.row_stride | jb.ld) & 3) == 0 && (jb.slice_stride & 3) == 0 && jb.rows_valid == jb.rows && jb.cols_valid == jb.cols &&
+           ((reinterpret_cast<uintptr_t>(jb.slab) | reinterpret_cast<uintptr_t>(jb.dst) | reinterpret_cast<uintptr_t>(jb.dst2)) & 15) == 0;
+}
+__host__ __device__ inline long reduce_job_wgs(const ReduceJob& jb, bool v4) {
+    const long n = (long)jb.rows * jb.cols;
+    return v4 ? ((n >> 2) + 15) / 16 : (n + 15) / 16;
+}
+typedef __attribute__((address_space(1))) const float* rq_gsrc;
+typedef __attribute__((address_space(1))) float* rq_gdst;
+typedef __attribute__((address_space(1))) const f32x4* rq_gsrc4;
+typedef __attribute__((address_space(1))) f32x4* rq_gdst4;
+__device__ __forceinline__ float4 rq_ld4(rq_gsrc p) { const f32x4 v = *(rq_gsrc4)p; return make_float4(v.x, v.y, v.z, v.w); }
+__device__ __forceinline__ void rq_add4(rq_gdst p, const float4& t) {
+    const rq_gdst4 d = (rq_gdst4)p;
+    const f32x4 v = *d;
+    *d = (f32x4){v.x + t.x, v.y + t.y, v.z + t.z, v.w + t.w};
+}
+template <bool V4>
+__device__ __forceinline__ void reduce_job_wg(const ReduceJob& jb, long wg, float4 (*part)[17]) {
     const long n = (long)jb.rows * jb.cols;
     const int o = threadIdx.x & 15, ph = threadIdx.x >> 4;
-    const bool v4 = ((jb.cols | jb.row_stride | jb.ld) & 3) == 0 && (jb.slice_stride & 3) == 0 && jb.rows_valid == jb.rows && jb.cols_valid == jb.cols &&
-                    ((reinterpret_cast<uintptr_t>(jb.slab) | reinterpret_cast<uintptr_t>(jb.dst) | reinterpret_cast<uintptr_t>(jb.dst2)) & 15) == 0;
-    if (v4) {
+    if (V4) {
         const long n4 = n >> 2;
-        if (blockIdx.x * 16L >= n4) return;
-        const long i4 = blockIdx.x * 16L + o;
+        const long i4 = wg * 16L + o;
         const long i = i4 << 2;
         const int row = (int)(i / jb.cols), col = (int)(i - (long)row * jb.cols);
         float4 sv[8];
 #pragma unroll
         for (int u = 0; u < 8; ++u) sv[u] = make_float4(0.f, 0.f, 0.f, 0.f);
         if (i4 < n4) {
-            const float* __restrict__ src = jb.slab + (long)row * jb.row_stride + col;
+            const rq_gsrc src = (rq_gsrc)jb.slab + (long)row * jb.row_stride + col;
             const long ss = jb.slice_stride, ns = jb.nslices;
             long k = ph;
             for (; k + 16 * 7 < ns; k += 16 * 8) {
                 float4 ld[8];
 #pragma unroll
-                for (int u = 0; u < 8; ++u) ld[u] = *reinterpret_cast<const float4*>(src + (k + 16 * u) * ss);
+                for (int u = 0; u < 8; ++u) ld[u] = rq_ld4(src + (k + 16 * u) * ss);
 #pragma unroll
                 for (int u = 0; u < 8; ++u) { sv[u].x += ld[u].x; sv[u].y += ld[u].y; sv[u].z += ld[u].z; sv[u].w += ld[u].w; }
             }
             for (; k < ns; k += 16) {
-                const float4 l = *reinterpret_cast<const float4*>(src + k * ss);
+                const float4 l = rq_ld4(src + k * ss);
                 sv[0].x += l.x; sv[0].y += l.y; sv[0].z += l.z; sv[0].w += l.w;
             }
         }
@@ -219,23 +238,18 @@
             float4 ts = make_float4(0.f, 0.f, 0.f, 0.f);
 #pragma unroll
             for (int q = 0; q < 16; ++q) ts = add4(ts, part[q][o]);
-            float4* d = reinterpret_cast<float4*>(jb.dst + (long)row * jb.ld + col);
-            *d = add4(*d, ts);
-            if (jb.dst2) {
-                float4* d2 = reinterpret_cast<float4*>(jb.dst2 + (long)row * jb.ld + col);
-                *d2 = add4(*d2, ts);
-            }
+            rq_add4((rq_gdst)jb.dst + (long)row * jb.ld + col, ts);
+            if (jb.dst2) rq_add4((rq_gdst)jb.dst2 + (long)row * jb.ld + col, ts);
         }
         return;
     }
-    if (blockIdx.x * 16L >= n) return;
-    const long i = blockIdx.x * 16L + o;
+    const long i = wg * 16L + o;
     const int row = (int)(i / jb.cols), col = (int)(i - (long)row * jb.cols);
     float sv[8];
 #pragma unroll
     for (int u = 0; u < 8; ++u) sv[u] = 0.f;
     if (i < n) {
-        const float* __restrict__ src = jb.slab + (long)row * jb.row_stride + col;
+        const rq_gsrc src = (rq_gsrc)jb.slab + (long)row * jb.row_stride + col;
         const long ss = jb.slice_stride, ns = jb.nslices;
         long k = ph;
         for (; k + 16 * 7 < ns; k += 16 * 8) {
@@ -251,51 +265,270 @@
         float tsum = 0.f;
 #pragma unroll
         for (int q = 0; q < 16; ++q) tsum += parts[q * 17 + o];
-        jb.dst[(long)row * jb.ld + col] += tsum;
-        if (jb.dst2) jb.dst2[(long)row * jb.ld + col] += tsum;
-    }
+        ((rq_gdst)jb.dst)[(long)row * jb.ld + col] += tsum;
+        if (jb.dst2) ((rq_gdst)jb.dst2)[(long)row * jb.ld + col] += tsum;
+    }
+}
+
+__device__ __forceinline__ ReduceJob reduce_job_uniform(const ReduceJob* p) {
+    constexpr int NW = sizeof(ReduceJob) / 4;
+    const int* q = reinterpret_cast<const int*>(p);
+    int w[NW];
+#pragma unroll
+    for (int k = 0; k < NW; ++k) w[k] = __builtin_amdgcn_readfirstlane(q[k]);
+    ReduceJob j;
+    __builtin_memcpy(&j, w, sizeof(ReduceJob));
+    return j;
+}
+__device__ __forceinline__ void reduce_chain_wg(const ReduceJob* jb, const ReduceJob* tab, long wg, float4 (*part)[17]) {
+    ReduceJob j = reduce_job_uniform(jb);
+    const bool v4 = j.v4 == 1;
+    for (;;) {
+        if (v4) reduce_job_wg<true>(j, wg, part);
+        else reduce_job_wg<false>(j, wg, part);
+        if (j.next < 0) break;
+        j = reduce_job_uniform(tab + j.next);
+        __syncthreads();
+    }
+}
+__global__ __launch_bounds__(256) void k_reduce_jobs_tab(ReduceJobTable t) {
+    __shared__ float4 part[16][17];
+    const ReduceJob& jb = t.j[blockIdx.y];
+    const bool v4 = reduce_job_v4(jb);
+    if ((long)blockIdx.x >= reduce_job_wgs(jb, v4)) return;
+    if (v4) reduce_job_wg<true>(jb, blockIdx.x, part);
+    else reduce_job_wg<false>(jb, blockIdx.x, part);
+}
+__global__ __launch_bounds__(256) void k_reduce_jobs(const ReduceImage* __restrict__ img) {
+    __shared__ float4 part[16][17];
+    __shared__ int s_cnt;
+    const int nh = img->nheads;
+    if (threadIdx.x == 0) s_cnt = 0;
+    __syncthreads();
+    int c = 0;
+    for (int k = threadIdx.x; k < nh; k += 256) c += img->wg_start[k] <= (int)blockIdx.x ? 1 : 0;
+    if (c) atomicAdd(&s_cnt, c);
+    __syncthreads();
+    const int job = __builtin_amdgcn_readfirstlane(s_cnt) - 1;
+    const int wg0 = __builtin_amdgcn_readfirstlane(img->wg_start[job]);
+    reduce_chain_wg(img->j + job, img->j, (long)((int)blockIdx.x - wg0), part);
 }
 
 static thread_local ReduceQueue* tl_rq = nullptr;
+static std::atomic<long long> g_rq_stats[LG_RQ_NSTATS];
+void reduce_queue_stats(long long out[LG_RQ_NSTATS], int reset) {
+    for (int k = 0; k < LG_RQ_NSTATS; ++k) out[k] = reset ? g_rq_stats[k].exchange(0) : g_rq_stats[k].load();
+}
+extern "C" __attribute__((visibility("default"))) int lg_debug_reduce_stats(long long* out6, int reset) {
+    if (!out6) return -1;
+    reduce_queue_stats(out6, reset);
+    return 0;
+}
 void reduce_queue_begin(ReduceQueue* q) { tl_rq = q; }
 int reduce_queue_end() {
     ReduceQueue* q = tl_rq;
     tl_rq = nullptr;
     return q ? q->flush() : 0;
 }
+
+namespace {
+constexpr int RQ_SLOTS = 16;
+struct RqSlot { std::vector<char> host; uint64_t hash = 0; };
+struct RqCache {
+    ReduceImage* dev = nullptr;
+    RqSlot slot[RQ_SLOTS];
+    int next_victim = 0;
+};
+std::mutex g_rq_mu;
+RqCache* g_rq_cache[64];
+size_t image_bytes(const ReduceImage& im) { return offsetof(ReduceImage, j) + (size_t)im.njobs * sizeof(ReduceJob); }
+uint64_t fnv1a(const char* p, size_t n) {
+    uint64_t h = 1469598103934665603ull;
+    const uint64_t* q = reinterpret_cast<const uint64_t*>(p);
+    for (size_t k = 0; k < n / 8; ++k) { h ^= q[k]; h *= 1099511628211ull; }
+    return h;
+}
+struct RqExtent { uintptr_t lo, hi; long ld; long cols; int job; };
+bool extents_clash(const RqExtent& a, const RqExtent& b) {
+    const long ld = a.ld ? a.ld : b.ld;
+    if (!ld) return true;
+    if ((a.ld && a.ld != ld) || (b.ld && b.ld != ld)) return true;
+    if (a.cols > ld || b.cols > ld) return true;
+    const long d = (long)(((b.lo - a.lo) / sizeof(float)) % (uintptr_t)ld);
+    return !(d >= a.cols && d + b.cols <= ld);
+}
+int check_disjoint(const ReduceImage& im) {
+    std::vector<RqExtent> ex;
+    ex.reserve(2 * (size_t)im.nheads);
+    for (int k = 0; k < im.nheads; ++k) {
+        const ReduceJob& j = im.j[k];
+        if (j.rows_valid <= 0 || j.cols_valid <= 0) continue;
+        float* dsts[2] = {j.dst, j.dst2};
+        for (float* d : dsts) {
+            if (!d) continue;
+            RqExtent e;
+            e.lo = reinterpret_cast<uintptr_t>(d);
+            e.hi = reinterpret_cast<uintptr_t>(d + (long)(j.rows_valid - 1) * j.ld + j.cols_valid);
+            e.ld = j.rows_valid > 1 ? j.ld : 0;
+            e.cols = j.cols_valid;
+            e.job = k;
+            ex.push_back(e);
+        }
+    }
+    std::sort(ex.begin(), ex.end(), [](const RqExtent& a, const RqExtent& b) { return a.lo < b.lo; });
+    for (size_t a = 0; a < ex.size(); ++a)
+        for (size_t b = a + 1; b < ex.size() && ex[b].lo < ex[a].hi; ++b)
+            if (extents_clash(ex[a], ex[b])) {
+                lg_set_error("reduce queue: jobs %d and %d of one launch add into the same gradient elements", ex[a].job, ex[b].job);
+                return -4;
+            }
+    return 0;
+}
+int launch_image(const ReduceImage& im, hipStream_t s) {
+    const size_t bytes = image_bytes(im);
+    const char* src = reinterpret_cast<const char*>(&im);
+    const uint64_t h = fnv1a(src, bytes);
+    std::lock_guard<std::mutex> lock(g_rq_mu);
+    RqCache*& c = g_rq_cache[DeviceOnce::dev()];
+    if (!c) {
+        RqCache* nc = new RqCache;
+        hipError_t e = hipMalloc(reinterpret_cast<void**>(&nc->dev), sizeof(ReduceImage) * RQ_SLOTS);
+        if (e != hipSuccess) { delete nc; lg_set_error("reduce queue: hipMalloc(job tables): %s", hipGetErrorString(e)); return (int)e; }
+        c = nc;
+    }
+    for (int k = 0; k < RQ_SLOTS; ++k) {
+        const RqSlot& sl = c->slot[k];
+        if (sl.hash == h && sl.host.size() == bytes && memcmp(sl.host.data(), src, bytes) == 0) {
+            k_reduce_jobs<<<(unsigned)im.total_wgs, 256, 0, s>>>(c->dev + k);
+            LG_CHECK_LAUNCH();
+            return 0;
+        }
+    }
+    int rc = check_disjoint(im);
+    if (rc) return rc;
+    const int k = c->next_victim;
+    c->next_victim = (k + 1) % RQ_SLOTS;
+    RqSlot& sl = c->slot[k];
+    hipError_t e = hipDeviceSynchronize();
+    if (e != hipSuccess) { lg_set_error("reduce queue: hipDeviceSynchronize: %s", hipGetErrorString(e)); return (int)e; }
+    sl.host.clear();
+    sl.hash = 0;
+    e = hipMemcpyAsync(c->dev + k, src, bytes, hipMemcpyHostToDevice, s);
+    if (e == hipSuccess) e = hipStreamSynchronize(s);
+    if (e != hipSuccess) { lg_set_error("reduce queue: upload of a job table: %s", hipGetErrorString(e)); return (int)e; }
+    sl.host.assign(src, src + bytes);
+    sl.hash = h;
+    g_rq_stats[2]++;
+    k_reduce_jobs<<<(unsigned)im.total_wgs, 256, 0, s>>>(c->dev + k);
+    LG_CHECK_LAUNCH();
+    return 0;
+}
+}
+
+extern "C" __attribute__((visibility("default"))) int lg_debug_reduce_disjoint(int n, const long long* dst_off, const long long* dst2_off,
+                                                                                const int* rows_valid, const int* cols_valid, const int* ld) {
+    if (n < 0 || n > LG_RQ_MAX_JOBS || !dst_off || !dst2_off || !rows_valid || !cols_valid || !ld) return -1;
+    static thread_local ReduceImage im;
+    float* const base = reinterpret_cast<float*>((uintptr_t)1 << 32);
+    for (int k = 0; k < n; ++k) {
+        ReduceJob& j = im.j[k];
+        j = ReduceJob();
+        j.slab = nullptr; j.dst = base + dst_off[k]; j.dst2 = dst2_off[k] >= 0 ? base + dst2_off[k] : nullptr;
+        j.rows = j.rows_valid = rows_valid[k]; j.cols = j.cols_valid = cols_valid[k]; j.ld = ld[k];
+    }
+    im.nheads = im.njobs = n;
+    return check_disjoint(im);
+}
+
 int ReduceQueue::flush() {
     off = 0;
-    if (tab.n == 0) return 0;
-    long nmax = 0;
-    for (int k = 0; k < tab.n; ++k) {
-        const long n = (long)tab.j[k].rows * tab.j[k].cols;
-        if (n > nmax) nmax = n;
-    }
-    dim3 grid((unsigned)((nmax + 15) / 16), (unsigned)tab.n);
+    if (n == 0) return 0;
+    const int nj = n;
+    n = 0;
+    g_rq_stats[0]++;
+    if (per_block) {
+        static thread_local ReduceJobTable tab;
+        long nmax = 0;
+        for (int k = 0; k < nj; ++k) {
+            tab.j[k] = jobs[k];
+            const long m = (long)jobs[k].rows * jobs[k].cols;
+            if (m > nmax) nmax = m;
+        }
+        tab.n = nj;
+        dim3 grid((unsigned)((nmax + 15) / 16), (unsigned)nj);
+        k_reduce_jobs_tab<<<grid, 256, 0, stream>>>(tab);
+        LG_CHECK_LAUNCH();
+        return 0;
+    }
+    static thread_local ReduceImage im;
+    static thread_local int head_of[LG_RQ_MAX_JOBS], tail_of[LG_RQ_MAX_JOBS], slot_of[LG_RQ_MAX_JOBS], heads[LG_RQ_MAX_JOBS], prev_of[LG_RQ_MAX_JOBS];
+    static thread_local int by_dst[4 * LG_RQ_MAX_JOBS];
+    const auto t0 = std::chrono::steady_clock::now();
+    memset(by_dst, 0xff, sizeof(by_dst));
+    int nheads = 0;
+    for (int i = 0; i < nj; ++i) {
+        const ReduceJob& a = jobs[i];
+        int h = -1;
+        unsigned p = (unsigned)((reinterpret_cast<uintptr_t>(a.dst) >> 2) * 0x9E3779B97F4A7C15ull >> 40) % (4 * LG_RQ_MAX_JOBS);
+        for (; by_dst[p] >= 0; p = (p + 1) % (4 * LG_RQ_MAX_JOBS)) {
+            const ReduceJob& b = jobs[by_dst[p]];
+            if (b.dst == a.dst && b.dst2 == a.dst2 && b.rows == a.rows && b.cols == a.cols && b.ld == a.ld && b.rows_valid == a.rows_valid &&
+                b.cols_valid == a.cols_valid) {
+                h = by_dst[p];
+                break;
+            }
+        }
+        if (h < 0) { by_dst[p] = i; heads[nheads++] = i; head_of[i] = i; tail_of[i] = i; prev_of[i] = -1; }
+        else { head_of[i] = h; prev_of[i] = tail_of[h]; tail_of[h] = i; }
+    }
+    int pos = 0;
+    for (int k = 0; k < nheads; ++k) slot_of[heads[k]] = pos++;
+    for (int i = 0; i < nj; ++i) if (head_of[i] != i) slot_of[i] = pos++;
+    memset(&im, 0, offsetof(ReduceImage, j));
+    for (int i = 0; i < nj; ++i) {
+        ReduceJob& d = im.j[slot_of[i]];
+        d = jobs[i];
+        d.next = -1;
+        d.v4 = reduce_job_v4(jobs[i]) ? 1 : 0;
+    }
+    for (int i = 0; i < nj; ++i) {
+        if (prev_of[i] >= 0) im.j[slot_of[prev_of[i]]].next = slot_of[i];
+        if (!im.j[slot_of[i]].v4) im.j[slot_of[head_of[i]]].v4 = 0;
+    }
+    long total = 0;
+    for (int k = 0; k < nheads; ++k) {
+        im.wg_start[k] = (int)total;
+        total += reduce_job_wgs(im.j[k], im.j[k].v4 == 1);
+    }
+    if (total <= 0 || total > 0x3fffffffL) { lg_set_error("reduce queue: %ld workgroups in one launch", total); return -4; }
+    im.nheads = nheads; im.njobs = nj; im.total_wgs = (int)total;
 #ifdef LG_RQ_DEBUG
-    fprintf(stderr, "[rq] flush: %d jobs, grid.x %u:", tab.n, grid.x);
-    for (int k = 0; k < tab.n; ++k) fprintf(stderr, " (%ld sl x %d x %d)", tab.j[k].nslices, tab.j[k].rows, tab.j[k].cols);
-    fprintf(stderr, "\n");
+    fprintf(stderr, "[rq] flush: %d jobs, %d chains, %ld workgroups\n", nj, nheads, total);
 #endif
-    k_reduce_jobs<<<grid, 256, 0, stream>>>(tab);
-    tab.n = 0;
-    LG_CHECK_LAUNCH();
-    return 0;
+    const int rc = launch_image(im, stream);
+    if (g_rq_stats[3].load() < nj) g_rq_stats[3] = nj;
+    if (g_rq_stats[5].load() < nheads) g_rq_stats[5] = nheads;
+    g_rq_stats[4] += std::chrono::duration_cast<std::chrono::nanoseconds>(std::chrono::steady_clock::now() - t0).count();
+    return rc;
 }
 int ReduceQueue::push(const ReduceJob& j) {
-    if (tab.n == LG_MAX_REDUCE_JOBS) {
+    if (n == (per_block ? LG_MAX_REDUCE_JOBS : LG_RQ_MAX_JOBS)) {
         const size_t keep = off;
+        g_rq_stats[1]++;
         int rc = flush();
         off = keep;
         if (rc) return rc;
     }
-    tab.j[tab.n++] = j;
+    jobs[n++] = j;
     return 0;
 }
 float* ReduceQueue::take(size_t nfloats) {
     nfloats = (nfloats + 63) & ~(size_t)63;
     if (nfloats > cap) { lg_set_error("reduce queue: slab of %zu floats exceeds the arena (%zu)", nfloats, cap); return nullptr; }
-    if (off + nfloats > cap && flush()) return nullptr;
+    if (off + nfloats > cap) {
+        g_rq_stats[1]++;
+        if (flush()) return nullptr;
+    }
     float* p = arena + off;
     off += nfloats;
     return p;
@@ -321,11 +554,11 @@
 }
 int launch_reduce_job(const ReduceJob& j, hipStream_t s) {
     if (tl_rq) return tl_rq->push(j);
-    ReduceJobTable t;
+    static thread_local ReduceJobTable t;
     t.j[0] = j;
     t.n = 1;
     const long n = (long)j.rows * j.cols;
-    k_reduce_jobs<<<dim3((unsigned)((n + 15) / 16), 1), 256, 0, s>>>(t);
+    k_reduce_jobs_tab<<<dim3((unsigned)((n + 15) / 16), 1), 256, 0, s>>>(t);
     LG_CHECK_LAUNCH();
     return 0;
 }
```

New measurement: 6217 image-pairs/sec (median of 6 runs). +1.1%, better.
